# chsakell/aca-dotnet-workshop

Measured on AMD Instinct MI355X. Metric: tasks_e2e_per_sec, higher is better.
Workload: dtype n/a (JSON over HTTP)

## Files before the change

aca_dotnet_workshop_amd/native/src/applog.hpp:

```cpp
#pragma once

#include <fcntl.h>
#include <pthread.h>
#include <sys/stat.h>
#include <unistd.h>

#include <cerrno>
#include <algorithm>
#include <atomic>
#include <chrono>
#include <condition_variable>
#include <cstdint>
#include <cstdio>
#include <cstdlib>
#include <cstring>
#include <exception>
#include <functional>
#include <future>
#include <map>
#include <mutex>
#include <stdexcept>
#include <string>
#include <string_view>
#include <thread>
#include <vector>

namespace tt {

class AppLog {
 public:
  AppLog() = default;
  AppLog(const AppLog&) = delete;
  AppLog& operator=(const AppLog&) = delete;
  ~AppLog() {
    stop_committer();
    close();
  }

  bool open(const std::string& path, int fsync_mode) {
    path_ = path;
    fsync_ = fsync_mode;
    open_fd();
    if (fsync_ == 2 && !gc_thread_.joinable()) gc_thread_ = std::thread([this] { commit_loop(); });
    return true;
  }
  bool is_open() const { return fd_ >= 0; }
  uint64_t bytes() const { return bytes_; }
  const std::string& path() const { return path_; }

  void close() {
    std::lock_guard<std::mutex> f(fd_mu_);
    if (fd_ >= 0) { ::close(fd_); fd_ = -1; }
  }

  bool group() const { return fsync_ == 2 && fd_ >= 0; }
  uint64_t mark() const { return written_.load(std::memory_order_acquire); }
  void after_durable(uint64_t mark, std::function<void()> cb) {
    if (!group() || synced_.load(std::memory_order_acquire) >= mark) {
      cb();
      return;
    }
    {
      std::lock_guard<std::mutex> l(gc_mu_);
      waiters_.emplace(mark, std::move(cb));
      gc_want_ = true;
    }
    gc_cv_.notify_one();
  }
  void wait_durable(uint64_t mark) {
    if (!group() || synced_.load(std::memory_order_acquire) >= mark) return;
    std::promise<void> done;
    auto f = done.get_future();
    after_durable(mark, [&done] { done.set_value(); });
    f.wait();
  }
  void wait_durable() { wait_durable(mark()); }
  struct CommitStats {
    uint64_t syncs, acks, written, synced;
    double sync_ms_total, sync_ms_max;
  };
  CommitStats commit_stats() {
    std::lock_guard<std::mutex> l(gc_mu_);
    return {gc_syncs_, gc_acks_, mark(), synced_.load(), gc_sync_s_ * 1e3, gc_sync_max_s_ * 1e3};
  }

  static void put_field(std::string& rec, std::string_view f) {
    uint32_t n = (uint32_t)f.size();
    rec.append(reinterpret_cast<const char*>(&n), 4);
    rec.append(f.data(), f.size());
  }
  template <class T>
  static std::string_view pod(const T& v) { return std::string_view(reinterpret_cast<const char*>(&v), sizeof(T)); }

  void append(char kind, const std::vector<std::string_view>& fields) {
    if (fd_ < 0) return;
    std::string rec;
    rec.resize(5);
    rec[4] = kind;
    for (auto f : fields) put_field(rec, f);
    uint32_t total = (uint32_t)rec.size();
    std::memcpy(&rec[0], &total, 4);
    if (batching_) {
      batch_ += rec;
      return;
    }
    write_all(rec);
  }

  class BatchScope {
   public:
    explicit BatchScope(AppLog& log) : log_(log) { log_.batching_ = true; }
    ~BatchScope() noexcept(false) {
      log_.batching_ = false;
      if (log_.batch_.empty()) return;
      std::string b;
      b.swap(log_.batch_);
      if (std::uncaught_exceptions() == 0) {
        log_.write_all(b);
        return;
      }
      try {
        log_.write_all(b);
      } catch (...) {
      }
    }
    BatchScope(const BatchScope&) = delete;
    BatchScope& operator=(const BatchScope&) = delete;

   private:
    AppLog& log_;
  };

  void replay(const std::function<void(char, std::vector<std::string_view>&)>& fn) {
    if (fd_ < 0) return;
    std::string data;
    data.resize(bytes_);
    size_t off = 0;
    while (off < data.size()) {
      ssize_t r = ::pread(fd_, &data[off], data.size() - off, (off_t)off);
      if (r <= 0) break;
      off += (size_t)r;
    }
    size_t pos = 0;
    std::vector<std::string_view> fields;
    while (pos + 5 <= off) {
      uint32_t total;
      std::memcpy(&total, &data[pos], 4);
      if (total < 5 || pos + total > off) break;
      char kind = data[pos + 4];
      fields.clear();
      size_t p = pos + 5, end = pos + total;
      bool ok = true;
      while (p < end) {
        if (p + 4 > end) { ok = false; break; }
        uint32_t n;
        std::memcpy(&n, &data[p], 4);
        p += 4;
        if (p + n > end) { ok = false; break; }
        fields.emplace_back(&data[p], n);
        p += n;
      }
      if (!ok) break;
      fn(kind, fields);
      pos = end;
    }
    if (pos < bytes_) {
      if (::ftruncate(fd_, (off_t)pos) == 0) bytes_ = pos;
    }
  }

  void rewrite(const std::function<void(AppLog&)>& writer) {
    if (fd_ < 0) return;
    std::string tmp = path_ + ".compact";
    AppLog out;
    ::unlink(tmp.c_str());
    out.open(tmp, 0);
    writer(out);
    ::fdatasync(out.fd_);
    out.close();
    {
      std::lock_guard<std::mutex> f(fd_mu_);
      if (::rename(tmp.c_str(), path_.c_str()) != 0) throw std::runtime_error("log compaction rename failed");
      if (fd_ >= 0) ::close(fd_);
      fd_ = -1;
      open_fd_locked();
    }
    if (fsync_ == 2) {
      {
        std::lock_guard<std::mutex> l(gc_mu_);
        gc_want_ = true;
      }
      gc_cv_.notify_one();
    }
  }

  void sync() {
    std::lock_guard<std::mutex> f(fd_mu_);
    if (fd_ >= 0) ::fdatasync(fd_);
  }

 private:
  static FILE* stall_file(double& min_s) {
    static double th = [] {
      const char* p = std::getenv("TT_STALL_MS");
      double ms = p && *p ? std::atof(p) : 100.0;
      return (ms > 0 ? ms : 100.0) / 1e3;
    }();
    static FILE* f = [] {
      const char* p = std::getenv("TT_STALL_LOG");
      return p && *p ? std::fopen(p, "a") : nullptr;
    }();
    min_s = th;
    return f;
  }

  void write_all(const std::string& rec) {
    double min_s;
    FILE* stall = stall_file(min_s);
    auto t0 = stall ? std::chrono::steady_clock::now() : std::chrono::steady_clock::time_point{};
    size_t off = 0;
    while (off < rec.size()) {
      ssize_t w = ::write(fd_, rec.data() + off, rec.size() - off);
      if (w < 0) {
        if (errno == EINTR) continue;
        throw std::runtime_error(std::string("log write failed: ") + std::strerror(errno));
      }
      off += (size_t)w;
    }
    bytes_ += rec.size();
    written_.fetch_add(rec.size(), std::memory_order_release);
    if (fsync_ == 1) ::fdatasync(fd_);
    if (stall) {
      double s = std::chrono::duration<double>(std::chrono::steady_clock::now() - t0).count();
      if (s > min_s) {
        double wall = std::chrono::duration<double>(std::chrono::system_clock::now().time_since_epoch()).count();
        std::fprintf(stall, "{\"what\": \"log-write\", \"ms\": %.2f, \"bytes\": %zu, \"log\": \"%s\", \"pid\": %d, \"wall\": %.4f}\n",
                     s * 1e3, rec.size(), path_.c_str(), (int)::getpid(), wall);
        std::fflush(stall);
      }
    }
  }

  void open_fd() {
    std::lock_guard<std::mutex> f(fd_mu_);
    open_fd_locked();
  }
  void open_fd_locked() {
    fd_ = ::open(path_.c_str(), O_RDWR | O_CREAT | O_APPEND | O_CLOEXEC, 0644);
    if (fd_ < 0) throw std::runtime_error("cannot open log " + path_ + ": " + std::strerror(errno));
    struct stat st;
    if (::fstat(fd_, &st) == 0) bytes_ = (uint64_t)st.st_size;
  }

  void commit_loop() {
    pthread_setname_np(pthread_self(), "tt-log-commit");
    std::unique_lock<std::mutex> l(gc_mu_);
    static const auto delay = [] {
      const char* v = std::getenv("TT_LOG_COMMIT_DELAY_US");
      return std::chrono::microseconds(v && *v ? std::max(0L, std::atol(v)) : 100L);
    }();
    while (true) {
      gc_cv_.wait(l, [this] { return gc_stop_ || gc_want_; });
      if (gc_stop_ && waiters_.empty()) return;
      if (delay.count() > 0 && !gc_stop_) gc_cv_.wait_for(l, delay, [this] { return gc_stop_; });
      gc_want_ = false;
      l.unlock();
      const uint64_t target = written_.load(std::memory_order_acquire);
      const auto t0 = std::chrono::steady_clock::now();
      {
        std::lock_guard<std::mutex> f(fd_mu_);
        if (fd_ >= 0) ::fdatasync(fd_);
      }
      const double s = std::chrono::duration<double>(std::chrono::steady_clock::now() - t0).count();
      uint64_t prev = synced_.load();
      while (prev < target && !synced_.compare_exchange_weak(prev, target)) {
      }
      std::vector<std::function<void()>> ready;
      l.lock();
      ++gc_syncs_;
      gc_sync_s_ += s;
      gc_sync_max_s_ = std::max(gc_sync_max_s_, s);
      auto end = waiters_.upper_bound(target);
      for (auto it = waiters_.begin(); it != end; ++it) ready.push_back(std::move(it->second));
      waiters_.erase(waiters_.begin(), end);
      gc_acks_ += ready.size();
      if (!waiters_.empty()) gc_want_ = true;
      l.unlock();
      for (auto& f : ready) f();
      l.lock();
    }
  }
  void stop_committer() {
    if (!gc_thread_.joinable()) return;
    {
      std::lock_guard<std::mutex> l(gc_mu_);
      gc_stop_ = true;
      gc_want_ = true;
    }
    gc_cv_.notify_one();
    gc_thread_.join();
  }

  int fd_ = -1;
  int fsync_ = 0;
  uint64_t bytes_ = 0;
  std::string path_;
  bool batching_ = false;
  std::string batch_;
  std::mutex fd_mu_;
  std::atomic<uint64_t> written_{0}, synced_{0};
  std::mutex gc_mu_;
  std::condition_variable gc_cv_;
  std::multimap<uint64_t, std::function<void()>> waiters_;
  std::thread gc_thread_;
  bool gc_stop_ = false, gc_want_ = false;
  uint64_t gc_syncs_ = 0, gc_acks_ = 0;
  double gc_sync_s_ = 0, gc_sync_max_s_ = 0;
};

}
```

aca_dotnet_workshop_amd/native/src/backingfront.hpp:

```cpp
#pragma once

#include <condition_variable>
#include <deque>
#include <filesystem>
#include <unordered_set>

#include <fcntl.h>
#include <unistd.h>

#include <sys/eventfd.h>

#include <array>
#include <atomic>
#include <cassert>
#include <cstring>
#include <map>
#include <mutex>
#include <shared_mutex>
#include <thread>
#include <unordered_map>

#include "broker.hpp"
#include "docstore.hpp"
#include "evhttp.hpp"
#include "json.hpp"
#include "textutil.hpp"

namespace tt {

namespace bf {

using text::unquote;
inline std::string jstr(std::string_view s) { return text::json_str(s); }
inline bool utf8_ok(std::string_view s) { return text::valid_utf8(s); }
inline std::string b64(std::string_view in) { return text::base64(in); }

inline std::string problem_json(int status, std::string_view detail) {
  return "{\"type\": \"https://tools.ietf.org/html/rfc9110#section-15." + std::to_string(status / 100) +
         "\", \"title\": " + jstr(ev::reason_phrase(status)) + ", \"status\": " + std::to_string(status) +
         ", \"detail\": " + jstr(detail) + "}";
}

struct Grant {
  std::string principal, scope;
  std::vector<std::string> actions;
};

}

inline bool scan_bulk_items(const std::string& body, std::vector<DocStore::BulkItem>& out) {
  std::string_view text = body.empty() ? std::string_view("[]") : std::string_view(body);
  if (!valid(text)) return false;
  const char* p = ws_end(text.data(), text.data() + text.size());
  const char* e = text.data() + text.size();
  if (*p != '[') return false;
  ++p;
  while (true) {
    p = ws_end(p, e);
    if (*p == ']') return true;
    if (*p != '{') return false;
    ++p;
    DocStore::BulkItem b;
    bool have_key = false, have_value = false;
    while (true) {
      p = ws_end(p, e);
      if (*p == '}') { ++p; break; }
      const char* ks = p;
      p = skip_value(p, e);
      std::string_view ktok(ks, (size_t)(p - ks));
      std::string k = ktok.find('\\') == std::string_view::npos ? std::string(ktok.substr(1, ktok.size() - 2))
                                                               : parse(ktok).s;
      p = ws_end(ws_end(p, e) + 1, e);
      const char* vs = p;
      p = skip_value(p, e);
      std::string_view raw(vs, (size_t)(p - vs));
      if (k == "key") {
        if (raw.front() != '"') return false;
        b.key = raw.find('\\') == std::string_view::npos ? std::string(raw.substr(1, raw.size() - 2)) : parse(raw).s;
        have_key = true;
      } else if (k == "value") {
        have_value = true;
        b.value = raw.front() == '"' ? parse(raw).s : compact(raw);
      } else if (k == "etag") {
        b.etag.reset();
        if (raw.front() == '"') {
          std::string s = parse(raw).s;
          if (!s.empty()) b.etag = std::move(s);
        }
      } else if (k == "firstWrite") {
        b.first_write = raw == "true";
      } else if (k == "ttlMs") {
        if (raw.front() != 'n' && raw.front() != '"' && std::strtod(std::string(raw).c_str(), nullptr) != 0) return false;
      }
      p = ws_end(p, e);
      if (*p == ',') ++p;
    }
    if (!have_key) return false;
    if (!have_value) b.value = "null";
    out.push_back(std::move(b));
    p = ws_end(p, e);
    if (*p == ',') ++p;
  }
}

inline bool scan_value_array(const char* p, const char* e, std::vector<std::string>& out);

inline bool scan_bulk_values(const std::string& body, std::vector<std::string>& out) {
  std::string_view text = body.empty() ? std::string_view("[]") : std::string_view(body);
  if (!valid(text)) return false;
  return scan_value_array(ws_end(text.data(), text.data() + text.size()), text.data() + text.size(), out);
}

inline bool scan_tx_values(const std::string& body, std::vector<std::string>& out) {
  std::string_view text(body);
  if (text.empty() || !valid(text)) return false;
  const char* e = text.data() + text.size();
  const char* p = ws_end(text.data(), e);
  if (*p != '{') return false;
  ++p;
  bool found = false;
  while (true) {
    p = ws_end(p, e);
    if (*p == '}') return found;
    const char* ks = p;
    p = skip_value(p, e);
    std::string_view ktok(ks, (size_t)(p - ks));
    std::string k = ktok.find('\\') == std::string_view::npos ? std::string(ktok.substr(1, ktok.size() - 2))
                                                             : parse(ktok).s;
    p = ws_end(ws_end(p, e) + 1, e);
    if (k == "ops") {
      out.clear();
      if (!scan_value_array(p, e, out)) return false;
      found = true;
    }
    p = ws_end(skip_value(p, e), e);
    if (*p == ',') ++p;
  }
}

inline bool scan_value_array(const char* p, const char* e, std::vector<std::string>& out) {
  if (*p != '[') return false;
  ++p;
  while (true) {
    p = ws_end(p, e);
    if (*p == ']') return true;
    if (*p != '{') return false;
    ++p;
    std::string value = "null";
    while (true) {
      p = ws_end(p, e);
      if (*p == '}') { ++p; break; }
      const char* ks = p;
      p = skip_value(p, e);
      std::string_view ktok(ks, (size_t)(p - ks));
      std::string k = ktok.find('\\') == std::string_view::npos ? std::string(ktok.substr(1, ktok.size() - 2))
                                                               : parse(ktok).s;
      p = ws_end(ws_end(p, e) + 1, e);
      const char* vs = p;
      p = skip_value(p, e);
      std::string_view raw(vs, (size_t)(p - vs));
      if (k == "value") value = raw.front() == '"' ? parse(raw).s : compact(raw);
      p = ws_end(p, e);
      if (*p == ',') ++p;
    }
    out.push_back(std::move(value));
    p = ws_end(p, e);
    if (*p == ',') ++p;
  }
}

class BackingFront {
 public:
  BackingFront(const std::string& host, int port, const std::string& fallback_uds, int threads = 1,
               const std::string& uds = "")
      : fallback_(ev::Endpoint::parse("unix:" + fallback_uds)) {
    ev::reserve_fd_table();
    threads = std::max(1, std::min(threads, 64));
    for (int i = 0; i < threads; ++i) {
      shards_.push_back(std::make_shared<Shard>(*this));
      shards_.back()->self = shards_.back();
    }
    ev::Endpoint ep;
    ep.unix_socket = false;
    ep.host = host;
    ep.port = port;
    for (auto& sh : shards_) {
      int p = ev::listen_on(sh->loop, ep, sh->handler, threads > 1);
      if (ep.port == 0) ep.port = p;
    }
    port_ = ep.port;
    if (!uds.empty()) {
      ev::Endpoint u;
      u.path = uds;
      int unused = 0;
      int fd = ev::bind_listen(u, false, unused);
      for (size_t i = 0; i < shards_.size(); ++i) {
        int f = i == 0 ? fd : ::fcntl(fd, F_DUPFD_CLOEXEC, 0);
        if (f < 0) break;
        auto l = std::make_shared<ev::Listener>(shards_[i]->loop, f, shards_[i]->handler);
        l->hand_off = [this, i](int c) {
          size_t to = next_uds_shard_.fetch_add(1, std::memory_order_relaxed) % shards_.size();
          if (to == i) return false;
          Shard* sh = shards_[to].get();
          sh->post_task([sh, c] { ev::adopt(sh->loop, c, sh->handler); });
          return true;
        };
        shards_[i]->loop.add(l, EPOLLIN | EPOLLEXCLUSIVE);
      }
    }
    for (auto& sh : shards_) sh->start();
  }
  ~BackingFront() { stop(); }

  struct QueryJob {
    std::string account, db, coll, body, prefix, traceparent, sent_mono, front_mono;
    bool sort_keys = false;
  };
  struct QueryResult {
    int status = 0;
    std::string body;
    ev::HeaderList headers;
  };
  using QueryFn = std::function<QueryResult(const QueryJob&)>;
  void set_query_fn(QueryFn fn) {
    std::lock_guard l(q_mu_);
    query_fn_ = std::move(fn);
    if (q_threads_.empty() && query_fn_) {
      int n = 4;
      if (const char* v = std::getenv("TT_BACKING_QUERY_THREADS"); v && std::atoi(v) > 0) n = std::min(32, std::atoi(v));
      for (int i = 0; i < n; ++i)
        q_threads_.emplace_back([this] {
          pthread_setname_np(pthread_self(), "tt-front-query");
          query_loop();
        });
    }
  }

  int port() const { return port_; }
  int threads() const { return (int)shards_.size(); }

  void stop() {
    if (stopped_) return;
    stopped_ = true;
    {
      std::lock_guard l(q_mu_);
      q_stop_ = true;
    }
    q_cv_.notify_all();
    for (auto& t : q_threads_)
      if (t.joinable()) t.join();
    q_threads_.clear();
    {
      std::lock_guard l(q_mu_);
      query_fn_ = nullptr;
    }
    for (auto& sh : shards_) sh->request_stop();
    for (auto& sh : shards_) sh->join();
  }

  void attach_store(const std::string& account, const std::string& db, const std::string& coll, DocStore* s) {
    std::unique_lock l(cfg_mu_);
    auto& c = colls_[account + "\x1f" + db + "\x1f" + coll];
    if (!c) c = std::make_unique<Coll>();
    c->store = s;
  }
  void attach_broker(const std::string& ns, Broker* b) {
    std::unique_lock l(cfg_mu_);
    brokers_[ns] = b;
  }
  void set_policy(const std::string& mode, const std::vector<std::pair<std::string, std::string>>& keys,
                  const std::vector<std::tuple<std::string, std::string, std::vector<std::string>>>& grants) {
    std::unique_lock l(cfg_mu_);
    enforce_ = mode == "enforce";
    keys_ = keys;
    grants_.clear();
    for (auto& [p, s, a] : grants) grants_.push_back(bf::Grant{p, s, a});
  }
  void set_blob_root(const std::string& root) {
    std::lock_guard l(blob_mu_);
    blob_root_ = root;
  }
  void blob_note(const std::string& account, const std::string& container, const std::string& name, bool added) {
    std::lock_guard l(blob_mu_);
    auto& names = blob_names_locked(account, container);
    if (added) names.insert(name);
    else names.erase(name);
  }
  size_t blob_count(const std::string& account, const std::string& container, const std::string& prefix) {
    std::lock_guard l(blob_mu_);
    auto& names = blob_names_locked(account, container);
    if (prefix.empty()) return names.size();
    size_t n = 0;
    for (auto& x : names) n += x.compare(0, prefix.size(), prefix) == 0;
    return n;
  }

  void notify(const std::string& ns, const std::string& entity) {
    for (auto& sh : shards_) sh->post(ns + "|" + entity);
  }
  std::map<std::string, uint64_t> stats() {
    std::map<std::string, uint64_t> out;
    for (size_t i = 0; i < kCounters.size(); ++i)
      if (uint64_t v = counters_[i].load(std::memory_order_relaxed)) out[kCounters[i]] = v;
    return out;
  }

 private:
  struct Coll {
    DocStore* store = nullptr;
  };
  struct Shard;
  struct QueuedQuery {
    std::shared_ptr<QueryJob> job;
    Shard* sh = nullptr;
    ev::Reply reply;
  };
  std::mutex q_mu_;
  std::condition_variable q_cv_;
  std::deque<QueuedQuery> q_jobs_;
  QueryFn query_fn_;
  std::vector<std::thread> q_threads_;
  bool q_stop_ = false;
  struct Parked {
    std::string ns, entity;
    size_t max;
    int64_t lock_ms;
    double deadline;
    ev::Reply reply;
    bool storage = false;
  };
  struct Shard;
  struct Wake : ev::IoObj {
    Shard* sh;
    explicit Wake(Shard* x) : sh(x) {}
    void on_event(uint32_t) override;
  };
  struct Shard {
    BackingFront& f;
    ev::Loop loop;
    ev::Client client;
    ev::Handler handler;
    std::thread thread;
    int wake_fd = -1;
    std::atomic<bool> stop_flag{false};
    std::mutex mu;
    std::vector<std::string> posted;
    std::vector<std::function<void()>> tasks;
    std::multimap<std::string, Parked> parked;
    std::weak_ptr<Shard> self;

    explicit Shard(BackingFront& front) : f(front), client(loop) {
      handler = [this](ev::Message&& m, ev::Reply r) { f.on_request(*this, std::move(m), std::move(r)); };
      wake_fd = eventfd(0, EFD_NONBLOCK | EFD_CLOEXEC);
      auto w = std::make_shared<Wake>(this);
      w->fd = dup(wake_fd);
      loop.add(w, EPOLLIN);
    }
    ~Shard() {
      if (wake_fd >= 0) ::close(wake_fd);
    }
    void start() {
      thread = std::thread([this] {
        pthread_setname_np(pthread_self(), "tt-front");
        ev::GapTracer gaps("backing-front");
        gaps.attach(loop);
        loop.run([this, &gaps](double t) {
          gaps.tick(t);
          on_tick(t);
        });
      });
    }
    std::atomic<bool> wake_pending{false};
    void wake() {
      if (wake_pending.exchange(true, std::memory_order_acq_rel)) return;
      uint64_t one = 1;
      ssize_t r = ::write(wake_fd, &one, sizeof one);
      (void)r;
    }
    void post(std::string key) {
      {
        std::lock_guard l(mu);
        posted.push_back(std::move(key));
      }
      wake();
    }
    void post_task(std::function<void()> fn) {
      {
        std::lock_guard l(mu);
        tasks.push_back(std::move(fn));
      }
      wake();
    }
    void request_stop() {
      stop_flag = true;
      wake();
    }
    void join() {
      if (thread.joinable()) thread.join();
    }
    void on_wake() {
      if (stop_flag) {
        for (auto& kv : parked) kv.second.reply.json(503, bf::problem_json(503, "shutting down"));
        parked.clear();
        loop.stop();
        return;
      }
      std::vector<std::string> keys;
      std::vector<std::function<void()>> todo;
      wake_pending.store(false, std::memory_order_release);
      {
        std::lock_guard l(mu);
        keys.swap(posted);
        todo.swap(tasks);
      }
      for (auto& k : keys) f.retry_parked(*this, k);
      for (auto& fn : todo) fn();
    }
    void on_tick(double now) {
      if (stop_flag) {
        on_wake();
        return;
      }
      std::vector<std::string> keys;
      for (auto& kv : parked)
        if (keys.empty() || keys.back() != kv.first) keys.push_back(kv.first);
      for (auto& k : keys) f.retry_parked(*this, k, now);
    }
  };

  ev::Endpoint fallback_;
  std::vector<std::shared_ptr<Shard>> shards_;
  std::atomic<size_t> next_uds_shard_{0};
  int port_ = 0;
  bool stopped_ = false;

  std::shared_mutex cfg_mu_;
  std::unordered_map<std::string, std::unique_ptr<Coll>> colls_;
  std::unordered_map<std::string, Broker*> brokers_;
  bool enforce_ = false;
  std::vector<std::pair<std::string, std::string>> keys_;
  std::vector<bf::Grant> grants_;
  std::mutex blob_mu_;
  std::string blob_root_;
  std::unordered_map<std::string, std::unordered_set<std::string>> blob_names_;

  std::unordered_set<std::string>& blob_names_locked(const std::string& account, const std::string& container) {
    std::string key = account + "/" + container;
    auto it = blob_names_.find(key);
    if (it != blob_names_.end()) return it->second;
    auto& names = blob_names_[key];
    namespace fs = std::filesystem;
    std::error_code ec;
    fs::path root = fs::path(blob_root_) / account / container;
    if (!blob_root_.empty() && fs::is_directory(root, ec))
      for (auto i = fs::recursive_directory_iterator(root, ec); !ec && i != fs::recursive_directory_iterator();
           i.increment(ec)) {
        if (!i->is_regular_file(ec)) continue;
        std::string n = i->path().lexically_relative(root).string();
        if (!ends_with(n, ".meta.json") && !ends_with(n, ".tmp")) names.insert(std::move(n));
      }
    return names;
  }
  static bool ends_with(const std::string& s, const char* suf) {
    size_t n = std::strlen(suf);
    return s.size() >= n && s.compare(s.size() - n, n, suf) == 0;
  }
  static bool safe_name(const std::string& in, std::string& out) {
    out.clear();
    for (unsigned char c : in) {
      if (c >= 0x80) return false;
      bool keep = (c >= 'a' && c <= 'z') || (c >= 'A' && c <= 'Z') || (c >= '0' && c <= '9') || c == '.' || c == '_' ||
                  c == '-';
      out += keep ? (char)c : '_';
    }
    return true;
  }
  static bool write_file(const std::string& path, std::string_view data) {
    int fd = ::open(path.c_str(), O_WRONLY | O_CREAT | O_TRUNC | O_CLOEXEC, 0644);
    if (fd < 0) return false;
    size_t off = 0;
    while (off < data.size()) {
      ssize_t w = ::write(fd, data.data() + off, data.size() - off);
      if (w < 0 && errno == EINTR) continue;
      if (w <= 0) {
        ::close(fd);
        return false;
      }
      off += (size_t)w;
    }
    return ::close(fd) == 0;
  }

  bool handle_blob(ev::Message& m, ev::Reply& r, const std::vector<std::string>& seg, const std::string& qs) {
    std::string acct, cont, root;
    if (!safe_name(seg[1], acct) || !safe_name(seg[3], cont)) return false;
    {
      std::lock_guard l(blob_mu_);
      root = blob_root_;
    }
    if (root.empty()) return false;
    if (seg.size() == 4 && m.method == "GET") {
      std::string c = query_get(qs, "count");
      for (auto& ch : c) ch = ::tt::ascii_lower(ch);
      if (c != "1" && c != "true") return false;
      if (!authorize(m, r, "blob.read", "storage/" + seg[1])) return true;
      count("blob.count");
      r.send(200, {{"content-type", "application/json"}},
             "{\"count\": " + std::to_string(blob_count(acct, cont, query_get(qs, "prefix"))) + "}");
      return true;
    }
    if (seg.size() < 5 || m.method != "PUT") return false;
    std::string name;
    for (size_t i = 4; i < seg.size(); ++i) {
      const std::string& p = seg[i];
      if (p.empty() || p == "." || p == ".." || p.find('/') != std::string::npos) return false;
      for (unsigned char c : p)
        if (c < 0x20 || c >= 0x80) return false;
      if (i > 4) name += '/';
      name += p;
    }
    if (ends_with(name, ".tmp") || ends_with(name, ".meta.json")) return false;
    if (!authorize(m, r, "blob.write", "storage/" + seg[1])) return true;
    count("blob.put");
    namespace fs = std::filesystem;
    fs::path f = fs::path(root) / acct / cont / name;
    std::error_code ec;
    fs::create_directories(f.parent_path(), ec);
    const std::string tmp = f.string() + ".tmp";
    auto* ct = m.header("content-type");
    char meta[160];
    std::snprintf(meta, sizeof meta, ", \"lastModified\": %.6f, \"size\": %zu}",
                  std::chrono::duration<double>(std::chrono::system_clock::now().time_since_epoch()).count(),
                  m.body.size());
    if (ec || !write_file(tmp, m.body) || ::rename(tmp.c_str(), f.c_str()) != 0 ||
        !write_file(f.string() + ".meta.json",
                    "{\"contentType\": " + bf::jstr(ct ? *ct : "application/octet-stream") + meta)) {
      r.send(500, {{"content-type", "application/problem+json; charset=utf-8"}},
             bf::problem_json(500, "blob write failed: " + f.string()));
      return true;
    }
    blob_note(acct, cont, name, true);
    r.send(201, {{"content-type", "application/json"}},
           "{\"blobURL\": " + bf::jstr("/storage/" + seg[1] + "/blobs/" + seg[3] + "/" + name) + "}");
    return true;
  }

  static constexpr std::array<const char*, 19> kCounters = {
      "doc.put", "sb.publish", "sb.receive", "sb.settle", "doc.get", "doc.bulkget", "doc.bulkset", "doc.query",
      "doc.throttled", "doc.delete", "doc.query_worker", "doc.query_worker_done", "forwarded",
      "queue.put", "queue.get", "queue.delete", "queue.update", "blob.put", "blob.count"};
  std::array<std::atomic<uint64_t>, kCounters.size()> counters_{};

  void count(const char* k) {
    for (size_t i = 0; i < kCounters.size(); ++i)
      if (std::strcmp(kCounters[i], k) == 0) {
        counters_[i].fetch_add(1, std::memory_order_relaxed);
        return;
      }
    assert(!"unknown backing front counter");
  }
  void broadcast(Shard& here, const std::string& key) {
    retry_parked(here, key);
    if (shards_.size() > 1)
      for (auto& sh : shards_)
        if (sh.get() != &here) sh->post(key);
  }

  bool allowed(const ev::Message& m, const std::string& action, const std::string& scope) {
    std::shared_lock l(cfg_mu_);
    if (!enforce_) return true;
    auto* key = m.header("x-tt-key");
    if (key && !key->empty())
      for (auto& [ks, k] : keys_)
        if (scope.rfind(ks, 0) == 0 && *key == k) return true;
    auto* ident = m.header("x-tt-identity");
    if (ident && !ident->empty())
      for (auto& g : grants_) {
        if (g.principal != *ident || scope.rfind(g.scope, 0) != 0) continue;
        for (auto& a : g.actions)
          if (a == "*" || a == action) return true;
      }
    return false;
  }
  bool authorize(const ev::Message& m, const ev::Reply& r, const std::string& action, const std::string& scope) {
    if (allowed(m, action, scope)) return true;
    auto* ident = m.header("x-tt-identity");
    std::string who = ident && !ident->empty() ? *ident : "anonymous";
    r.send(403, {{"content-type", "application/problem+json; charset=utf-8"}},
           bf::problem_json(403, who + " is not authorized to perform " + action + " on " + scope));
    return false;
  }

  static void split(const std::string& target, std::string& path, std::string& qs) {
    auto q = target.find('?');
    path = target.substr(0, q);
    qs = q == std::string::npos ? "" : target.substr(q + 1);
  }
  static std::string query_get(const std::string& qs, const std::string& name) {
    size_t i = 0;
    while (i <= qs.size() && !qs.empty()) {
      size_t j = qs.find('&', i);
      if (j == std::string::npos) j = qs.size();
      std::string_view kv(qs.data() + i, j - i);
      size_t eq = kv.find('=');
      if (bf::unquote(kv.substr(0, eq), true) == name)
        return eq == std::string_view::npos ? "" : bf::unquote(kv.substr(eq + 1), true);
      i = j + 1;
    }
    return "";
  }

  void on_request(Shard& sh, ev::Message&& m, ev::Reply r) {
    std::string path, qs;
    split(m.target, path, qs);
    std::vector<std::string> seg;
    seg.reserve(8);
    for (size_t i = 1; i <= path.size();) {
      size_t j = path.find('/', i);
      if (j == std::string::npos) j = path.size();
      seg.push_back(bf::unquote(std::string_view(path).substr(i, j - i)));
      i = j + 1;
    }
    if (seg.size() == 6 && seg[0] == "cosmos" && seg[4] == "docs" && handle_doc(sh, m, r, seg)) return;
    if (seg.size() == 5 && seg[0] == "cosmos" && seg[4] == "bulkset" && m.method == "POST" &&
        handle_bulkset(sh, m, r, seg))
      return;
    if (seg.size() == 5 && seg[0] == "cosmos" && seg[4] == "bulkget" && m.method == "POST" && handle_bulkget(m, r, seg))
      return;
    if (seg.size() == 5 && seg[0] == "cosmos" && seg[4] == "query" && m.method == "POST" && handle_query(sh, m, r, seg, qs))
      return;
    if (seg.size() >= 3 && seg[0] == "servicebus" && handle_bus(sh, m, r, seg, qs)) return;
    if (seg.size() >= 5 && seg[0] == "storage" && seg[2] == "queues" && handle_storage_queue(sh, m, r, seg, qs)) return;
    if (seg.size() >= 4 && seg[0] == "storage" && seg[2] == "blobs" && handle_blob(m, r, seg, qs)) return;
    forward(sh, std::move(m), std::move(r));
  }

  void forward(Shard& sh, ev::Message&& m, ev::Reply r) {
    count("forwarded");
    ev::HeaderList h;
    for (auto& kv : m.headers)
      if (!ev::is_hop_header(kv.first)) h.push_back(kv);
    if (m.header("traceparent")) {
      char t[32];
      std::snprintf(t, sizeof t, "%.6f", ev::now_s());
      h.emplace_back("x-tt-front-mono", t);
    }
    sh.client.request(fallback_, m.method, m.target, h, m.body, 0, [r](ev::ClientResult&& res) {
      if (res.err) {
        r.send(503, {{"content-type", "application/problem+json; charset=utf-8"}},
               bf::problem_json(503, "backing control plane unreachable"));
        return;
      }
      if (res.resp.header("x-tt-handler-end-mono")) {
        ev::HeaderList h2 = res.resp.headers;
        char t[32];
        std::snprintf(t, sizeof t, "%.6f", ev::now_s());
        h2.emplace_back("x-tt-front-rx-mono", t);
        r.send(res.resp.status, h2, res.resp.body);
        return;
      }
      r.send(res.resp.status, res.resp.headers, res.resp.body);
    });
  }

  bool throttled(ev::Message& m, ev::Reply& r, DocStore* s, double ru, int kind) {
    if (!s->provisioned()) {
      s->charge(ru);
      return false;
    }
    uint64_t ticket = 0, out = 0;
    if (const std::string* t = m.header("x-tt-ru-ticket")) ticket = std::strtoull(t->c_str(), nullptr, 10);
    const uint64_t bind = DocStore::bind_of(m.method + " " + m.target,
                                            kind == DocStore::kQuery || m.method == "POST" ? std::string_view(m.body)
                                                                                           : std::string_view());
    int64_t wait_ms = s->charge(ru, ticket, out, bind, kind);
    if (!wait_ms) return false;
    count("doc.throttled");
    ev::HeaderList h{{"x-ms-retry-after-ms", std::to_string(wait_ms)},
                     {"retry-after", std::to_string((wait_ms + 999) / 1000)},
                     {"content-type", "application/problem+json; charset=utf-8"}};
    if (out) h.emplace_back("x-tt-ru-ticket", std::to_string(out));
    r.send(429, h, bf::problem_json(429, "Request rate is large: the container's provisioned throughput is exhausted"));
    return true;
  }

  Coll* coll_of(const std::vector<std::string>& seg) {
    thread_local std::string k;
    k.assign(seg[1]);
    k += '\x1f';
    k += seg[2];
    k += '\x1f';
    k += seg[3];
    std::shared_lock l(cfg_mu_);
    auto it = colls_.find(k);
    return it != colls_.end() && it->second->store ? it->second.get() : nullptr;
  }

  template <class Engine>
  void send_durable(Shard& sh, Engine* eng, ev::Reply& r, int status, ev::HeaderList h, std::string body) {
    if (!eng->group_commit()) {
      r.send(status, h, body);
      return;
    }
    std::weak_ptr<Shard> w = sh.self;
    eng->after_durable(eng->log_mark(), [w, r, status, h = std::move(h), body = std::move(body)] {
      if (auto s = w.lock()) s->post_task([r, status, h, body] { r.send(status, h, body); });
    });
  }

  bool handle_doc(Shard& sh, ev::Message& m, ev::Reply& r, const std::vector<std::string>& seg) {
    Coll* c = coll_of(seg);
    if (!c) return false;
    const std::string& key = seg[5];
    const std::string scope = "cosmos/" + seg[1];
    if (m.method == "GET") {
      if (!authorize(m, r, "cosmos.read", scope)) return true;
      count("doc.get");
      if (throttled(m, r, c->store, DocStore::read_ru(0), DocStore::kRead)) return true;
      auto v = c->store->get(key);
      if (!v) r.empty(404);
      else r.send(200, {{"etag", v->second}, {"content-type", "application/json"}}, v->first);
      return true;
    }
    if (m.method != "PUT" && m.method != "DELETE") return false;
    auto* ttl = m.header("x-tt-ttl-ms");
    if (ttl && !ttl->empty() && *ttl != "0") return false;
    if (!authorize(m, r, "cosmos.write", scope)) return true;
    auto* im = m.header("if-match");
    std::optional<std::string> etag;
    if (im && !im->empty()) etag = *im;
    const char* pj = "application/problem+json; charset=utf-8";
    if (throttled(m, r, c->store, DocStore::write_ru(m.method == "PUT" ? m.body.size() : 0),
                  m.method == "PUT" ? DocStore::kWrite : DocStore::kDelete))
      return true;
    if (m.method == "PUT") {
      count("doc.put");
      auto* fw = m.header("x-tt-first-write");
      try {
        std::string e = c->store->set(key, m.body, etag, fw && *fw == "1", 0);
        send_durable(sh, c->store, r, 200, {{"etag", e}, {"content-type", "application/json"}},
                     "{\"etag\": " + bf::jstr(e) + "}");
      } catch (const EtagMismatch& ex) {
        r.send(412, {{"content-type", pj}}, bf::problem_json(412, ex.what()));
      } catch (const ParseError& ex) {
        r.send(400, {{"content-type", pj}}, bf::problem_json(400, std::string("invalid JSON: ") + ex.what()));
      }
      return true;
    }
    count("doc.delete");
    try {
      bool ok = c->store->del(key, etag);
      if (ok) send_durable(sh, c->store, r, 204, {}, {});
      else r.empty(404);
    } catch (const EtagMismatch& ex) {
      r.send(412, {{"content-type", pj}}, bf::problem_json(412, ex.what()));
    }
    return true;
  }

  bool handle_bulkset(Shard& sh, ev::Message& m, ev::Reply& r, const std::vector<std::string>& seg) {
    Coll* c = coll_of(seg);
    if (!c) return false;
    std::vector<DocStore::BulkItem> batch;
    if (!scan_bulk_items(m.body, batch)) return false;
    if (!authorize(m, r, "cosmos.write", "cosmos/" + seg[1])) return true;
    count("doc.bulkset");
    double ru = 0;
    for (auto& b : batch) ru += DocStore::write_ru(b.value.size());
    if (throttled(m, r, c->store, ru, DocStore::kWrite)) return true;
    const std::vector<DocStore::BulkResult> res = c->store->set_many(batch);
    std::string out = "[";
    bool etag_err = false, other_err = false;
    for (size_t i = 0; i < res.size(); ++i) {
      if (i) out += ", ";
      out += "{\"key\": " + bf::jstr(batch[i].key);
      if (res[i].err == 0) {
        out += ", \"etag\": " + bf::jstr(res[i].etag) + "}";
      } else {
        (res[i].err == 1 ? etag_err : other_err) = true;
        out += std::string(", \"error\": ") + (res[i].err == 1 ? "\"etag\"" : "\"invalid\"") +
               ", \"detail\": " + bf::jstr(res[i].detail) + "}";
      }
    }
    out += "]";
    send_durable(sh, c->store, r, etag_err ? 412 : other_err ? 400 : 200, {{"content-type", "application/json"}}, out);
    return true;
  }

  bool handle_bulkget(ev::Message& m, ev::Reply& r, const std::vector<std::string>& seg) {
    Coll* c = coll_of(seg);
    if (!c) return false;
    Value body;
    try {
      body = parse(m.body);
    } catch (const ParseError&) {
      return false;
    }
    const Value* keys = body.get("keys");
    if (!keys || keys->t != Value::Array) return false;
    for (auto& k : keys->items)
      if (k.t != Value::String) return false;
    if (!authorize(m, r, "cosmos.read", "cosmos/" + seg[1])) return true;
    count("doc.bulkget");
    if (throttled(m, r, c->store, DocStore::read_ru(0) * (double)std::max<size_t>(1, keys->items.size()), DocStore::kRead))
      return true;
    std::string out = "[";
    for (size_t i = 0; i < keys->items.size(); ++i) {
      const std::string& k = keys->items[i].s;
      if (i) out += ", ";
      out += "{\"key\": " + bf::jstr(k);
      if (auto v = c->store->get(k)) out += ", \"data\": " + v->first + ", \"etag\": " + bf::jstr(v->second);
      out += "}";
    }
    out += "]";
    r.send(200, {{"content-type", "application/json"}}, out);
    return true;
  }

  static bool indexable(const Value* f) {
    if (!f || f->t != Value::Object || f->keys.size() != 1) return false;
    std::string op = f->keys[0];
    for (auto& ch : op) ch = (char)std::toupper((unsigned char)ch);
    const Value& arg = f->items[0];
    if (op == "EQ" || op == "IN") {
      if (arg.t != Value::Object || arg.items.empty()) return false;
      const Value& v = arg.items[0];
      auto plain = [](const Value& x) { return x.t == Value::Null || x.t == Value::Bool; };
      if (v.t != Value::Array) return !plain(v);
      for (auto& x : v.items)
        if (!plain(x)) return true;
      return false;
    }
    if (op == "AND") {
      if (arg.t != Value::Array) return false;
      for (auto& x : arg.items)
        if (indexable(&x)) return true;
      return false;
    }
    if (op == "OR") {
      if (arg.t != Value::Array || arg.items.empty()) return false;
      for (auto& x : arg.items)
        if (!indexable(&x)) return false;
      return true;
    }
    return false;
  }
  static bool sampled(const ev::Message& m) {
    const std::string* tp = m.header("traceparent");
    if (!tp || tp->size() < 55) return false;
    return (std::strtol(tp->c_str() + tp->size() - 2, nullptr, 16) & 1) != 0;
  }

  bool to_query_worker(Shard& sh, ev::Message& m, ev::Reply& r, Coll* c, const std::vector<std::string>& seg,
                       const std::string& qs) {
    {
      std::lock_guard l(q_mu_);
      if (!query_fn_ || q_stop_) return false;
    }
    if (!authorize(m, r, "cosmos.read", "cosmos/" + seg[1])) return true;
    if (throttled(m, r, c->store, DocStore::query_ru(0), DocStore::kQuery)) return true;
    count("doc.query_worker");
    auto job = std::make_shared<QueryJob>();
    job->account = seg[1];
    job->db = seg[2];
    job->coll = seg[3];
    job->body = std::move(m.body);
    job->prefix = query_get(qs, "prefix");
    std::string project = query_get(qs, "project");
    for (auto& ch : project) ch = (char)std::tolower((unsigned char)ch);
    job->sort_keys = project == "sortkeys";
    if (const std::string* tp = m.header("traceparent")) job->traceparent = *tp;
    if (const std::string* t = m.header("x-tt-sent-mono")) job->sent_mono = *t;
    char t[32];
    std::snprintf(t, sizeof t, "%.6f", ev::now_s());
    job->front_mono = t;
    {
      std::lock_guard l(q_mu_);
      q_jobs_.push_back({job, &sh, r});
    }
    q_cv_.notify_one();
    return true;
  }

  void query_loop() {
    while (true) {
      QueuedQuery qq;
      QueryFn fn;
      {
        std::unique_lock l(q_mu_);
        q_cv_.wait(l, [this] { return q_stop_ || !q_jobs_.empty(); });
        if (q_stop_) {
          for (auto& j : q_jobs_)
            j.sh->post_task([r = j.reply] { r.json(503, bf::problem_json(503, "shutting down")); });
          q_jobs_.clear();
          return;
        }
        qq = std::move(q_jobs_.front());
        q_jobs_.pop_front();
        fn = query_fn_;
      }
      QueryResult res;
      try {
        res = fn(*qq.job);
      } catch (const std::exception& ex) {
        res.status = 500;
        res.body = ex.what();
      }
      qq.sh->post_task([this, qq, res = std::move(res)]() mutable {
        count("doc.query_worker_done");
        if (res.status == 200) {
          if (!res.headers.empty()) {
            char t[32];
            std::snprintf(t, sizeof t, "%.6f", ev::now_s());
            res.headers.emplace_back("x-tt-front-rx-mono", t);
          }
          res.headers.emplace_back("content-type", "application/json");
          qq.reply.send(200, res.headers, res.body);
        } else {
          qq.reply.send(res.status ? res.status : 500, {{"content-type", "application/problem+json; charset=utf-8"}},
                        bf::problem_json(res.status ? res.status : 500, res.body));
        }
      });
    }
  }

  bool handle_query(Shard& sh, ev::Message& m, ev::Reply& r, const std::vector<std::string>& seg, const std::string& qs) {
    Coll* c = coll_of(seg);
    if (!c) return false;
    bool indexed = false;
    try {
      Value q = parse(m.body.empty() ? std::string("{}") : m.body);
      if (q.t != Value::Object) return false;
      indexed = indexable(q.get("filter"));
    } catch (const ParseError&) {
      return false;
    }
    if (!indexed || sampled(m)) return to_query_worker(sh, m, r, c, seg, qs);
    if (!authorize(m, r, "cosmos.read", "cosmos/" + seg[1])) return true;
    if (throttled(m, r, c->store, DocStore::query_ru(0), DocStore::kQuery)) return true;
    std::string body;
    try {
      std::string project = query_get(qs, "project");
      for (auto& ch : project) ch = (char)std::tolower((unsigned char)ch);
      body = c->store->query(m.body, query_get(qs, "prefix"), project == "sortkeys");
    } catch (const std::exception& ex) {
      r.send(400, {{"content-type", "application/problem+json; charset=utf-8"}}, bf::problem_json(400, ex.what()));
      return true;
    }
    count("doc.query");
    c->store->debit(DocStore::query_ru(body.size()) - DocStore::query_ru(0));
    r.send(200, {{"content-type", "application/json"}}, body);
    return true;
  }

  static std::string entity_scope(const std::string& entity) {
    auto p = entity.find("/subscriptions/");
    if (p != std::string::npos) return "topics/" + entity.substr(0, p);
    return "queues/" + entity;
  }

  bool handle_bus(Shard& sh, ev::Message& m, ev::Reply& r, const std::vector<std::string>& seg,
                  const std::string& qs) {
    Broker* b = nullptr;
    {
      std::shared_lock l(cfg_mu_);
      auto it = brokers_.find(seg[1]);
      if (it != brokers_.end()) b = it->second;
    }
    if (!b) return false;
    const std::string& ns = seg[1];
    if (seg.size() == 5 && seg[2] == "topics" && seg[4] == "messages" && m.method == "POST") {
      if (!authorize(m, r, "sb.send", "servicebus/" + ns + "/topics/" + seg[3])) return true;
      count("sb.publish");
      auto* ct = m.header("content-type");
      auto* props = m.header("x-tt-props");
      auto* mid = m.header("x-tt-message-id");
      auto* ttl = m.header("x-tt-ttl-ms");
      auto* delay = m.header("x-tt-delay-ms");
      uint64_t seq = b->publish(seg[3], m.body, ct ? *ct : "application/json", props ? *props : "{}", mid ? *mid : "",
                                ttl && !ttl->empty() ? std::atoll(ttl->c_str()) : 0,
                                delay && !delay->empty() ? std::atoll(delay->c_str()) : 0);
      send_durable(sh, b, r, 201, {{"content-type", "application/json"}}, "{\"seq\": " + std::to_string(seq) + "}");
      for (auto& sub : b->subscriptions(seg[3])) broadcast(sh, ns + "|" + seg[3] + "/subscriptions/" + sub);
      return true;
    }
    if (seg.size() == 3 && seg[2] == "receive" && m.method == "POST") {
      std::string entity = query_get(qs, "entity");
      if (!authorize(m, r, "sb.receive", "servicebus/" + ns + "/" + entity_scope(entity))) return true;
      count("sb.receive");
      std::string mx = query_get(qs, "max"), lk = query_get(qs, "lockMs"), wt = query_get(qs, "waitMs");
      Parked p{ns, entity, (size_t)std::max(1, mx.empty() ? 1 : std::atoi(mx.c_str())),
               lk.empty() ? 0 : std::atoll(lk.c_str()), ev::now_s() + (wt.empty() ? 0 : std::atoi(wt.c_str())) / 1000.0,
               r};
      if (!try_receive(b, p, false)) sh.parked.emplace(ns + "|" + entity, std::move(p));
      return true;
    }
    if (seg.size() == 3 && seg[2] == "settle" && m.method == "POST") {
      Value body;
      try {
        body = parse(m.body.empty() ? std::string_view("{}") : std::string_view(m.body));
      } catch (const std::exception&) {
        return false;
      }
      std::string entity;
      if (auto* e = body.get("entity"); e && e->t == Value::String) entity = e->s;
      if (!authorize(m, r, "sb.receive", "servicebus/" + ns + "/" + entity_scope(entity))) return true;
      count("sb.settle");
      auto list = [&](const char* k) -> const std::vector<Value>* {
        auto* v = body.get(k);
        return v && v->t == Value::Array ? &v->items : nullptr;
      };
      auto str = [](const Value& o, const char* k) {
        auto* v = o.get(k);
        return v && v->t == Value::String ? v->s : std::string();
      };
      auto num = [](const Value& o, const char* k) {
        auto* v = o.get(k);
        return v && v->t == Value::Number ? (int64_t)v->n : (int64_t)0;
      };
      std::string out = "{\"complete\": [";
      if (auto* l = list("complete"))
        for (size_t i = 0; i < l->size(); ++i) out += std::string(i ? ", " : "") + (b->complete(entity, (*l)[i].s) ? "true" : "false");
      out += "], \"abandon\": [";
      bool abandoned = false;
      if (auto* l = list("abandon"))
        for (size_t i = 0; i < l->size(); ++i) {
          abandoned = true;
          out += std::string(i ? ", " : "") +
                 (b->abandon(entity, str((*l)[i], "token"), num((*l)[i], "delayMs")) ? "true" : "false");
        }
      out += "], \"deadletter\": [";
      if (auto* l = list("deadletter"))
        for (size_t i = 0; i < l->size(); ++i)
          out += std::string(i ? ", " : "") +
                 (b->dead_letter(entity, str((*l)[i], "token"), str((*l)[i], "reason")) ? "true" : "false");
      out += "], \"renew\": [";
      if (auto* l = list("renew"))
        for (size_t i = 0; i < l->size(); ++i)
          out += std::string(i ? ", " : "") +
                 (b->renew(entity, str((*l)[i], "token"), num((*l)[i], "lockMs")) ? "true" : "false");
      out += "]}";
      send_durable(sh, b, r, 200, {{"content-type", "application/json"}}, out);
      if (abandoned) broadcast(sh, ns + "|" + entity);
      return true;
    }
    if (seg.size() == 3 && seg[2] == "counts" && m.method == "GET") {
      auto [a, s, l, d, e, c, rc] = b->counts(query_get(qs, "entity"));
      r.send(200, {{"content-type", "application/json"}},
             "{\"active\": " + std::to_string(a) + ", \"scheduled\": " + std::to_string(s) + ", \"locked\": " +
                 std::to_string(l) + ", \"dead_letter\": " + std::to_string(d) + ", \"enqueued\": " + std::to_string(e) +
                 ", \"completed\": " + std::to_string(c) + ", \"received\": " + std::to_string(rc) + "}");
      return true;
    }
    return false;
  }

  static bool plain_uint(const std::string& v, int64_t& out) {
    if (v.empty() || v.size() > 15) return false;
    int64_t x = 0;
    for (char c : v) {
      if (c < '0' || c > '9') return false;
      x = x * 10 + (c - '0');
    }
    out = x;
    return true;
  }
  static bool uint_param(const std::string& qs, const char* name, int64_t dflt, int64_t& out) {
    std::string v = query_get(qs, name);
    if (v.empty()) {
      out = dflt;
      return true;
    }
    return plain_uint(v, out);
  }

  bool handle_storage_queue(Shard& sh, ev::Message& m, ev::Reply& r, const std::vector<std::string>& seg,
                            const std::string& qs) {
    const std::string ns = "storage-" + seg[1];
    Broker* b = nullptr;
    {
      std::shared_lock l(cfg_mu_);
      auto it = brokers_.find(ns);
      if (it != brokers_.end()) b = it->second;
    }
    if (!b) return false;
    const std::string& account = seg[1];
    const std::string& queue = seg[3];
    if (seg.size() == 5 && seg[4] == "messages" && m.method == "POST") {
      int64_t ttl_s, delay_s;
      if (!uint_param(qs, "messagettl", 0, ttl_s) || !uint_param(qs, "visibilitytimeout", 0, delay_s)) return false;
      if (!authorize(m, r, "queue.send", "storage/" + account)) return true;
      count("queue.put");
      uint64_t seq = b->send(queue, m.body, "text/plain", "{}", "", ttl_s * 1000, delay_s * 1000);
      send_durable(sh, b, r, 201, {{"content-type", "application/json"}},
                   "{\"messageId\": \"" + std::to_string(seq) + "\"}");
      broadcast(sh, ns + "|" + queue);
      return true;
    }
    if (seg.size() == 5 && seg[4] == "messages" && m.method == "GET") {
      int64_t mx, vis, wait_ms;
      if (!uint_param(qs, "numofmessages", 1, mx) || mx < 1 || !uint_param(qs, "visibilityMs", 30000, vis) ||
          !uint_param(qs, "waitMs", 0, wait_ms))
        return false;
      if (!authorize(m, r, "queue.receive", "storage/" + account)) return true;
      count("queue.get");
      Parked p{ns, queue, (size_t)mx, vis, ev::now_s() + (double)wait_ms / 1000.0, r, true};
      if (!try_receive(b, p, false)) sh.parked.emplace(ns + "|" + queue, std::move(p));
      return true;
    }
    if (seg.size() == 6 && seg[4] == "messages" && (m.method == "DELETE" || m.method == "PUT")) {
      int64_t vis = 0;
      if (m.method == "PUT" && !uint_param(qs, "visibilityMs", 0, vis)) return false;
      if (!authorize(m, r, "queue.receive", "storage/" + account)) return true;
      count(m.method == "DELETE" ? "queue.delete" : "queue.update");
      bool ok = m.method == "DELETE" ? b->complete(queue, seg[5]) : b->abandon(queue, seg[5], vis);
      send_durable(sh, b, r, ok ? 204 : 404, {}, "");
      if (m.method == "PUT") broadcast(sh, ns + "|" + queue);
      return true;
    }
    return false;
  }

  bool try_receive(Broker* b, Parked& p, bool expired) {
    if (p.reply.abandoned()) {
      p.reply.send(204, {}, {});
      return true;
    }
    std::vector<Received> msgs;
    try {
      msgs = b->receive(p.entity, p.max, p.lock_ms);
    } catch (const std::exception& e) {
      p.reply.send(404, {{"content-type", "application/problem+json; charset=utf-8"}}, bf::problem_json(404, e.what()));
      return true;
    }
    if (msgs.empty() && !expired && ev::now_s() < p.deadline) return false;
    std::string out = "[";
    if (p.storage) {
      for (size_t i = 0; i < msgs.size(); ++i) {
        auto& x = msgs[i];
        if (i) out += ", ";
        out += "{\"messageId\": \"" + std::to_string(x.seq) + "\", \"popReceipt\": " + bf::jstr(x.lock_token) +
               ", \"dequeueCount\": " + std::to_string(x.delivery_count) +
               ", \"insertionMs\": " + std::to_string(x.enqueued_wall);
        if (bf::utf8_ok(x.body)) out += ", \"body\": " + bf::jstr(x.body) + "}";
        else out += ", \"bodyB64\": \"" + bf::b64(x.body) + "\"}";
      }
      out += "]";
      p.reply.send(200, {{"content-type", "application/json"}}, out);
      return true;
    }
    for (size_t i = 0; i < msgs.size(); ++i) {
      auto& x = msgs[i];
      if (i) out += ", ";
      std::string props = x.props.empty() ? "{}" : x.props;
      out += "{\"lockToken\": " + bf::jstr(x.lock_token) + ", \"seq\": " + std::to_string(x.seq) + ", \"id\": " +
             bf::jstr(x.id) + ", \"contentType\": " + bf::jstr(x.content_type) + ", \"props\": " + props +
             ", \"deliveryCount\": " + std::to_string(x.delivery_count) + ", \"enqueuedMs\": " +
             std::to_string(x.enqueued_wall);
      if (bf::utf8_ok(x.body)) out += ", \"body\": " + bf::jstr(x.body) + "}";
      else out += ", \"bodyB64\": \"" + bf::b64(x.body) + "\"}";
    }
    out += "]";
    p.reply.send(200, {{"content-type", "application/json"}}, out);
    return true;
  }

  void retry_parked(Shard& sh, const std::string& key, double now = 0) {
    auto range = sh.parked.equal_range(key);
    if (range.first == range.second) return;
    Broker* b = nullptr;
    {
      std::shared_lock l(cfg_mu_);
      auto it = brokers_.find(key.substr(0, key.find('|')));
      if (it != brokers_.end()) b = it->second;
    }
    for (auto it = range.first; it != range.second;) {
      bool expired = now > 0 && now >= it->second.deadline;
      if (b && try_receive(b, it->second, expired)) it = sh.parked.erase(it);
      else ++it;
    }
  }
};

inline void BackingFront::Wake::on_event(uint32_t) {
  uint64_t v;
  while (::read(fd, &v, sizeof v) == (ssize_t)sizeof v) {
  }
  sh->on_wake();
}

}
```

aca_dotnet_workshop_amd/native/src/broker.hpp:

```cpp
#pragma once

#include <chrono>
#include <cstdint>
#include <deque>
#include <map>
#include <memory>
#include <mutex>
#include <random>
#include <string>
#include <tuple>
#include <unordered_map>
#include <vector>

#include "applog.hpp"

namespace tt {

inline int64_t mono_ms() {
  return std::chrono::duration_cast<std::chrono::milliseconds>(std::chrono::steady_clock::now().time_since_epoch()).count();
}
inline int64_t wall_ms() {
  return std::chrono::duration_cast<std::chrono::milliseconds>(std::chrono::system_clock::now().time_since_epoch()).count();
}

struct Message {
  uint64_t seq = 0;
  std::string id;
  std::string body;
  std::string content_type;
  std::string props;
  int64_t enqueued_wall = 0;
  int64_t visible_at = 0;
  int64_t expires_at = 0;
  uint32_t delivery_count = 0;
  std::string lock_token;
  int64_t locked_until = 0;
  std::string dl_reason;
};
using MsgPtr = std::shared_ptr<Message>;

struct Received {
  std::string lock_token;
  uint64_t seq;
  std::string id;
  std::string body;
  std::string content_type;
  std::string props;
  uint32_t delivery_count;
  int64_t enqueued_wall;
};

struct QueueOptions {
  int64_t lock_ms = 60000;
  uint32_t max_delivery = 10;
  int64_t default_ttl_ms = 0;
  bool dead_letter_on_expiry = false;
};

class Queue {
 public:
  std::string path;
  QueueOptions opt;
  std::map<uint64_t, MsgPtr> ready;
  std::multimap<int64_t, MsgPtr> delayed;
  std::unordered_map<std::string, MsgPtr> locked;
  std::multimap<int64_t, std::string> lock_expiry;
  std::deque<MsgPtr> dlq;
  uint64_t n_enqueued = 0, n_completed = 0, n_dead = 0, n_received = 0, n_expired = 0;

  void enqueue(MsgPtr m, int64_t now) {
    ++n_enqueued;
    if (m->visible_at > now) delayed.emplace(m->visible_at, m);
    else ready.emplace(m->seq, m);
  }

  void tick(int64_t now) {
    while (!delayed.empty() && delayed.begin()->first <= now) {
      MsgPtr m = delayed.begin()->second;
      delayed.erase(delayed.begin());
      ready.emplace(m->seq, m);
    }
    while (!lock_expiry.empty() && lock_expiry.begin()->first <= now) {
      std::string tok = lock_expiry.begin()->second;
      lock_expiry.erase(lock_expiry.begin());
      auto it = locked.find(tok);
      if (it == locked.end() || it->second->locked_until > now) continue;
      MsgPtr m = it->second;
      locked.erase(it);
      release(m, now, "MaxDeliveryCountExceeded");
    }
  }

  void release(MsgPtr m, int64_t now, const char* reason) {
    m->lock_token.clear();
    m->locked_until = 0;
    if (opt.max_delivery && m->delivery_count >= opt.max_delivery) {
      dead_letter(m, reason);
      return;
    }
    if (m->visible_at > now) delayed.emplace(m->visible_at, m);
    else ready.emplace(m->seq, m);
  }

  void dead_letter(MsgPtr m, const std::string& reason) {
    m->dl_reason = reason;
    m->lock_token.clear();
    dlq.push_back(m);
    ++n_dead;
  }
};

class Broker {
 public:
  explicit Broker(const std::string& path = "", int fsync_mode = 0) : rng_(std::random_device{}()) {
    if (!path.empty()) {
      log_.open(path, fsync_mode);
      replaying_ = true;
      log_.replay([this](char kind, std::vector<std::string_view>& f) { apply_log(kind, f); });
      replaying_ = false;
    }
  }

  void create_queue(const std::string& name, const QueueOptions& o) {
    std::lock_guard<std::mutex> g(mu_);
    auto& q = queues_[name];
    q.path = name;
    q.opt = o;
  }

  void create_topic(const std::string& topic) {
    std::lock_guard<std::mutex> g(mu_);
    topics_[topic];
  }

  void create_subscription(const std::string& topic, const std::string& sub, const QueueOptions& o) {
    std::lock_guard<std::mutex> g(mu_);
    auto& t = topics_[topic];
    auto it = t.find(sub);
    if (it == t.end()) {
      std::string p = topic + "/subscriptions/" + sub;
      auto& q = t[sub];
      q.path = p;
      q.opt = o;
      if (!replaying_) log_.append('S', {topic, sub, AppLog::pod(o.lock_ms), AppLog::pod(o.max_delivery),
                                         AppLog::pod(o.default_ttl_ms)});
    } else {
      it->second.opt = o;
    }
  }

  bool delete_entity(const std::string& path) {
    std::lock_guard<std::mutex> g(mu_);
    if (queues_.erase(path)) return true;
    auto [topic, sub] = split(path);
    auto t = topics_.find(topic);
    if (t == topics_.end()) return false;
    if (sub.empty()) { topics_.erase(t); return true; }
    return t->second.erase(sub) > 0;
  }

  std::vector<std::string> subscriptions(const std::string& topic) {
    std::lock_guard<std::mutex> g(mu_);
    std::vector<std::string> out;
    auto t = topics_.find(topic);
    if (t != topics_.end())
      for (auto& [n, _] : t->second) out.push_back(n);
    return out;
  }

  std::vector<std::string> entities() {
    std::lock_guard<std::mutex> g(mu_);
    std::vector<std::string> out;
    for (auto& [n, _] : queues_) out.push_back(n);
    for (auto& [t, subs] : topics_) {
      out.push_back(t);
      for (auto& [s, _] : subs) out.push_back(t + "/subscriptions/" + s);
    }
    return out;
  }

  uint64_t publish(const std::string& topic, const std::string& body, const std::string& ctype,
                   const std::string& props, const std::string& id, int64_t ttl_ms, int64_t delay_ms) {
    std::lock_guard<std::mutex> g(mu_);
    auto& t = topics_[topic];
    uint64_t seq = ++seq_;
    int64_t now = mono_ms();
    std::string mid = id.empty() ? new_id() : id;
    for (auto& [name, q] : t) {
      auto m = make(seq, mid, body, ctype, props, ttl_ms ? ttl_ms : q.opt.default_ttl_ms, delay_ms, now);
      q.enqueue(m, now);
    }
    if (!t.empty()) log_msg('P', topic, seq, mid, body, ctype, props);
    total_published_++;
    return t.empty() ? 0 : seq;
  }

  uint64_t send(const std::string& queue, const std::string& body, const std::string& ctype,
                const std::string& props, const std::string& id, int64_t ttl_ms, int64_t delay_ms) {
    std::lock_guard<std::mutex> g(mu_);
    auto& q = queue_locked(queue);
    uint64_t seq = ++seq_;
    int64_t now = mono_ms();
    std::string mid = id.empty() ? new_id() : id;
    q.enqueue(make(seq, mid, body, ctype, props, ttl_ms ? ttl_ms : q.opt.default_ttl_ms, delay_ms, now), now);
    log_msg('Q', queue, seq, mid, body, ctype, props);
    total_published_++;
    return seq;
  }

  std::vector<Received> receive(const std::string& path, size_t max_messages, int64_t lock_ms) {
    std::lock_guard<std::mutex> g(mu_);
    Queue* q = find(path, true);
    std::vector<Received> out;
    if (!q) return out;
    int64_t now = mono_ms();
    q->tick(now);
    int64_t lms = lock_ms > 0 ? lock_ms : q->opt.lock_ms;
    while (out.size() < max_messages && !q->ready.empty()) {
      MsgPtr m = q->ready.begin()->second;
      q->ready.erase(q->ready.begin());
      if (m->expires_at && m->expires_at <= now) {
        ++q->n_expired;
        if (q->opt.dead_letter_on_expiry) q->dead_letter(m, "TTLExpiredException");
        continue;
      }
      m->delivery_count++;
      m->lock_token = new_token();
      m->locked_until = now + lms;
      q->locked.emplace(m->lock_token, m);
      q->lock_expiry.emplace(m->locked_until, m->lock_token);
      q->n_received++;
      out.push_back({m->lock_token, m->seq, m->id, m->body, m->content_type, m->props, m->delivery_count,
                     m->enqueued_wall});
    }
    return out;
  }

  bool complete(const std::string& path, const std::string& token) {
    std::lock_guard<std::mutex> g(mu_);
    Queue* q = find(path, false);
    if (!q) return false;
    auto it = q->locked.find(token);
    if (it == q->locked.end()) return false;
    uint64_t seq = it->second->seq;
    q->locked.erase(it);
    q->n_completed++;
    if (log_.is_open()) log_.append('C', {path, AppLog::pod(seq)});
    return true;
  }

  bool abandon(const std::string& path, const std::string& token, int64_t delay_ms) {
    std::lock_guard<std::mutex> g(mu_);
    Queue* q = find(path, false);
    if (!q) return false;
    auto it = q->locked.find(token);
    if (it == q->locked.end()) return false;
    MsgPtr m = it->second;
    q->locked.erase(it);
    int64_t now = mono_ms();
    m->visible_at = now + std::max<int64_t>(0, delay_ms);
    q->release(m, now, "MaxDeliveryCountExceeded");
    if (!m->dl_reason.empty() && log_.is_open()) log_.append('C', {path, AppLog::pod(m->seq)});
    return true;
  }

  bool dead_letter(const std::string& path, const std::string& token, const std::string& reason) {
    std::lock_guard<std::mutex> g(mu_);
    Queue* q = find(path, false);
    if (!q) return false;
    auto it = q->locked.find(token);
    if (it == q->locked.end()) return false;
    MsgPtr m = it->second;
    q->locked.erase(it);
    q->dead_letter(m, reason);
    if (log_.is_open()) log_.append('C', {path, AppLog::pod(m->seq)});
    return true;
  }

  bool renew(const std::string& path, const std::string& token, int64_t lock_ms) {
    std::lock_guard<std::mutex> g(mu_);
    Queue* q = find(path, false);
    if (!q) return false;
    auto it = q->locked.find(token);
    if (it == q->locked.end()) return false;
    int64_t now = mono_ms();
    it->second->locked_until = now + (lock_ms > 0 ? lock_ms : q->opt.lock_ms);
    q->lock_expiry.emplace(it->second->locked_until, token);
    return true;
  }

  std::vector<std::tuple<uint64_t, std::string, std::string, std::string, uint32_t>> drain_dead_letters(
      const std::string& path, size_t max) {
    std::lock_guard<std::mutex> g(mu_);
    std::vector<std::tuple<uint64_t, std::string, std::string, std::string, uint32_t>> out;
    Queue* q = find(path, false);
    if (!q) return out;
    while (out.size() < max && !q->dlq.empty()) {
      MsgPtr m = q->dlq.front();
      q->dlq.pop_front();
      out.emplace_back(m->seq, m->id, m->body, m->dl_reason, m->delivery_count);
    }
    return out;
  }

  std::tuple<size_t, size_t, size_t, size_t, uint64_t, uint64_t, uint64_t> counts(const std::string& path) {
    std::lock_guard<std::mutex> g(mu_);
    Queue* q = find(path, false);
    if (!q) return {0, 0, 0, 0, 0, 0, 0};
    q->tick(mono_ms());
    return {q->ready.size(), q->delayed.size(), q->locked.size(), q->dlq.size(), q->n_enqueued, q->n_completed,
            q->n_received};
  }

  size_t purge(const std::string& path) {
    std::lock_guard<std::mutex> g(mu_);
    Queue* q = find(path, false);
    if (!q) return 0;
    size_t n = q->ready.size() + q->delayed.size();
    q->ready.clear();
    q->delayed.clear();
    return n;
  }

  uint64_t total_published() {
    std::lock_guard<std::mutex> g(mu_);
    return total_published_;
  }

  bool group_commit() const { return log_.group(); }
  uint64_t log_mark() const { return log_.mark(); }
  void after_durable(uint64_t mark, std::function<void()> cb) { log_.after_durable(mark, std::move(cb)); }
  void wait_durable() { log_.wait_durable(); }
  AppLog::CommitStats commit_stats() { return log_.commit_stats(); }

 private:
  static std::pair<std::string, std::string> split(const std::string& path) {
    auto pos = path.find("/subscriptions/");
    if (pos == std::string::npos) return {path, ""};
    return {path.substr(0, pos), path.substr(pos + 15)};
  }

  Queue& queue_locked(const std::string& name) {
    auto it = queues_.find(name);
    if (it != queues_.end()) return it->second;
    auto& q = queues_[name];
    q.path = name;
    return q;
  }

  Queue* find(const std::string& path, bool create) {
    auto [topic, sub] = split(path);
    if (sub.empty()) {
      auto it = queues_.find(path);
      if (it != queues_.end()) return &it->second;
      if (!create) return nullptr;
      return &queue_locked(path);
    }
    auto& t = topics_[topic];
    auto it = t.find(sub);
    if (it != t.end()) return &it->second;
    if (!create) return nullptr;
    auto& q = t[sub];
    q.path = path;
    if (!replaying_ && log_.is_open()) log_.append('S', {topic, sub, AppLog::pod(q.opt.lock_ms),
                                                        AppLog::pod(q.opt.max_delivery), AppLog::pod(q.opt.default_ttl_ms)});
    return &q;
  }

  MsgPtr make(uint64_t seq, const std::string& id, const std::string& body, const std::string& ctype,
              const std::string& props, int64_t ttl_ms, int64_t delay_ms, int64_t now) {
    auto m = std::make_shared<Message>();
    m->seq = seq;
    m->id = id;
    m->body = body;
    m->content_type = ctype;
    m->props = props;
    m->enqueued_wall = wall_ms();
    m->visible_at = now + std::max<int64_t>(0, delay_ms);
    m->expires_at = ttl_ms > 0 ? now + ttl_ms : 0;
    return m;
  }

  std::string new_token() {
    uint64_t a = rng_(), b = rng_();
    char buf[40];
    std::snprintf(buf, sizeof buf, "%016llx%016llx", (unsigned long long)a, (unsigned long long)b);
    return buf;
  }
  std::string new_id() {
    uint64_t a = rng_(), b = rng_();
    char buf[40];
    std::snprintf(buf, sizeof buf, "%08llx-%04llx-4%03llx-%04llx-%012llx", (unsigned long long)(a >> 32),
                  (unsigned long long)((a >> 16) & 0xffff), (unsigned long long)(a & 0xfff),
                  (unsigned long long)(0x8000 | ((b >> 48) & 0x3fff)), (unsigned long long)(b & 0xffffffffffffULL));
    return buf;
  }

  void log_msg(char kind, const std::string& entity, uint64_t seq, const std::string& id, const std::string& body,
               const std::string& ctype, const std::string& props) {
    if (!log_.is_open() || replaying_) return;
    log_.append(kind, {entity, AppLog::pod(seq), id, body, ctype, props});
  }

  void apply_log(char kind, std::vector<std::string_view>& f) {
    int64_t now = mono_ms();
    if (kind == 'S' && f.size() == 5) {
      QueueOptions o;
      std::memcpy(&o.lock_ms, f[2].data(), 8);
      std::memcpy(&o.max_delivery, f[3].data(), 4);
      std::memcpy(&o.default_ttl_ms, f[4].data(), 8);
      auto& q = topics_[std::string(f[0])][std::string(f[1])];
      q.path = std::string(f[0]) + "/subscriptions/" + std::string(f[1]);
      q.opt = o;
    } else if ((kind == 'P' || kind == 'Q') && f.size() == 6) {
      uint64_t seq;
      std::memcpy(&seq, f[1].data(), 8);
      seq_ = std::max(seq_, seq);
      std::string entity(f[0]);
      if (kind == 'P') {
        for (auto& [name, q] : topics_[entity]) {
          q.enqueue(make(seq, std::string(f[2]), std::string(f[3]), std::string(f[4]), std::string(f[5]), 0, 0, now), now);
          pending_[q.path][seq] = true;
        }
      } else {
        auto& q = queue_locked(entity);
        q.enqueue(make(seq, std::string(f[2]), std::string(f[3]), std::string(f[4]), std::string(f[5]), 0, 0, now), now);
      }
    } else if (kind == 'C' && f.size() == 2) {
      uint64_t seq;
      std::memcpy(&seq, f[1].data(), 8);
      Queue* q = find(std::string(f[0]), false);
      if (q) q->ready.erase(seq);
    }
  }

  std::mutex mu_;
  std::map<std::string, Queue> queues_;
  std::map<std::string, std::map<std::string, Queue>> topics_;
  std::unordered_map<std::string, std::map<uint64_t, bool>> pending_;
  AppLog log_;
  bool replaying_ = false;
  uint64_t seq_ = 0;
  uint64_t total_published_ = 0;
  std::mt19937_64 rng_;
};

}
```

aca_dotnet_workshop_amd/native/src/docstore.hpp:

```cpp
#pragma once

#include <sys/random.h>

#include <algorithm>
#include <atomic>
#include <chrono>
#include <cmath>
#include <cstdint>
#include <map>
#include <memory>
#include <mutex>
#include <optional>
#include <string>
#include <thread>
#include <unordered_map>
#include <unordered_set>
#include <vector>

#include "applog.hpp"
#include "json.hpp"
#include "shardedmap.hpp"

namespace tt {

struct EtagMismatch : std::runtime_error {
  using std::runtime_error::runtime_error;
};
struct QueryError : std::runtime_error {
  using std::runtime_error::runtime_error;
};

inline int64_t now_ms() {
  return std::chrono::duration_cast<std::chrono::milliseconds>(std::chrono::system_clock::now().time_since_epoch()).count();
}

struct Filter {
  enum Op { ALL, EQ, NEQ, GT, GTE, LT, LTE, IN, AND, OR } op = ALL;
  std::string path;
  Value val;
  std::vector<Value> vals;
  std::vector<Filter> kids;
};

inline bool ieq(std::string_view a, const char* b) {
  size_t n = std::strlen(b);
  if (a.size() != n) return false;
  for (size_t i = 0; i < n; ++i)
    if (std::toupper((unsigned char)a[i]) != b[i]) return false;
  return true;
}

inline Filter compile_filter(const Value& f) {
  Filter out;
  if (f.t == Value::Null) return out;
  if (f.t != Value::Object) throw QueryError("filter must be an object");
  if (f.keys.empty()) return out;
  if (f.keys.size() != 1) throw QueryError("filter object must have exactly one operator");
  const std::string& op = f.keys[0];
  const Value& arg = f.items[0];
  if (ieq(op, "AND") || ieq(op, "OR")) {
    out.op = ieq(op, "AND") ? Filter::AND : Filter::OR;
    if (arg.t != Value::Array || arg.items.empty()) throw QueryError(op + " expects a non-empty array");
    for (auto& k : arg.items) out.kids.push_back(compile_filter(k));
    return out;
  }
  static const std::pair<const char*, Filter::Op> table[] = {
      {"EQ", Filter::EQ}, {"NEQ", Filter::NEQ}, {"GT", Filter::GT}, {"GTE", Filter::GTE},
      {"LT", Filter::LT}, {"LTE", Filter::LTE}, {"IN", Filter::IN}};
  bool found = false;
  for (auto& [name, code] : table)
    if (ieq(op, name)) { out.op = code; found = true; }
  if (!found) throw QueryError("unsupported filter operator " + op);
  if (arg.t != Value::Object || arg.keys.size() != 1) throw QueryError(op + " expects {\"path\": value}");
  out.path = arg.keys[0];
  if (out.op == Filter::IN) {
    if (arg.items[0].t != Value::Array) throw QueryError("IN expects an array of values");
    out.vals = arg.items[0].items;
  } else {
    out.val = arg.items[0];
  }
  return out;
}

inline bool eval_filter(const Filter& f, const Value& doc) {
  switch (f.op) {
    case Filter::ALL: return true;
    case Filter::AND:
      for (auto& k : f.kids) if (!eval_filter(k, doc)) return false;
      return true;
    case Filter::OR:
      for (auto& k : f.kids) if (eval_filter(k, doc)) return true;
      return false;
    case Filter::IN: {
      const Value* v = doc.path(f.path);
      if (!v) return false;
      for (auto& x : f.vals) if (equals(*v, x)) return true;
      return false;
    }
    default: {
      const Value* v = doc.path(f.path);
      if (!v) return f.op == Filter::NEQ;
      if (f.op == Filter::EQ) return equals(*v, f.val);
      if (f.op == Filter::NEQ) return !equals(*v, f.val);
      if (v->t != f.val.t) return false;
      int c = compare(*v, f.val);
      switch (f.op) {
        case Filter::GT: return c > 0;
        case Filter::GTE: return c >= 0;
        case Filter::LT: return c < 0;
        case Filter::LTE: return c <= 0;
        default: return false;
      }
    }
  }
}

struct SortKey {
  std::string path;
  bool desc = false;
};

struct Doc {
  std::string value;
  Value parsed;
  uint64_t etag = 0;
  uint64_t seq = 0;
  int64_t expire_ms = 0;
  uint32_t mrow = UINT32_MAX;
};

inline void mirror_key(const Value& v, std::string& k) {
  k.clear();
  switch (v.t) {
    case Value::Null: k = "n"; break;
    case Value::Bool: k = v.b ? "b1" : "b0"; break;
    case Value::Number: {
      double d = v.n + 0.0;
      uint64_t bits;
      std::memcpy(&bits, &d, sizeof bits);
      k.assign("d");
      k.append(reinterpret_cast<const char*>(&bits), sizeof bits);
      break;
    }
    case Value::String: k = "s"; k += v.s; break;
    default: k = "j"; dump_to(k, v);
  }
}

struct MirrorColumn {
  std::string path;
  ShardedMap<int32_t> dict;
  std::vector<std::string> values;
  std::vector<int32_t> ids;
};

struct ColumnMirror {
  bool on = false;
  bool disabled = false;
  uint64_t gen = 1;
  std::vector<MirrorColumn> cols;
  std::vector<std::pair<const std::string, Doc>*> nodes;
  std::vector<int64_t> seqs;
  std::vector<uint8_t> live;
  std::vector<uint32_t> kills;
  size_t live_rows = 0;
  uint64_t compactions = 0;
};

struct MirrorDelta {
  uint64_t gen = 0;
  bool on = false, disabled = false, full = false;
  size_t n = 0, from = 0, kill_cursor = 0;
  std::vector<std::string> paths;
  std::vector<size_t> dict_from;
  std::vector<std::vector<std::string>> new_values;
  std::vector<std::vector<int32_t>> ids;
  std::vector<int64_t> seqs;
  std::vector<uint8_t> live;
  std::vector<uint32_t> kills;
};

struct TxOp {
  bool is_delete = false;
  std::string key;
  std::string value;
  std::optional<std::string> etag;
  bool first_write = false;
  int64_t ttl_ms = 0;
};

class DocStore {
 public:
  explicit DocStore(const std::string& path = "", int fsync_mode = 0, size_t index_threshold = 256)
      : index_threshold_(index_threshold) {
    if (!path.empty()) {
      log_.open(path, fsync_mode);
      log_.replay([this](char kind, std::vector<std::string_view>& f) { apply_log(kind, f); });
    }
  }

  std::string set(const std::string& key, const std::string& value, const std::optional<std::string>& etag,
                  bool first_write, int64_t ttl_ms) {
    Value parsed = parse(value);
    std::string text(value);
    std::vector<Doc> graveyard;
    std::lock_guard<std::mutex> g(mu_);
    int64_t now = now_ms();
    auto it = docs_.find(key);
    check_etag_at(it, etag, first_write, now);
    it = put_at(it, key, std::move(text), std::move(parsed), ttl_ms > 0 ? now + ttl_ms : 0, &graveyard);
    log_put(key, it->second.value, it->second.etag, it->second.expire_ms);
    maybe_compact();
    return std::to_string(it->second.etag);
  }

  struct BulkItem {
    std::string key, value;
    std::optional<std::string> etag;
    bool first_write = false;
    bool have_parsed = false;
    Value parsed;
  };
  struct BulkResult {
    std::string etag;
    int err = 0;
    std::string detail;
  };
  std::vector<BulkResult> set_many(std::vector<BulkItem>& items) {
    std::vector<BulkResult> out(items.size());
    for (size_t i = 0; i < items.size(); ++i) {
      if (items[i].have_parsed) continue;
      try {
        items[i].parsed = parse(items[i].value);
      } catch (const ParseError& e) {
        out[i].err = 2;
        out[i].detail = std::string("invalid JSON: ") + e.what();
      }
    }
    std::vector<Doc> graveyard;
    graveyard.reserve(items.size());
    {
      std::lock_guard<std::mutex> g(mu_);
      {
        AppLog::BatchScope batch(log_);
        const int64_t now = now_ms();
        for (size_t i = 0; i < items.size(); ++i) {
          if (out[i].err) continue;
          BulkItem& it = items[i];
          auto dit = docs_.find(it.key);
          const bool exists = dit != docs_.end() && !expired(dit->second, now);
          if (it.etag && !it.etag->empty()) {
            if (!exists || *it.etag != std::to_string(dit->second.etag)) {
              out[i].err = 1;
              out[i].detail = "possible etag mismatch";
              continue;
            }
          } else if (it.first_write && exists) {
            out[i].err = 1;
            out[i].detail = "possible etag mismatch: first-write on existing key without etag";
            continue;
          }
          dit = put_at(dit, it.key, std::move(it.value), std::move(it.parsed), 0, &graveyard);
          log_put(it.key, dit->second.value, dit->second.etag, dit->second.expire_ms);
          out[i].etag = std::to_string(dit->second.etag);
        }
      }
      maybe_compact();
    }
    return out;
  }

  std::optional<std::pair<std::string, std::string>> get(const std::string& key) {
    std::lock_guard<std::mutex> g(mu_);
    auto it = docs_.find(key);
    if (it == docs_.end()) return std::nullopt;
    if (expired(it->second, now_ms())) { erase_locked(key, true); return std::nullopt; }
    return std::make_pair(it->second.value, std::to_string(it->second.etag));
  }

  bool del(const std::string& key, const std::optional<std::string>& etag) {
    std::lock_guard<std::mutex> g(mu_);
    auto it = docs_.find(key);
    int64_t now = now_ms();
    if (it == docs_.end() || expired(it->second, now)) {
      if (etag && !etag->empty()) throw EtagMismatch("possible etag mismatch: key not found");
      return false;
    }
    if (etag && !etag->empty() && *etag != std::to_string(it->second.etag)) throw EtagMismatch("possible etag mismatch");
    erase_locked(key, true);
    maybe_compact();
    return true;
  }

  void transact(const std::vector<TxOp>& ops) {
    std::vector<Value> parsed(ops.size());
    for (size_t i = 0; i < ops.size(); ++i)
      if (!ops[i].is_delete) parsed[i] = parse(ops[i].value);
    std::lock_guard<std::mutex> g(mu_);
    int64_t now = now_ms();
    for (auto& op : ops) {
      if (op.is_delete) {
        if (op.etag && !op.etag->empty()) {
          auto it = docs_.find(op.key);
          if (it == docs_.end() || *op.etag != std::to_string(it->second.etag)) throw EtagMismatch("possible etag mismatch in transaction");
        }
      } else {
        check_etag(op.key, op.etag, op.first_write, now);
      }
    }
    log_.append('T', {std::string_view("begin")});
    for (size_t i = 0; i < ops.size(); ++i) {
      auto& op = ops[i];
      if (op.is_delete) {
        if (docs_.count(op.key)) erase_locked(op.key, true);
      } else {
        uint64_t e = put(op.key, op.value, std::move(parsed[i]), op.ttl_ms > 0 ? now + op.ttl_ms : 0);
        log_put(op.key, op.value, e, docs_[op.key].expire_ms);
      }
    }
    log_.append('T', {std::string_view("commit")});
    maybe_compact();
  }

  static void sort_keys_to(std::string& out, std::string_view key, const Doc& d, const std::vector<std::string>& paths) {
    out += "{\"key\":";
    escape_to(out, key);
    out += ",\"etag\":\"";
    out += std::to_string(d.etag);
    out += "\",\"sort\":[";
    for (size_t j = 0; j < paths.size(); ++j) {
      if (j) out += ',';
      const Value* v = d.parsed.path(paths[j]);
      if (v) dump_to(out, *v);
      else out += "null";
    }
    out += "]}";
  }

  std::string query(const std::string& query_json, const std::string& prefix, bool sort_keys = false) {
    Value q = parse(query_json.empty() ? std::string("{}") : query_json);
    if (q.t != Value::Object) throw QueryError("query must be a JSON object");
    Filter f;
    if (auto* fv = q.get_ci("filter")) f = compile_filter(*fv);
    std::vector<SortKey> sort;
    if (auto* sv = q.get_ci("sort")) {
      if (sv->t != Value::Array) throw QueryError("sort must be an array");
      for (auto& s : sv->items) {
        const Value* k = s.get_ci("key");
        if (!k || k->t != Value::String) throw QueryError("sort entry needs a string key");
        SortKey sk{k->s, false};
        if (auto* o = s.get_ci("order")) sk.desc = o->t == Value::String && ieq(o->s, "DESC");
        sort.push_back(sk);
      }
    }
    size_t limit = 0, offset = 0;
    if (auto* pv = q.get_ci("page")) {
      if (auto* l = pv->get_ci("limit")) limit = l->t == Value::Number && l->n > 0 ? (size_t)l->n : 0;
      if (auto* t = pv->get_ci("token")) {
        if (t->t == Value::String && !t->s.empty()) offset = (size_t)std::strtoull(t->s.c_str(), nullptr, 10);
      }
    }

    std::lock_guard<std::mutex> g(mu_);
    int64_t now = now_ms();
    ensure_indexes(f);
    std::vector<std::pair<const std::string*, const Doc*>> hits;
    auto consider = [&](const std::string& key, const Doc& d) {
      if (!prefix.empty() && key.compare(0, prefix.size(), prefix) != 0) return;
      if (expired(d, now)) return;
      if (!eval_filter(f, d.parsed)) return;
      hits.emplace_back(&key, &d);
    };
    std::unordered_set<std::string> cand;
    if (candidates(f, cand)) {
      ++stats_indexed_queries_;
      for (auto& k : cand) {
        auto it = docs_.find(k);
        if (it != docs_.end()) consider(it->first, it->second);
      }
    } else {
      ++stats_scan_queries_;
      for (auto& [k, d] : docs_) consider(k, d);
    }
    if (sort.empty()) {
      std::sort(hits.begin(), hits.end(), [](auto& a, auto& b) { return a.second->seq < b.second->seq; });
    } else {
      static const Value kNull;
      std::stable_sort(hits.begin(), hits.end(), [&](auto& a, auto& b) {
        for (auto& sk : sort) {
          const Value* x = a.second->parsed.path(sk.path);
          const Value* y = b.second->parsed.path(sk.path);
          int c = compare(x ? *x : kNull, y ? *y : kNull);
          if (c) return sk.desc ? c > 0 : c < 0;
        }
        return a.second->seq < b.second->seq;
      });
    }
    size_t begin = std::min(offset, hits.size());
    size_t end = limit ? std::min(hits.size(), begin + limit) : hits.size();
    std::string out = "{\"results\":[";
    std::vector<std::string> sort_paths;
    if (sort_keys)
      for (auto& sk : sort) sort_paths.push_back(sk.path);
    for (size_t i = begin; i < end; ++i) {
      if (i > begin) out += ',';
      if (sort_keys) {
        sort_keys_to(out, std::string_view(*hits[i].first).substr(prefix.size()), *hits[i].second, sort_paths);
        continue;
      }
      out += "{\"key\":";
      escape_to(out, std::string_view(*hits[i].first).substr(prefix.size()));
      out += ",\"data\":";
      out += hits[i].second->value;
      out += ",\"etag\":\"";
      out += std::to_string(hits[i].second->etag);
      out += "\"}";
    }
    out += "]";
    if (limit && end < hits.size()) {
      out += ",\"token\":\"" + std::to_string(end) + "\"";
    }
    out += "}";
    return out;
  }

  std::vector<std::string> keys(const std::string& prefix, size_t limit) {
    std::lock_guard<std::mutex> g(mu_);
    std::vector<std::pair<uint64_t, std::string>> ks;
    int64_t now = now_ms();
    for (auto& [k, d] : docs_)
      if ((prefix.empty() || k.compare(0, prefix.size(), prefix) == 0) && !expired(d, now)) ks.emplace_back(d.seq, k);
    std::sort(ks.begin(), ks.end());
    std::vector<std::string> out;
    for (auto& p : ks) { if (limit && out.size() >= limit) break; out.push_back(p.second); }
    return out;
  }

  struct EncodedColumn {
    std::vector<std::string> values;
    std::vector<int32_t> ids;
  };
  struct Encoded {
    std::string key_blob;
    std::vector<int64_t> key_off;
    std::vector<int64_t> seqs;
    std::vector<EncodedColumn> cols;
  };
  Encoded encode_columns(const std::string& prefix, const std::vector<std::string>& paths) {
    std::lock_guard<std::mutex> g(mu_);
    int64_t now = now_ms();
    std::vector<std::pair<uint64_t, const std::pair<const std::string, Doc>*>> rows;
    rows.reserve(docs_.size());
    for (auto& kv : docs_)
      if ((prefix.empty() || kv.first.compare(0, prefix.size(), prefix) == 0) && !expired(kv.second, now))
        rows.emplace_back(kv.second.seq, &kv);
    std::sort(rows.begin(), rows.end(), [](auto& a, auto& b) { return a.first < b.first; });
    Encoded out;
    out.key_off.reserve(rows.size() + 1);
    out.seqs.reserve(rows.size());
    out.key_off.push_back(0);
    for (auto& r : rows) {
      out.key_blob += r.second->first;
      out.key_off.push_back((int64_t)out.key_blob.size());
      out.seqs.push_back((int64_t)r.first);
    }
    out.cols.resize(paths.size());
    auto encode_one = [&](size_t c) {
      const std::string& path = paths[c];
      EncodedColumn& col = out.cols[c];
      col.ids.resize(rows.size());
      std::unordered_map<std::string, int32_t> dict;
      std::string k;
      for (size_t i = 0; i < rows.size(); ++i) {
        const std::string& key = rows[i].second->first;
        const Value& doc = rows[i].second->second.parsed;
        Value tmp;
        const Value* v;
        if (path == std::string("\x00keyprefix", 10)) {
          size_t p = key.find("||");
          tmp = Value::string(p == std::string::npos ? std::string() : key.substr(0, p + 2));
          v = &tmp;
        } else if (path == std::string("\x00value", 6)) {
          v = doc.t == Value::Object ? nullptr : &doc;
        } else {
          v = doc.path(path);
        }
        if (!v) {
          col.ids[i] = -1;
          continue;
        }
        mirror_key(*v, k);
        auto it = dict.find(k);
        if (it == dict.end()) {
          it = dict.emplace(k, (int32_t)col.values.size()).first;
          col.values.push_back(dump(*v));
        }
        col.ids[i] = it->second;
      }
        };
    if (paths.size() <= 1 || rows.size() < 100000) {
      for (size_t c = 0; c < paths.size(); ++c) encode_one(c);
    } else {
      std::vector<std::thread> ts;
      for (size_t c = 0; c < paths.size(); ++c) ts.emplace_back(encode_one, c);
      for (auto& t : ts) t.join();
    }
    return out;
  }

  static double read_ru(size_t bytes) { return std::max<double>(1.0, std::ceil(bytes / 1024.0)); }
  static double write_ru(size_t bytes) { return 5.0 * std::max<double>(1.0, std::ceil(bytes / 1024.0)); }
  static double query_ru(size_t result_bytes) { return 2.5 + std::ceil(result_bytes / 1024.0); }

  void set_throughput(double ru_per_s, double ticket_ttl_s = kTicketTtlS) {
    std::lock_guard<std::mutex> g(ru_mu_);
    ru_ticket_ttl_s_ = ticket_ttl_s;
    ru_rate_ = std::max(0.0, ru_per_s);
    ru_on_.store(ru_rate_ > 0, std::memory_order_relaxed);
    ru_tokens_ = 0;
    ru_last_ = mono_s();
    ru_tickets_.clear();
    ru_by_slot_.clear();
    ru_by_bind_.clear();
  }

  static constexpr double kMaxReserveS = 25.0;
  static constexpr double kTicketTtlS = 10.0;
  enum Kind : int { kRead = 0, kWrite = 1, kQuery = 2, kDelete = 3 };

  int64_t charge(double ru) {
    uint64_t unused = 0;
    return charge(ru, 0, unused);
  }
  bool provisioned() const { return ru_on_.load(std::memory_order_relaxed); }

  static uint64_t bind_of(std::string_view a, std::string_view b = {}) {
    uint64_t h = 1469598103934665603ull;
    for (unsigned char c : a) h = (h ^ c) * 1099511628211ull;
    h = (h ^ 0xff) * 1099511628211ull;
    for (unsigned char c : b) h = (h ^ c) * 1099511628211ull;
    return h ? h : 1;
  }

  int64_t charge(double ru, uint64_t ticket, uint64_t& ticket_out, uint64_t bind = 0, int kind = kWrite) {
    std::lock_guard<std::mutex> g(ru_mu_);
    ticket_out = 0;
    if (ru_rate_ <= 0) {
      ru_consumed_ += ru;
      return 0;
    }
    double now = mono_s();
    ru_tokens_ = std::min(ru_rate_, ru_tokens_ + (now - ru_last_) * ru_rate_);
    ru_last_ = now;
    lapse(now);
    auto own = ru_tickets_.end();
    if (ticket) {
      own = ru_tickets_.find(ticket);
      if (own != ru_tickets_.end() && bind && own->second.bind != bind) own = ru_tickets_.end();
    }
    if (own == ru_tickets_.end() && bind) {
      auto range = ru_by_bind_.equal_range(bind);
      for (auto it = range.first; it != range.second; ++it) {
        auto t = ru_tickets_.find(it->second);
        if (t != ru_tickets_.end() && (own == ru_tickets_.end() || t->second.slot < own->second.slot)) own = t;
      }
    }
    if (own != ru_tickets_.end()) {
      if (now + 5e-4 >= own->second.slot) {
        ru_consumed_ += own->second.ru;
        ++ru_reserved_admits_;
        drop(own);
        return 0;
      }
      ticket_out = own->first;
      ++ru_throttled_;
      ++ru_early_retries_;
      return std::max<int64_t>(1, (int64_t)std::ceil((own->second.slot - now) * 1000.0));
    }
    ru = std::min(ru, ru_rate_);
    ++ru_calls_;
    if (ru_tokens_ >= ru) {
      ru_tokens_ -= ru;
      ru_consumed_ += ru;
      return 0;
    }
    ++ru_throttled_;
    ++ru_throttled_kind_[kind & 3];
    double wait = (ru - ru_tokens_) / ru_rate_;
    if (wait > kMaxReserveS) return std::max<int64_t>(1, (int64_t)std::ceil(wait * 1000.0));
    ru_tokens_ -= ru;
    do ticket_out = next_ticket();
    while (ru_tickets_.count(ticket_out));
    Reservation res{now + wait, ru, bind};
    ru_tickets_.emplace(ticket_out, res);
    ru_by_slot_.emplace(res.slot, ticket_out);
    if (bind) ru_by_bind_.emplace(bind, ticket_out);
    return std::max<int64_t>(1, (int64_t)std::ceil(wait * 1000.0));
  }

  void debit(double ru) {
    std::lock_guard<std::mutex> g(ru_mu_);
    ru_consumed_ += ru;
    if (ru_rate_ <= 0) return;
    double now = mono_s();
    ru_tokens_ = std::min(ru_rate_, ru_tokens_ + (now - ru_last_) * ru_rate_) - ru;
    ru_last_ = now;
  }

  std::unordered_map<std::string, double> throughput_stats() {
    std::lock_guard<std::mutex> g(ru_mu_);
    return {{"ru_per_s", ru_rate_}, {"ru_consumed", ru_consumed_}, {"throttled", (double)ru_throttled_},
            {"reserved_admits", (double)ru_reserved_admits_}, {"open_reservations", (double)ru_tickets_.size()},
            {"calls", (double)ru_calls_}, {"early_retries", (double)ru_early_retries_},
            {"lapsed_reservations", (double)ru_lapsed_}, {"refunded_ru", ru_refunded_},
            {"throttled_read", (double)ru_throttled_kind_[kRead]}, {"throttled_write", (double)ru_throttled_kind_[kWrite]},
            {"throttled_query", (double)ru_throttled_kind_[kQuery]},
            {"throttled_delete", (double)ru_throttled_kind_[kDelete]},
            {"mono", mono_s()}};
  }

  bool mirror_enable(const std::vector<std::string>& paths) {
    std::lock_guard<std::mutex> g(mu_);
    if (mirror_.disabled) return false;
    std::vector<std::string> add;
    for (auto& p : paths) {
      bool have = false;
      for (auto& c : mirror_.cols) have = have || c.path == p;
      for (auto& a : add) have = have || a == p;
      if (!have) add.push_back(p);
    }
    if (mirror_.on && add.empty()) return true;
    if (!mirror_.on) {
      for (auto& [k, d] : docs_)
        if (d.expire_ms) { mirror_.disabled = true; return false; }
      mirror_.on = true;
      mirror_.cols.clear();
      for (auto& p : add) { mirror_.cols.emplace_back(); mirror_.cols.back().path = p; }
      mirror_rebuild_rows();
    } else {
      size_t first = mirror_.cols.size();
      for (auto& p : add) { mirror_.cols.emplace_back(); mirror_.cols.back().path = p; }
      auto enc = [&](size_t c) {
        MirrorColumn& col = mirror_.cols[c];
        col.ids.assign(mirror_.nodes.size(), -1);
        std::string k;
        for (size_t r = 0; r < mirror_.nodes.size(); ++r) {
          if (!mirror_.live[r]) continue;
          auto& kv = *mirror_.nodes[r];
          col.ids[r] = mirror_encode(col, kv.first, kv.second.parsed, k);
        }
      };
      parallel_for_columns(first, mirror_.cols.size(), enc);
      ++mirror_.gen;
      mirror_.kills.clear();
    }
    return true;
  }

  MirrorDelta mirror_delta(uint64_t gen, size_t from, size_t kill_from, const std::vector<size_t>& dict_sizes) {
    std::lock_guard<std::mutex> g(mu_);
    MirrorDelta d;
    d.gen = mirror_.gen;
    d.on = mirror_.on;
    d.disabled = mirror_.disabled;
    if (!mirror_.on) return d;
    size_t n = mirror_.nodes.size();
    d.full = gen != mirror_.gen || dict_sizes.size() != mirror_.cols.size() || from > n ||
             kill_from > mirror_.kills.size();
    if (d.full) from = 0, kill_from = mirror_.kills.size();
    d.n = n;
    d.from = from;
    d.kill_cursor = mirror_.kills.size();
    for (size_t i = kill_from; i < mirror_.kills.size(); ++i)
      if (mirror_.kills[i] < from) d.kills.push_back(mirror_.kills[i]);
    d.seqs.assign(mirror_.seqs.begin() + from, mirror_.seqs.end());
    d.live.assign(mirror_.live.begin() + from, mirror_.live.end());
    for (size_t c = 0; c < mirror_.cols.size(); ++c) {
      auto& col = mirror_.cols[c];
      size_t df = d.full ? 0 : std::min(dict_sizes[c], col.values.size());
      d.paths.push_back(col.path);
      d.dict_from.push_back(df);
      d.new_values.emplace_back(col.values.begin() + df, col.values.end());
      d.ids.emplace_back(col.ids.begin() + from, col.ids.end());
    }
    return d;
  }

  bool mirror_results(const int32_t* rows, size_t nrows, const std::string& prefix, const std::string& token,
                      uint64_t gen, std::string& out, size_t* skipped = nullptr,
                      const std::vector<std::string>* sort_paths = nullptr) {
    std::lock_guard<std::mutex> g(mu_);
    if (gen != mirror_.gen) return false;
    int64_t now = now_ms();
    out.clear();
    if (!sort_paths && !docs_.empty()) out.reserve(32 + token.size() + nrows * (live_bytes_ / docs_.size() + 48));
    out += "{\"results\":[";
    size_t skip = 0;
    bool first = true;
    for (size_t i = 0; i < nrows; ++i) {
      uint32_t r = (uint32_t)rows[i];
      if (r >= mirror_.nodes.size() || !mirror_.live[r]) { ++skip; continue; }
      auto* it = mirror_.nodes[r];
      const std::string& key = it->first;
      if (it->second.mrow != r || expired(it->second, now)) { ++skip; continue; }
      if (!first) out += ',';
      first = false;
      if (sort_paths) {
        sort_keys_to(out, std::string_view(key).substr(std::min(prefix.size(), key.size())), it->second, *sort_paths);
        continue;
      }
      out += "{\"key\":";
      escape_to(out, std::string_view(key).substr(std::min(prefix.size(), key.size())));
      out += ",\"data\":";
      out += it->second.value;
      out += ",\"etag\":\"";
      out += std::to_string(it->second.etag);
      out += "\"}";
    }
    out += "]";
    if (!token.empty()) out += ",\"token\":\"" + token + "\"";
    out += "}";
    if (skipped) *skipped = skip;
    return true;
  }

  std::unordered_map<std::string, uint64_t> mirror_stats() {
    std::lock_guard<std::mutex> g(mu_);
    return {{"on", mirror_.on}, {"disabled", mirror_.disabled}, {"gen", mirror_.gen},
            {"rows", mirror_.nodes.size()}, {"live_rows", mirror_.live_rows}, {"columns", mirror_.cols.size()},
            {"compactions", mirror_.compactions}};
  }

  size_t size() {
    std::lock_guard<std::mutex> g(mu_);
    return docs_.size();
  }

  void compact() {
    std::lock_guard<std::mutex> g(mu_);
    compact_locked();
  }

  void sync() { std::lock_guard<std::mutex> g(mu_); log_.sync(); }
  bool group_commit() const { return log_.group(); }
  uint64_t log_mark() const { return log_.mark(); }
  void after_durable(uint64_t mark, std::function<void()> cb) { log_.after_durable(mark, std::move(cb)); }
  void wait_durable() { log_.wait_durable(); }
  AppLog::CommitStats commit_stats() { return log_.commit_stats(); }

  std::unordered_map<std::string, uint64_t> stats() {
    std::lock_guard<std::mutex> g(mu_);
    return {{"docs", docs_.size()}, {"live_bytes", live_bytes_}, {"log_bytes", log_.bytes()},
            {"indexes", indexes_.size()}, {"indexed_queries", stats_indexed_queries_},
            {"scan_queries", stats_scan_queries_}, {"etag", etag_}};
  }

  std::vector<std::string> indexed_paths() {
    std::lock_guard<std::mutex> g(mu_);
    std::vector<std::string> out;
    for (auto& [p, _] : indexes_) out.push_back(p);
    std::sort(out.begin(), out.end());
    return out;
  }

 private:
  using Index = std::unordered_map<std::string, std::unordered_set<std::string>>;
  using Docs = ShardedMap<Doc>;

  static bool expired(const Doc& d, int64_t now) { return d.expire_ms && d.expire_ms <= now; }

  void check_etag(const std::string& key, const std::optional<std::string>& etag, bool first_write, int64_t now) {
    check_etag_at(docs_.find(key), etag, first_write, now);
  }

  void check_etag_at(Docs::iterator it, const std::optional<std::string>& etag,
                     bool first_write, int64_t now) {
    bool exists = it != docs_.end() && !expired(it->second, now);
    if (etag && !etag->empty()) {
      if (!exists || *etag != std::to_string(it->second.etag)) throw EtagMismatch("possible etag mismatch");
    } else if (first_write && exists) {
      throw EtagMismatch("possible etag mismatch: first-write on existing key without etag");
    }
  }

  uint64_t put(const std::string& key, const std::string& value, Value parsed, int64_t expire_ms) {
    return put_at(docs_.find(key), key, std::string(value), std::move(parsed), expire_ms, nullptr)->second.etag;
  }

  static bool same_scalar(const Value* a, const Value* b) {
    if (!a || !b) return a == b;
    if (a->t != b->t) return false;
    switch (a->t) {
      case Value::Null: return true;
      case Value::Bool: return a->b == b->b;
      case Value::Number: return std::memcmp(&a->n, &b->n, sizeof(double)) == 0;
      case Value::String: return a->s == b->s;
      default: return false;
    }
  }

  Docs::iterator put_at(Docs::iterator it,
                                                       const std::string& key, std::string&& value, Value parsed,
                                                       int64_t expire_ms, std::vector<Doc>* graveyard) {
    uint64_t e = ++etag_;
    if (expire_ms && mirror_.on) mirror_disable();
    int32_t* reuse = nullptr;
    if (it == docs_.end()) {
      Doc d;
      live_bytes_ += key.size() + value.size();
      d.value = std::move(value);
      d.parsed = std::move(parsed);
      d.etag = e;
      d.seq = ++seq_;
      d.expire_ms = expire_ms;
      index_add(key, d.parsed);
      it = docs_.emplace(key, std::move(d)).first;
    } else {
      Doc& d = it->second;
      index_update(key, d.parsed, parsed);
      if (mirror_.on && d.mrow < mirror_.live.size() && mirror_.live[d.mrow]) {
        reuse_.resize(mirror_.cols.size());
        for (size_t c = 0; c < mirror_.cols.size(); ++c)
          reuse_[c] = same_column_value(mirror_.cols[c], d.parsed, parsed) ? mirror_.cols[c].ids[d.mrow] : kEncode;
        reuse = reuse_.data();
      }
      live_bytes_ += value.size();
      live_bytes_ -= d.value.size();
      if (graveyard) {
        graveyard->emplace_back();
        graveyard->back().value.swap(d.value);
        graveyard->back().parsed = std::move(d.parsed);
      }
      d.value = std::move(value);
      d.parsed = std::move(parsed);
      d.etag = e;
      d.expire_ms = expire_ms;
      mirror_kill(d);
    }
    if (mirror_.on) mirror_append(*it, reuse);
    return it;
  }

  void erase_locked(const std::string& key, bool log) {
    auto it = docs_.find(key);
    if (it == docs_.end()) return;
    index_remove(key, it->second.parsed);
    mirror_kill(it->second);
    live_bytes_ -= key.size() + it->second.value.size();
    docs_.erase(it);
    if (log) log_.append('D', {key});
  }

  void log_put(const std::string& key, const std::string& value, uint64_t etag, int64_t expire) {
    if (!log_.is_open()) return;
    log_.append('P', {key, value, AppLog::pod(etag), AppLog::pod(expire)});
  }

  void apply_log(char kind, std::vector<std::string_view>& f) {
    if (kind == 'P' && f.size() == 4) {
      std::string key(f[0]), value(f[1]);
      uint64_t e;
      int64_t exp;
      std::memcpy(&e, f[2].data(), 8);
      std::memcpy(&exp, f[3].data(), 8);
      Value parsed;
      try { parsed = parse(value); } catch (...) { return; }
      put(key, value, std::move(parsed), exp);
      docs_[key].etag = e;
      etag_ = std::max(etag_, e);
    } else if (kind == 'D' && f.size() == 1) {
      erase_locked(std::string(f[0]), false);
    }
  }

  void maybe_compact() {
    if (!log_.is_open()) return;
    uint64_t live = live_bytes_ + docs_.size() * 40;
    if (log_.bytes() > (1u << 20) && log_.bytes() > 4 * live) compact_locked();
  }

  void compact_locked() {
    if (!log_.is_open()) return;
    std::vector<std::pair<uint64_t, const std::pair<const std::string, Doc>*>> rows;
    for (auto& kv : docs_) rows.emplace_back(kv.second.seq, &kv);
    std::sort(rows.begin(), rows.end(), [](auto& a, auto& b) { return a.first < b.first; });
    log_.rewrite([&](AppLog& out) {
      for (auto& r : rows)
        out.append('P', {r.second->first, r.second->second.value, AppLog::pod(r.second->second.etag),
                         AppLog::pod(r.second->second.expire_ms)});
    });
  }

  template <class F>
  void parallel_for_columns(size_t lo, size_t hi, F&& f) {
    if (hi - lo <= 1 || mirror_.nodes.size() < 100000) {
      for (size_t c = lo; c < hi; ++c) f(c);
      return;
    }
    std::vector<std::thread> ts;
    for (size_t c = lo; c < hi; ++c) ts.emplace_back(f, c);
    for (auto& t : ts) t.join();
  }

  static int32_t mirror_encode(MirrorColumn& col, const std::string& key, const Value& doc, std::string& k) {
    static const std::string kPrefix("\x00keyprefix", 10), kValue("\x00value", 6);
    Value tmp;
    const Value* v;
    if (col.path == kPrefix) {
      size_t p = key.find("||");
      tmp = Value::string(p == std::string::npos ? std::string() : key.substr(0, p + 2));
      v = &tmp;
    } else if (col.path == kValue) {
      v = doc.t == Value::Object ? nullptr : &doc;
    } else {
      v = doc.path(col.path);
    }
    if (!v) return -1;
    mirror_key(*v, k);
    auto it = col.dict.find(k);
    if (it == col.dict.end()) {
      it = col.dict.emplace(k, (int32_t)col.values.size()).first;
      col.values.push_back(dump(*v));
    }
    return it->second;
  }

  static bool same_column_value(const MirrorColumn& col, const Value& before, const Value& after) {
    static const std::string kPrefix("\x00keyprefix", 10), kValue("\x00value", 6);
    if (col.path == kPrefix) return true;
    if (col.path == kValue)
      return before.t != Value::Object && after.t != Value::Object && same_scalar(&before, &after);
    return same_scalar(before.path(col.path), after.path(col.path));
  }

  void mirror_append(std::pair<const std::string, Doc>& kv, const int32_t* reuse = nullptr) {
    uint32_t r = (uint32_t)mirror_.nodes.size();
    mirror_.nodes.push_back(&kv);
    mirror_.seqs.push_back((int64_t)kv.second.seq);
    mirror_.live.push_back(1);
    std::string k;
    for (size_t c = 0; c < mirror_.cols.size(); ++c) {
      MirrorColumn& col = mirror_.cols[c];
      col.ids.push_back(reuse && reuse[c] != kEncode ? reuse[c] : mirror_encode(col, kv.first, kv.second.parsed, k));
    }
    kv.second.mrow = r;
    ++mirror_.live_rows;
    if (mirror_.nodes.size() > 65536 && mirror_.nodes.size() > 2 * mirror_.live_rows) mirror_compact();
  }

  void mirror_kill(Doc& d) {
    if (d.mrow == UINT32_MAX) return;
    if (mirror_.on && d.mrow < mirror_.live.size() && mirror_.live[d.mrow]) {
      mirror_.live[d.mrow] = 0;
      mirror_.kills.push_back(d.mrow);
      --mirror_.live_rows;
    }
    d.mrow = UINT32_MAX;
  }

  void mirror_disable() {
    for (auto& kv : docs_) kv.second.mrow = UINT32_MAX;
    uint64_t gen = mirror_.gen;
    mirror_ = ColumnMirror{};
    mirror_.gen = gen + 1;
    mirror_.disabled = true;
  }

  void mirror_rebuild_rows() {
    std::vector<std::pair<uint64_t, std::pair<const std::string, Doc>*>> rows;
    rows.reserve(docs_.size());
    for (auto& kv : docs_) rows.emplace_back(kv.second.seq, &kv);
    std::sort(rows.begin(), rows.end(), [](auto& a, auto& b) { return a.first < b.first; });
    mirror_.nodes.clear();
    mirror_.seqs.clear();
    mirror_.kills.clear();
    mirror_.nodes.reserve(rows.size());
    for (auto& r : rows) {
      r.second->second.mrow = (uint32_t)mirror_.nodes.size();
      mirror_.nodes.push_back(r.second);
      mirror_.seqs.push_back((int64_t)r.first);
    }
    mirror_.live.assign(rows.size(), 1);
    mirror_.live_rows = rows.size();
    auto enc = [&](size_t c) {
      MirrorColumn& col = mirror_.cols[c];
      col.ids.resize(rows.size());
      std::string k;
      for (size_t i = 0; i < rows.size(); ++i)
        col.ids[i] = mirror_encode(col, rows[i].second->first, rows[i].second->second.parsed, k);
    };
    parallel_for_columns(0, mirror_.cols.size(), enc);
    ++mirror_.gen;
  }

  void mirror_compact() {
    size_t w = 0, n = mirror_.nodes.size();
    for (size_t r = 0; r < n; ++r) {
      if (!mirror_.live[r]) continue;
      if (w != r) {
        mirror_.nodes[w] = mirror_.nodes[r];
        mirror_.seqs[w] = mirror_.seqs[r];
        for (auto& col : mirror_.cols) col.ids[w] = col.ids[r];
        mirror_.nodes[w]->second.mrow = (uint32_t)w;
      }
      ++w;
    }
    mirror_.nodes.resize(w);
    mirror_.seqs.resize(w);
    for (auto& col : mirror_.cols) col.ids.resize(w);
    mirror_.live.assign(w, 1);
    mirror_.live_rows = w;
    mirror_.kills.clear();
    ++mirror_.gen;
    ++mirror_.compactions;
  }

  void collect_eq_paths(const Filter& f, std::vector<std::string>& out) {
    if (f.op == Filter::EQ || f.op == Filter::IN) out.push_back(f.path);
    for (auto& k : f.kids) collect_eq_paths(k, out);
  }

  void ensure_indexes(const Filter& f) {
    if (docs_.size() < index_threshold_) return;
    std::vector<std::string> paths;
    collect_eq_paths(f, paths);
    for (auto& p : paths) {
      if (indexes_.count(p)) continue;
      Index& idx = indexes_[p];
      for (auto& [k, d] : docs_) {
        const Value* v = d.parsed.path(p);
        if (v && v->t != Value::Array && v->t != Value::Object) idx[index_key(*v)].insert(k);
      }
    }
  }

  void index_add(const std::string& key, const Value& doc) {
    for (auto& [p, idx] : indexes_) {
      const Value* v = doc.path(p);
      if (v && v->t != Value::Array && v->t != Value::Object) idx[index_key(*v)].insert(key);
    }
  }

  void index_update(const std::string& key, const Value& before, const Value& after) {
    for (auto& [p, idx] : indexes_) {
      const Value* a = before.path(p);
      const Value* b = after.path(p);
      if (same_scalar(a, b)) continue;
      if (a && a->t != Value::Array && a->t != Value::Object) {
        auto it = idx.find(index_key(*a));
        if (it != idx.end()) {
          it->second.erase(key);
          if (it->second.empty()) idx.erase(it);
        }
      }
      if (b && b->t != Value::Array && b->t != Value::Object) idx[index_key(*b)].insert(key);
    }
  }

  void index_remove(const std::string& key, const Value& doc) {
    for (auto& [p, idx] : indexes_) {
      const Value* v = doc.path(p);
      if (!v || v->t == Value::Array || v->t == Value::Object) continue;
      auto it = idx.find(index_key(*v));
      if (it != idx.end()) {
        it->second.erase(key);
        if (it->second.empty()) idx.erase(it);
      }
    }
  }

  bool candidates(const Filter& f, std::unordered_set<std::string>& out) {
    switch (f.op) {
      case Filter::EQ: {
        auto ix = indexes_.find(f.path);
        if (ix == indexes_.end() || f.val.t == Value::Array || f.val.t == Value::Object) return false;
        auto it = ix->second.find(index_key(f.val));
        if (it != ix->second.end()) out.insert(it->second.begin(), it->second.end());
        return true;
      }
      case Filter::IN: {
        auto ix = indexes_.find(f.path);
        if (ix == indexes_.end()) return false;
        for (auto& v : f.vals) {
          if (v.t == Value::Array || v.t == Value::Object) return false;
          auto it = ix->second.find(index_key(v));
          if (it != ix->second.end()) out.insert(it->second.begin(), it->second.end());
        }
        return true;
      }
      case Filter::AND: {
        bool any = false;
        std::unordered_set<std::string> best;
        for (auto& k : f.kids) {
          std::unordered_set<std::string> c;
          if (candidates(k, c) && (!any || c.size() < best.size())) { best.swap(c); any = true; }
        }
        if (any) out.insert(best.begin(), best.end());
        return any;
      }
      case Filter::OR: {
        std::unordered_set<std::string> acc;
        for (auto& k : f.kids)
          if (!candidates(k, acc)) return false;
        out.insert(acc.begin(), acc.end());
        return true;
      }
      default: return false;
    }
  }

  std::mutex mu_;
  Docs docs_;
  std::unordered_map<std::string, Index> indexes_;
  AppLog log_;
  uint64_t etag_ = 0;
  uint64_t seq_ = 0;
  uint64_t live_bytes_ = 0;
  uint64_t stats_indexed_queries_ = 0;
  uint64_t stats_scan_queries_ = 0;
  size_t index_threshold_;
  ColumnMirror mirror_;
  static constexpr int32_t kEncode = INT32_MIN;
  std::vector<int32_t> reuse_;
  std::mutex ru_mu_;
  std::atomic<bool> ru_on_{false};
  double ru_rate_ = 0, ru_tokens_ = 0, ru_last_ = 0, ru_consumed_ = 0;
  uint64_t ru_throttled_ = 0, ru_reserved_admits_ = 0, ru_calls_ = 0, ru_early_retries_ = 0, ru_lapsed_ = 0;
  uint64_t ru_throttled_kind_[4] = {0, 0, 0, 0};
  double ru_refunded_ = 0;
  double ru_ticket_ttl_s_ = kTicketTtlS;
  struct Reservation {
    double slot, ru;
    uint64_t bind;
  };
  std::unordered_map<uint64_t, Reservation> ru_tickets_;
  std::multimap<double, uint64_t> ru_by_slot_;
  std::unordered_multimap<uint64_t, uint64_t> ru_by_bind_;
  uint64_t ru_rng_[2] = {0, 0};
  uint64_t next_ticket() {
    if ((ru_rng_[0] | ru_rng_[1]) == 0) {
      if (getrandom(ru_rng_, sizeof ru_rng_, 0) != (ssize_t)sizeof ru_rng_ || (ru_rng_[0] | ru_rng_[1]) == 0)
        ru_rng_[0] = 0x9e3779b97f4a7c15ull ^ (uint64_t)(mono_s() * 1e9);
    }
    uint64_t a = ru_rng_[0];
    const uint64_t b = ru_rng_[1];
    ru_rng_[0] = b;
    a ^= a << 23;
    ru_rng_[1] = a ^ b ^ (a >> 17) ^ (b >> 26);
    uint64_t v = (ru_rng_[1] + b) >> 1;
    return v ? v : 1;
  }
  void drop(std::unordered_map<uint64_t, Reservation>::iterator it) {
    auto range = ru_by_slot_.equal_range(it->second.slot);
    for (auto s = range.first; s != range.second; ++s)
      if (s->second == it->first) {
        ru_by_slot_.erase(s);
        break;
      }
    if (it->second.bind) {
      auto b = ru_by_bind_.equal_range(it->second.bind);
      for (auto x = b.first; x != b.second; ++x)
        if (x->second == it->first) {
          ru_by_bind_.erase(x);
          break;
        }
    }
    ru_tickets_.erase(it);
  }
  void lapse(double now) {
    while (!ru_by_slot_.empty() && ru_by_slot_.begin()->first + ru_ticket_ttl_s_ < now) {
      auto t = ru_tickets_.find(ru_by_slot_.begin()->second);
      if (t == ru_tickets_.end()) {
        ru_by_slot_.erase(ru_by_slot_.begin());
        continue;
      }
      ru_tokens_ = std::min(ru_rate_, ru_tokens_ + t->second.ru);
      ru_refunded_ += t->second.ru;
      ++ru_lapsed_;
      drop(t);
    }
  }
  static double mono_s() {
    return std::chrono::duration<double>(std::chrono::steady_clock::now().time_since_epoch()).count();
  }
};

}
```

aca_dotnet_workshop_amd/native/src/module.cpp:

```cpp
#include <unistd.h>

#include <pybind11/pybind11.h>
#include <pybind11/numpy.h>
#include <pybind11/stl.h>

#include "apphost.hpp"
#include "daprpb.hpp"
#include "backingfront.hpp"
#include "broker.hpp"
#include "cpuscan.hpp"
#include "docstore.hpp"
#include "dutycycle.hpp"
#include "httpparse.hpp"
#include "taskcodec.hpp"
#include "sweepcodec.hpp"
#include "pcsample.hpp"
#include "formcodec.hpp"
#include "strrank.hpp"

namespace py = pybind11;
using namespace tt;

template <class List>
static py::dict headers_dict(const List& headers) {
  py::dict hd;
  for (auto& [k, v] : headers) {
    py::str key(k);
    if (hd.contains(key)) {
      if (k == "set-cookie") {
        py::object prev = hd[key];
        py::list l;
        if (py::isinstance<py::list>(prev)) l = prev.cast<py::list>();
        else l.append(prev);
        l.append(py::str(v));
        hd[key] = l;
      } else {
        hd[key] = py::str(hd[key].cast<std::string>() + ", " + v);
      }
    } else {
      hd[key] = py::str(v);
    }
  }
  return hd;
}

static ev::HeaderList header_list(const py::handle& seq) {
  ev::HeaderList out;
  for (auto item : seq) {
    auto t = item.cast<py::tuple>();
    std::string k = t[0].cast<std::string>();
    for (auto& ch : k) ch = (char)std::tolower((unsigned char)ch);
    out.emplace_back(std::move(k), py::str(t[1]).cast<std::string>());
  }
  return out;
}

static std::string_view utf8_view(PyObject* o) {
  Py_ssize_t n;
  const char* p = PyUnicode_AsUTF8AndSize(o, &n);
  if (p == nullptr) throw py::error_already_set();
  return std::string_view(p, (size_t)n);
}

static std::string str_of(PyObject* o) {
  if (PyUnicode_Check(o)) return std::string(utf8_view(o));
  py::object s = py::reinterpret_steal<py::object>(PyObject_Str(o));
  if (!s) throw py::error_already_set();
  return std::string(utf8_view(s.ptr()));
}

static std::string_view need_str(PyObject* o, const char* what) {
  if (!PyUnicode_Check(o)) throw py::type_error(std::string(what) + " must be a str");
  return utf8_view(o);
}

static long long need_int(PyObject* o, const char* what) {
  long long v = PyLong_AsLongLong(o);
  if (v == -1 && PyErr_Occurred()) {
    PyErr_Clear();
    throw py::type_error(std::string(what) + " must be an int");
  }
  return v;
}

static py::object seq_fast(PyObject* o, const char* what) {
  py::object f = py::reinterpret_steal<py::object>(PySequence_Fast(o, what));
  if (!f) throw py::error_already_set();
  return f;
}

static ev::HeaderList header_list_fast(PyObject* seq) {
  py::object f = seq_fast(seq, "headers must be a sequence of (name, value)");
  Py_ssize_t n = PySequence_Fast_GET_SIZE(f.ptr());
  PyObject** items = PySequence_Fast_ITEMS(f.ptr());
  ev::HeaderList out;
  out.reserve((size_t)n);
  for (Py_ssize_t i = 0; i < n; ++i) {
    py::object kv = seq_fast(items[i], "a header must be a (name, value) pair");
    if (PySequence_Fast_GET_SIZE(kv.ptr()) != 2) throw py::value_error("a header must be a (name, value) pair");
    PyObject** p = PySequence_Fast_ITEMS(kv.ptr());
    std::string k(need_str(p[0], "header name"));
    for (auto& ch : k) ch = (char)std::tolower((unsigned char)ch);
    out.emplace_back(std::move(k), str_of(p[1]));
  }
  return out;
}

static std::string body_of(PyObject* o) {
  char* p;
  Py_ssize_t n;
  if (PyBytes_AsStringAndSize(o, &p, &n) != 0) throw py::error_already_set();
  return std::string(p, (size_t)n);
}

static void set_item(PyObject* tup, Py_ssize_t i, PyObject* v) {
  if (v == nullptr) throw py::error_already_set();
  PyTuple_SET_ITEM(tup, i, v);
}

static PyObject* new_str(const std::string& s) { return PyUnicode_DecodeUTF8(s.data(), (Py_ssize_t)s.size(), "replace"); }

static PyObject* headers_dict_fast(const ev::HeaderList& headers) {
  py::object d = py::reinterpret_steal<py::object>(PyDict_New());
  if (!d) throw py::error_already_set();
  for (auto& [k, v] : headers) {
    py::object key = py::reinterpret_steal<py::object>(new_str(k));
    py::object val = py::reinterpret_steal<py::object>(new_str(v));
    if (!key || !val) throw py::error_already_set();
    PyObject* prev = PyDict_GetItemWithError(d.ptr(), key.ptr());
    if (prev == nullptr && PyErr_Occurred()) throw py::error_already_set();
    if (prev == nullptr) {
      if (PyDict_SetItem(d.ptr(), key.ptr(), val.ptr()) != 0) throw py::error_already_set();
    } else if (k == "set-cookie") {
      if (PyList_Check(prev)) {
        if (PyList_Append(prev, val.ptr()) != 0) throw py::error_already_set();
      } else {
        py::object l = py::reinterpret_steal<py::object>(PyList_New(2));
        if (!l) throw py::error_already_set();
        Py_INCREF(prev);
        PyList_SET_ITEM(l.ptr(), 0, prev);
        PyList_SET_ITEM(l.ptr(), 1, val.release().ptr());
        if (PyDict_SetItem(d.ptr(), key.ptr(), l.ptr()) != 0) throw py::error_already_set();
      }
    } else {
      std::string joined = str_of(prev) + ", " + v;
      py::object j = py::reinterpret_steal<py::object>(new_str(joined));
      if (!j || PyDict_SetItem(d.ptr(), key.ptr(), j.ptr()) != 0) throw py::error_already_set();
    }
  }
  return d.release().ptr();
}

static py::list events_to_py(std::vector<apphost::Event>& evs, bool with_times) {
  struct Item {
    long batch = -1;
    size_t ev = 0;
  };
  std::vector<Item> items;
  items.reserve(evs.size());
  std::vector<std::pair<std::pair<int, std::string>, std::string>> batches;
  for (size_t i = 0; i < evs.size(); ++i) {
    auto& e = evs[i];
    if (e.kind != apphost::Event::LOG || e.line.empty() || with_times) {
      items.push_back({-1, i});
      continue;
    }
    auto key = std::make_pair(e.err, e.msg.method);
    if (!items.empty() && items.back().batch >= 0 && batches[(size_t)items.back().batch].first == key) {
      batches[(size_t)items.back().batch].second += e.line;
      continue;
    }
    batches.emplace_back(key, e.line);
    items.push_back({(long)batches.size() - 1, 0});
  }
  py::list out(items.size());
  for (size_t ki = 0; ki < items.size(); ++ki) {
    if (items[ki].batch < 0) continue;
    auto& b = batches[(size_t)items[ki].batch];
    py::object t = py::reinterpret_steal<py::object>(PyTuple_New(4));
    if (!t) throw py::error_already_set();
    set_item(t.ptr(), 0, PyLong_FromLong(4));
    set_item(t.ptr(), 1, PyLong_FromLong(b.first.first));
    set_item(t.ptr(), 2, new_str(b.first.second));
    set_item(t.ptr(), 3, new_str(b.second));
    PyList_SET_ITEM(out.ptr(), (Py_ssize_t)ki, t.release().ptr());
  }
  for (size_t ki = 0; ki < items.size(); ++ki) {
    if (items[ki].batch >= 0) continue;
    auto& e = evs[items[ki].ev];
    py::object t;
    if (e.kind == apphost::Event::REQUEST) {
      t = py::reinterpret_steal<py::object>(PyTuple_New(with_times ? 9 : 8));
      if (!t) throw py::error_already_set();
      set_item(t.ptr(), 0, PyLong_FromLong(0));
      set_item(t.ptr(), 1, PyLong_FromUnsignedLongLong(e.id));
      set_item(t.ptr(), 2, PyLong_FromLong(e.server));
      set_item(t.ptr(), 3, new_str(e.msg.method));
      set_item(t.ptr(), 4, new_str(e.msg.target));
      set_item(t.ptr(), 5, PyBool_FromLong(e.msg.http10));
      set_item(t.ptr(), 6, headers_dict_fast(e.msg.headers));
      set_item(t.ptr(), 7, PyBytes_FromStringAndSize(e.msg.body.data(), (Py_ssize_t)e.msg.body.size()));
      if (with_times) set_item(t.ptr(), 8, PyFloat_FromDouble(e.t));
    } else if (e.kind == apphost::Event::RESPONSE) {
      t = py::reinterpret_steal<py::object>(PyTuple_New(with_times ? 6 : 5));
      if (!t) throw py::error_already_set();
      set_item(t.ptr(), 0, PyLong_FromLong(1));
      set_item(t.ptr(), 1, PyLong_FromUnsignedLongLong(e.id));
      set_item(t.ptr(), 2, PyLong_FromLong(e.msg.status));
      set_item(t.ptr(), 3, headers_dict_fast(e.msg.headers));
      set_item(t.ptr(), 4, PyBytes_FromStringAndSize(e.msg.body.data(), (Py_ssize_t)e.msg.body.size()));
      if (with_times) set_item(t.ptr(), 5, PyFloat_FromDouble(e.t));
    } else if (e.kind == apphost::Event::LOG) {
      t = py::reinterpret_steal<py::object>(PyTuple_New(with_times ? 8 : 7));
      if (!t) throw py::error_already_set();
      set_item(t.ptr(), 0, PyLong_FromLong(3));
      set_item(t.ptr(), 1, PyLong_FromLong(e.err));
      set_item(t.ptr(), 2, new_str(e.msg.method));
      set_item(t.ptr(), 3, new_str(e.msg.body));
      set_item(t.ptr(), 4, new_str(e.msg.target));
      set_item(t.ptr(), 5, new_str(e.msg.reason));
      set_item(t.ptr(), 6, new_str(e.line));
      if (with_times) set_item(t.ptr(), 7, PyFloat_FromDouble(e.t));
    } else {
      if (with_times) t = py::make_tuple(2, e.id, e.err, py::str(std::strerror(e.err)), e.t);
      else t = py::make_tuple(2, e.id, e.err, py::str(std::strerror(e.err)));
    }
    PyList_SET_ITEM(out.ptr(), (Py_ssize_t)ki, t.release().ptr());
  }
  return out;
}

static std::string bytes_of(const py::handle& b) {
  char* p;
  Py_ssize_t n;
  if (PyBytes_AsStringAndSize(b.ptr(), &p, &n) != 0) throw py::error_already_set();
  return std::string(p, (size_t)n);
}

PYBIND11_MODULE(_ttnative, m) {
  m.def("sharded_map_growth", [](size_t n) {
    tt::ShardedMap<int32_t> map;
    constexpr size_t S = tt::ShardedMap<int32_t>::shards();
    std::vector<size_t> bkt(S);
    for (size_t s = 0; s < S; ++s) bkt[s] = map.bucket_count(s);
    std::vector<std::pair<size_t, size_t>> out;
    uint64_t x = 0x9e3779b97f4a7c15ull;
    char key[37];
    for (size_t i = 0; i < n; ++i) {
      x ^= x << 13, x ^= x >> 7, x ^= x << 17;
      uint64_t y = x * 0x2545f4914f6cdd1dull;
      std::snprintf(key, sizeof key, "%08x-%04x-4%03x-a%03x-%012llx", (unsigned)(x >> 32), (unsigned)(x >> 16) & 0xffff,
                    (unsigned)x & 0xfff, (unsigned)(y >> 52), (unsigned long long)(y & 0xffffffffffffull));
      map[key] = (int32_t)i;
      size_t grown = 0;
      for (size_t s = 0; s < S; ++s)
        if (map.bucket_count(s) != bkt[s]) bkt[s] = map.bucket_count(s), ++grown;
      if (grown) out.emplace_back(i, grown);
    }
    return out;
  }, py::call_guard<py::gil_scoped_release>());
  m.def("pc_sample_start", [] { tt::pcsample::start(); });
  m.def("pc_sample_dump", [](const std::string& who) { tt::pcsample::dump(who.c_str()); },
        py::call_guard<py::gil_scoped_release>());
  m.doc() = "Native document store + message broker engines (C++17)";

  static py::exception<EtagMismatch> etag_exc(m, "EtagMismatch");
  py::register_exception_translator([](std::exception_ptr p) {
    try {
      if (p) std::rethrow_exception(p);
    } catch (const EtagMismatch& e) {
      PyErr_SetString(etag_exc.ptr(), e.what());
    } catch (const QueryError& e) {
      PyErr_SetString(PyExc_ValueError, e.what());
    } catch (const ParseError& e) {
      PyErr_SetString(PyExc_ValueError, (std::string("invalid JSON: ") + e.what()).c_str());
    }
  });

  m.def("schedstat_ns", [](const std::vector<int>& fds) {
    std::vector<long long> out(fds.size(), -1);
    {
      py::gil_scoped_release r;
      char buf[128];
      for (size_t i = 0; i < fds.size(); ++i) {
        ssize_t n = ::pread(fds[i], buf, sizeof buf - 1, 0);
        if (n <= 0) continue;
        buf[n] = 0;
        char* end = nullptr;
        long long v = std::strtoll(buf, &end, 10);
        if (end != buf) out[i] = v;
      }
    }
    return out;
  });
  m.def("bulk_values", [](py::bytes body) -> py::object {
    std::string b = body;
    std::vector<std::string> vals;
    if (!scan_bulk_values(b, vals)) return py::none();
    py::list l(vals.size());
    for (size_t i = 0; i < vals.size(); ++i) l[i] = py::str(vals[i]);
    return l;
  });

  m.def("tx_values", [](py::bytes body) -> py::object {
    std::string b = body;
    std::vector<std::string> vals;
    if (!scan_tx_values(b, vals)) return py::none();
    py::list l(vals.size());
    for (size_t i = 0; i < vals.size(); ++i) l[i] = py::str(vals[i]);
    return l;
  });

  py::class_<DutyCycle>(m, "DutyCycle")
      .def(py::init<double>(), py::arg("period_s"))
      .def("add", &DutyCycle::add, py::arg("name"), py::arg("pid"), py::arg("cpu"),
           py::call_guard<py::gil_scoped_release>())
      .def("remove", &DutyCycle::remove, py::arg("name"), py::call_guard<py::gil_scoped_release>())
      .def("start", &DutyCycle::start)
      .def("stop", &DutyCycle::stop, py::call_guard<py::gil_scoped_release>())
      .def_property_readonly("period_s", &DutyCycle::period_s)
      .def("stats", [](DutyCycle& d) {
        std::map<std::string, DutyCycle::Stats> st;
        {
          py::gil_scoped_release r;
          st = d.stats();
        }
        py::dict out;
        for (auto& kv : st) {
          py::dict x;
          x["throttled_periods"] = kv.second.throttled_periods;
          x["cpu_seconds"] = kv.second.cpu_seconds;
          x["stopped_seconds"] = kv.second.stopped_seconds;
          x["stopped"] = kv.second.stopped;
          out[py::str(kv.first)] = x;
        }
        return out;
      });
  m.def("parse_http_head", [](py::bytes raw) {
    std::string_view sv = raw;
    HttpHead h;
    try {
      h = parse_head(sv);
    } catch (const std::invalid_argument& e) {
      throw py::value_error(e.what());
    }
    return py::make_tuple(py::str(h.a), py::str(h.b), py::str(h.c), headers_dict(h.headers));
  });

  m.def("task_create", [](py::bytes body) -> py::object {
    static taskcodec::Entropy rng;
    static taskcodec::Created c;
    char* p;
    Py_ssize_t n;
    if (PyBytes_AsStringAndSize(body.ptr(), &p, &n) != 0) throw py::error_already_set();
    if (!taskcodec::create(std::string_view(p, (size_t)n), rng, c)) return py::none();
    return py::make_tuple(py::str(c.id), py::str(c.name), py::str(c.assigned_to),
                          py::bytes(c.task_json), py::bytes(c.state_body));
  });

  m.def("cloudevent_unwrap", [](py::bytes body) -> py::object {
    static taskcodec::Unwrapped u;
    char* p;
    Py_ssize_t n;
    if (PyBytes_AsStringAndSize(body.ptr(), &p, &n) != 0) throw py::error_already_set();
    if (!taskcodec::unwrap_cloudevent(std::string_view(p, (size_t)n), u)) return py::none();
    py::dict attrs;
    for (const auto& kv : u.attrs) {
      const tt::Value& v = *kv.second;
      py::object o;
      if (v.t == tt::Value::String) o = py::str(v.s);
      else if (v.t == tt::Value::Bool) o = py::bool_(v.b);
      else if (v.t == tt::Value::Null) o = py::none();
      else o = py::module_::import("json").attr("loads")(py::str(tt::dump(v)));
      attrs[py::str(kv.first)] = o;
    }
    return py::make_tuple(py::bytes(u.data), py::str(u.content_type), attrs);
  });

  m.def("tasks_mark_overdue", [](py::bytes body) -> py::object {
    char* p;
    Py_ssize_t n;
    if (PyBytes_AsStringAndSize(body.ptr(), &p, &n) != 0) throw py::error_already_set();
    std::vector<std::string> ids;
    std::string bulk;
    if (!taskcodec::mark_overdue(std::string_view(p, (size_t)n), ids, bulk)) return py::none();
    py::list l(ids.size());
    for (size_t i = 0; i < ids.size(); ++i) l[i] = py::str(ids[i]);
    return py::make_tuple(l, py::bytes(bulk));
  });

  auto view = [](const py::bytes& b) {
    char* p;
    Py_ssize_t n;
    if (PyBytes_AsStringAndSize(b.ptr(), &p, &n) != 0) throw py::error_already_set();
    return std::string_view(p, (size_t)n);
  };
  m.def("dapr_pb_save_state_bulk", [view](const std::string& store, py::bytes body) -> py::object {
    std::string out;
    if (!tt::daprpb::save_state_bulk(store, view(body), out)) return py::none();
    return py::bytes(out);
  });
  m.def("dapr_pb_get_bulk_state", [](const std::string& store, const std::vector<std::string>& keys, int parallelism) {
    return py::bytes(tt::daprpb::get_bulk_state(store, keys, parallelism));
  });
  m.def("dapr_pb_bulk_state_json", [view](py::bytes msg) -> py::object {
    std::string out;
    if (!tt::daprpb::bulk_state_response_json(view(msg), out)) return py::none();
    return py::bytes(out);
  });
  m.def("dapr_pb_query_from_json", [view](py::bytes body) -> py::object {
    std::string out;
    if (!tt::daprpb::query_response_pb(view(body), out)) return py::none();
    return py::bytes(out);
  });
  m.def("tasks_from_query_pb", [view](py::bytes msg, bool by_created, bool descending) -> py::object {
    std::string out;
    size_t count = 0;
    bool more = false;
    if (!taskcodec::query_pb_tasks(view(msg), out, count, by_created, &more, descending)) return py::none();
    return py::make_tuple(count, py::bytes(out), more);
  });
  m.def("tasks_conditional_mark_pb", [view](py::bytes msg, const std::string& store) -> py::object {
    std::string save;
    std::vector<std::string> ids;
    size_t skipped = 0;
    if (!taskcodec::conditional_mark_pb(view(msg), store, save, ids, skipped)) return py::none();
    return py::make_tuple(py::bytes(save), ids, skipped);
  });
  m.def("tasks_mark_overdue_ids", [view](py::bytes body) -> py::object {
    std::vector<std::string> ids;
    if (!taskcodec::mark_overdue_ids(view(body), ids)) return py::none();
    return py::cast(ids);
  });
  m.def("dapr_pb_query_json", [view](py::bytes msg) -> py::object {
    std::string out;
    if (!tt::daprpb::query_response_json(view(msg), out)) return py::none();
    return py::bytes(out);
  });

  m.def("task_update_bind", [view](py::bytes body) -> py::object {
    taskcodec::Update u;
    if (!taskcodec::bind_update(view(body), u)) return py::none();
    return py::make_tuple(py::str(u.name), py::str(u.assigned_to), py::str(u.due));
  });
  m.def("task_edit", [view](py::bytes stored, bool complete, py::object update) -> py::object {
    taskcodec::Update u;
    const taskcodec::Update* up = nullptr;
    if (!update.is_none()) {
      auto t = update.cast<py::tuple>();
      u.name = t[0].cast<std::string>();
      u.assigned_to = t[1].cast<std::string>();
      u.due = t[2].cast<std::string>();
      up = &u;
    }
    std::string out, id, old;
    if (!taskcodec::edit_task(view(stored), up, complete, out, id, old)) return py::none();
    return py::make_tuple(py::bytes(out), py::str(id), py::str(old));
  });
  m.def("task_json", [view](py::bytes stored) -> py::object {
    std::string out;
    if (!taskcodec::task_json(view(stored), out)) return py::none();
    return py::bytes(out);
  });
  m.def("ascii_ieq", [](const std::string& a, const std::string& b) -> py::object {
    int r = taskcodec::ascii_ieq(a, b);
    if (r < 0) return py::none();
    return py::bool_(r == 1);
  });

  m.def("tasks_conditional_mark", [](py::bytes got) -> py::object {
    char* p;
    Py_ssize_t n;
    if (PyBytes_AsStringAndSize(got.ptr(), &p, &n) != 0) throw py::error_already_set();
    std::vector<std::string> ids;
    std::string bulk;
    size_t skipped = 0;
    if (!taskcodec::conditional_mark(std::string_view(p, (size_t)n), bulk, ids, skipped)) return py::none();
    py::list l(ids.size());
    for (size_t i = 0; i < ids.size(); ++i) l[i] = py::str(ids[i]);
    return py::make_tuple(l, py::bytes(bulk), skipped);
  });

  m.def("tasks_overdue_filter", [](py::bytes body, const std::string& run_day) -> py::object {
    char* p;
    Py_ssize_t n;
    if (PyBytes_AsStringAndSize(body.ptr(), &p, &n) != 0) throw py::error_already_set();
    size_t retrieved = 0, kept = 0;
    std::string out;
    if (!taskcodec::overdue_filter(std::string_view(p, (size_t)n), run_day, retrieved, kept, out)) return py::none();
    return py::make_tuple(retrieved, kept, py::bytes(out));
  });

  m.def("tasks_overdue_filter_chunks", [](py::bytes body, const std::string& run_day, size_t chunk) -> py::object {
    char* p;
    Py_ssize_t n;
    if (PyBytes_AsStringAndSize(body.ptr(), &p, &n) != 0) throw py::error_already_set();
    if (chunk == 0) return py::none();
    size_t retrieved = 0, kept = 0;
    std::string out;
    std::vector<size_t> starts;
    if (!taskcodec::overdue_filter(std::string_view(p, (size_t)n), run_day, retrieved, kept, out, &starts))
      return py::none();
    py::list parts;
    const size_t body_end = out.size() - 1;
    for (size_t a = 0; a < starts.size(); a += chunk) {
      const size_t b = std::min(starts.size(), a + chunk);
      const size_t from = starts[a], to = b < starts.size() ? starts[b] - 1 : body_end;
      std::string part;
      part.reserve(to - from + 2);
      part += '[';
      part.append(out, from, to - from);
      part += ']';
      parts.append(py::bytes(part));
    }
    return py::make_tuple(retrieved, kept, parts);
  });

  m.def("frontend_create_form", [](py::bytes body, py::bytes cookie, py::bytes key) -> py::object {
    char *pb, *pc, *pk;
    Py_ssize_t nb, nc, nk;
    if (PyBytes_AsStringAndSize(body.ptr(), &pb, &nb) != 0 || PyBytes_AsStringAndSize(cookie.ptr(), &pc, &nc) != 0 ||
        PyBytes_AsStringAndSize(key.ptr(), &pk, &nk) != 0)
      throw py::error_already_set();
    std::string json;
    auto v = formcodec::create_task(std::string_view(pb, (size_t)nb), std::string_view(pc, (size_t)nc),
                                    std::string_view(pk, (size_t)nk), ".AspNetCore.Antiforgery", "TasksCreatedByCookie",
                                    json);
    if (v == formcodec::Verdict::kDecline) return py::none();
    if (v == formcodec::Verdict::kBadToken) return py::make_tuple(false, py::bytes(""));
    return py::make_tuple(true, py::bytes(json));
  });

  m.def("frontend_edit_form", [view](py::bytes body, py::bytes cookie, py::bytes key, const std::string& path_id)
            -> py::object {
    std::string json, id;
    auto v = formcodec::edit_task(view(body), view(cookie), view(key), ".AspNetCore.Antiforgery", path_id, json, id);
    if (v == formcodec::Verdict::kDecline) return py::none();
    if (v == formcodec::Verdict::kBadToken) return py::make_tuple(false, py::bytes(""), py::str(""));
    return py::make_tuple(true, py::bytes(json), py::str(id));
  });
  m.def("frontend_index_form", [view](py::bytes body, py::bytes cookie, py::bytes key) -> py::object {
    auto v = formcodec::index_post(view(body), view(cookie), view(key), ".AspNetCore.Antiforgery");
    if (v == formcodec::Verdict::kDecline) return py::none();
    return py::bool_(v == formcodec::Verdict::kOk);
  });

  m.def("tasks_from_query", [](py::bytes body, bool by_created, bool descending) -> py::object {
    char* p;
    Py_ssize_t n;
    if (PyBytes_AsStringAndSize(body.ptr(), &p, &n) != 0) throw py::error_already_set();
    std::string out;
    size_t count = 0;
    bool more = false;
    if (!taskcodec::query_tasks(std::string_view(p, (size_t)n), out, count, by_created, &more, descending))
      return py::none();
    return py::make_tuple(count, py::bytes(out), more);
  }, py::arg("body"), py::arg("by_created") = false, py::arg("descending") = false);
  m.def("tasks_query_in_store_layout", [](py::bytes body) {
    std::string_view b = body.cast<std::string_view>();
    std::string buf;
    std::vector<taskcodec::TaskRow> rows;
    bool token = false;
    return taskcodec::valid_utf8(b) && taskcodec::fast_query_tasks(b, buf, rows, token);
  });

  m.def("json_array_chunks", [](py::bytes body, long n) -> py::object {
    char* pb;
    Py_ssize_t nb;
    if (PyBytes_AsStringAndSize(body.ptr(), &pb, &nb) != 0) throw py::error_already_set();
    std::string_view s(pb, (size_t)nb);
    if (n < 1 || !tt::valid(s)) return py::none();
    const char* p = tt::ws_end(s.data(), s.data() + s.size());
    const char* e = s.data() + s.size();
    if (p >= e || *p != '[') return py::none();
    ++p;
    py::list out;
    std::string cur = "[";
    long in_cur = 0;
    while (true) {
      p = tt::ws_end(p, e);
      if (p < e && *p == ']') break;
      const char* vs = p;
      p = tt::skip_value(p, e);
      if (in_cur) cur += ',';
      cur.append(vs, (size_t)(p - vs));
      if (++in_cur == n) {
        cur += ']';
        out.append(py::bytes(cur));
        cur = "[";
        in_cur = 0;
      }
      p = tt::ws_end(p, e);
      if (p < e && *p == ',') ++p;
    }
    if (in_cur) {
      cur += ']';
      out.append(py::bytes(cur));
    }
    return out;
  });

  m.def("task_model_name", [](py::bytes body) -> py::object {
    char* p;
    Py_ssize_t n;
    if (PyBytes_AsStringAndSize(body.ptr(), &p, &n) != 0) throw py::error_already_set();
    std::string name;
    if (!taskcodec::task_model_name(std::string_view(p, (size_t)n), name)) return py::none();
    return py::str(name);
  });

  m.def("scan_select",
        [](py::list columns, py::array_t<uint16_t, py::array::c_style> live, int64_t nrows,
           py::array_t<int32_t, py::array::c_style> code, py::array_t<uint32_t, py::array::c_style> bitmaps,
           int threads, bool simd) {
          std::vector<cpuscan::Col> cols;
          std::vector<py::array> keep;
          const int64_t padded = (nrows + 63) / 64 * 64;
          for (auto item : columns) {
            auto t = item.cast<py::tuple>();
            py::array a = t[0].cast<py::array>();
            int w = t[1].cast<int>();
            if (w != 0 && w != 1 && w != 2 && w != 4) throw py::value_error("column width must be 0 (2 bits), 1, 2 or 4");
            if (!(a.flags() & py::array::c_style)) throw py::value_error("columns must be contiguous");
            if ((int64_t)a.nbytes() < (w == 0 ? padded / 4 : padded * w))
              throw py::value_error("column shorter than the padded row count");
            cols.push_back({static_cast<const uint8_t*>(a.data()), w});
            keep.push_back(a);
          }
          if ((int64_t)live.size() * 16 < padded) throw py::value_error("liveness shorter than the padded row count");
          if (code.ndim() != 2 || code.shape(1) != 4) throw py::value_error("code must be [L, 4]");
          cpuscan::Program pg;
          pg.code.assign(code.data(), code.data() + code.size());
          pg.bitmaps.assign(bitmaps.data(), bitmaps.data() + bitmaps.size());
          cpuscan::Selection sel(cols, live.data(), nrows, pg, std::max(1, threads), simd);
          int64_t total;
          {
            py::gil_scoped_release rel;
            total = sel.count();
          }
          int32_t* dst = static_cast<int32_t*>(cpuscan::huge_alloc((size_t)std::max<int64_t>(total, 1) * sizeof(int32_t)));
          py::capsule owner(dst, [](void* p) { std::free(p); });
          {
            py::gil_scoped_release rel;
            sel.write(dst);
          }
          return py::array_t<int32_t>({(py::ssize_t)total}, {(py::ssize_t)sizeof(int32_t)}, dst, owner);
        },
        py::arg("columns"), py::arg("live"), py::arg("nrows"), py::arg("code"), py::arg("bitmaps"), py::arg("threads"),
        py::arg("simd") = true);

  py::class_<TxOp>(m, "TxOp")
      .def(py::init([](bool is_delete, std::string key, std::string value, std::optional<std::string> etag,
                       bool first_write, int64_t ttl_ms) {
             TxOp op;
             op.is_delete = is_delete;
             op.key = std::move(key);
             op.value = std::move(value);
             op.etag = std::move(etag);
             op.first_write = first_write;
             op.ttl_ms = ttl_ms;
             return op;
           }),
           py::arg("is_delete"), py::arg("key"), py::arg("value") = "", py::arg("etag") = std::nullopt,
           py::arg("first_write") = false, py::arg("ttl_ms") = 0)
      .def_readonly("is_delete", &TxOp::is_delete)
      .def_readonly("key", &TxOp::key)
      .def_readonly("value", &TxOp::value)
      .def_readonly("ttl_ms", &TxOp::ttl_ms);

  py::class_<StrRanker>(m, "StrRanker")
      .def(py::init<>())
      .def_property_readonly("size", &StrRanker::size)
      .def(
          "extend",
          [](StrRanker& r, py::list values, py::array_t<int64_t, py::array::c_style> ranks) -> int64_t {
            const size_t n0 = r.size(), n = (size_t)PyList_GET_SIZE(values.ptr());
            if (n < n0) return -1;
            if ((size_t)ranks.size() < n || !ranks.writeable()) throw std::invalid_argument("rank buffer too small");
            std::vector<std::string_view> vs;
            vs.reserve(n - n0);
            for (size_t i = n0; i < n; ++i) {
              PyObject* o = PyList_GET_ITEM(values.ptr(), (Py_ssize_t)i);
              if (!PyUnicode_Check(o)) return -1;
              Py_ssize_t len = 0;
              const char* p = PyUnicode_AsUTF8AndSize(o, &len);
              if (!p) {
                PyErr_Clear();
                return -1;
              }
              vs.emplace_back(p, (size_t)len);
            }
            int64_t* out = ranks.mutable_data();
            return (int64_t)r.extend(vs.size(), [&](size_t i) { return vs[i]; }, out);
          },
          py::arg("values"), py::arg("ranks"));

  py::class_<DocStore>(m, "DocStore")
      .def(py::init<const std::string&, int, size_t>(), py::arg("path") = "", py::arg("fsync_mode") = 0,
           py::arg("index_threshold") = 256)
      .def("set",
           [](DocStore& s, const std::string& key, const std::string& value, const std::optional<std::string>& etag,
              bool first_write, int64_t ttl_ms) {
             std::string e = s.set(key, value, etag, first_write, ttl_ms);
             s.wait_durable();
             return e;
           },
           py::arg("key"), py::arg("value"), py::arg("etag") = std::nullopt, py::arg("first_write") = false,
           py::arg("ttl_ms") = 0, py::call_guard<py::gil_scoped_release>())
      .def("get", &DocStore::get, py::arg("key"))
      .def("delete",
           [](DocStore& s, const std::string& key, const std::optional<std::string>& etag) {
             bool ok = s.del(key, etag);
             s.wait_durable();
             return ok;
           },
           py::arg("key"), py::arg("etag") = std::nullopt, py::call_guard<py::gil_scoped_release>())
      .def("transact",
           [](DocStore& s, const std::vector<TxOp>& ops) {
             s.transact(ops);
             s.wait_durable();
           },
           py::arg("ops"), py::call_guard<py::gil_scoped_release>())
      .def("group_commit", &DocStore::group_commit)
      .def("wait_durable", &DocStore::wait_durable, py::call_guard<py::gil_scoped_release>())
      .def("commit_stats",
           [](DocStore& s) {
             auto c = s.commit_stats();
             py::dict d;
             d["syncs"] = c.syncs;
             d["acks"] = c.acks;
             d["written_bytes"] = c.written;
             d["synced_bytes"] = c.synced;
             d["sync_ms_total"] = c.sync_ms_total;
             d["sync_ms_max"] = c.sync_ms_max;
             return d;
           })
      .def("query", &DocStore::query, py::arg("query"), py::arg("prefix") = "", py::arg("sort_keys") = false,
           py::call_guard<py::gil_scoped_release>())
      .def("keys", &DocStore::keys, py::arg("prefix") = "", py::arg("limit") = 0)
      .def("encode_columns",
           [](DocStore& s, const std::string& prefix, const std::vector<std::string>& paths) {
             DocStore::Encoded e;
             {
               py::gil_scoped_release r;
               e = s.encode_columns(prefix, paths);
             }
             py::list cols;
             for (auto& c : e.cols) {
               py::array_t<int32_t> ids((py::ssize_t)c.ids.size());
               std::memcpy(ids.mutable_data(), c.ids.data(), c.ids.size() * sizeof(int32_t));
               cols.append(py::make_tuple(py::cast(c.values), ids));
             }
             py::array_t<int64_t> seqs((py::ssize_t)e.seqs.size());
             std::memcpy(seqs.mutable_data(), e.seqs.data(), e.seqs.size() * sizeof(int64_t));
             py::array_t<int64_t> offs((py::ssize_t)e.key_off.size());
             std::memcpy(offs.mutable_data(), e.key_off.data(), e.key_off.size() * sizeof(int64_t));
             return py::make_tuple(py::make_tuple(py::bytes(e.key_blob), offs), seqs, cols);
           },
           py::arg("prefix"), py::arg("paths"))
      .def("mirror_enable", &DocStore::mirror_enable, py::arg("paths"), py::call_guard<py::gil_scoped_release>())
      .def("mirror_delta",
           [](DocStore& s, uint64_t gen, size_t from, size_t kill_from, const std::vector<size_t>& dict_sizes) {
             MirrorDelta d;
             {
               py::gil_scoped_release r;
               d = s.mirror_delta(gen, from, kill_from, dict_sizes);
             }
             auto arr = [](const auto& v) {
               using T = typename std::decay_t<decltype(v)>::value_type;
               py::array_t<T> a((py::ssize_t)v.size());
               if (!v.empty()) std::memcpy(a.mutable_data(), v.data(), v.size() * sizeof(T));
               return a;
             };
             py::list cols;
             for (size_t c = 0; c < d.paths.size(); ++c) {
               const auto& nv = d.new_values[c];
               const bool all_str =
                   std::all_of(nv.begin(), nv.end(), [](const std::string& v) { return !v.empty() && v[0] == '"'; });
               cols.append(py::make_tuple(d.paths[c], d.dict_from[c], py::cast(nv), arr(d.ids[c]), all_str));
             }
             py::dict out;
             out["gen"] = d.gen;
             out["on"] = d.on;
             out["disabled"] = d.disabled;
             out["full"] = d.full;
             out["n"] = d.n;
             out["from"] = d.from;
             out["kill_cursor"] = d.kill_cursor;
             out["kills"] = arr(d.kills);
             out["seqs"] = arr(d.seqs);
             out["live"] = arr(d.live);
             out["columns"] = cols;
             return out;
           },
           py::arg("gen"), py::arg("from_row"), py::arg("kill_from"), py::arg("dict_sizes"))
      .def("mirror_results",
           [](DocStore& s, py::array_t<int32_t, py::array::c_style | py::array::forcecast> rows,
              const std::string& prefix, const std::string& token, uint64_t gen,
              std::optional<std::vector<std::string>> sort_paths) -> py::object {
             size_t skipped = 0;
             std::string out;
             const int32_t* p = rows.data();
             size_t n = (size_t)rows.size();
             bool ok;
             {
               py::gil_scoped_release r;
               ok = s.mirror_results(p, n, prefix, token, gen, out, &skipped, sort_paths ? &*sort_paths : nullptr);
             }
             if (!ok) return py::none();
             return py::make_tuple(py::bytes(out), skipped);
           },
           py::arg("rows"), py::arg("prefix") = "", py::arg("token") = "", py::arg("gen") = 0,
           py::arg("sort_paths") = py::none())
      .def("mirror_stats", &DocStore::mirror_stats)
      .def("set_throughput", &DocStore::set_throughput, py::arg("ru_per_s"), py::arg("ticket_ttl_s") = DocStore::kTicketTtlS)
      .def("charge", [](DocStore& s, double ru, uint64_t ticket, std::string bind, int kind) {
             uint64_t out = 0;
             int64_t wait = s.charge(ru, ticket, out, bind.empty() ? 0 : DocStore::bind_of(bind), kind);
             return py::make_tuple(wait, out);
           }, py::arg("ru"), py::arg("ticket") = 0, py::arg("bind") = "", py::arg("kind") = (int)DocStore::kWrite,
           "(wait_ms, ticket): 0 = admitted; else a 429 whose ticket claims the reserved slot.  `bind`: the "
           "request's identity (method + target [+ query / bulk body]): a retry of the same request without "
           "the ticket claims its due reservation; `kind`: 0 read, 1 write, 2 query, 3 delete")
      .def("debit", &DocStore::debit, py::arg("ru"))
      .def("throughput_stats", &DocStore::throughput_stats)
      .def_static("read_ru", &DocStore::read_ru)
      .def_static("write_ru", &DocStore::write_ru)
      .def_static("query_ru", &DocStore::query_ru)
      .def("size", &DocStore::size)
      .def("__len__", &DocStore::size)
      .def("compact", &DocStore::compact)
      .def("sync", &DocStore::sync)
      .def("stats", &DocStore::stats)
      .def("indexed_paths", &DocStore::indexed_paths);

  py::class_<QueueOptions>(m, "QueueOptions")
      .def(py::init([](int64_t lock_ms, uint32_t max_delivery, int64_t default_ttl_ms, bool dead_letter_on_expiry) {
             QueueOptions o;
             o.lock_ms = lock_ms;
             o.max_delivery = max_delivery;
             o.default_ttl_ms = default_ttl_ms;
             o.dead_letter_on_expiry = dead_letter_on_expiry;
             return o;
           }),
           py::arg("lock_ms") = 60000, py::arg("max_delivery") = 10, py::arg("default_ttl_ms") = 0,
           py::arg("dead_letter_on_expiry") = false)
      .def_readwrite("lock_ms", &QueueOptions::lock_ms)
      .def_readwrite("max_delivery", &QueueOptions::max_delivery)
      .def_readwrite("default_ttl_ms", &QueueOptions::default_ttl_ms)
      .def_readwrite("dead_letter_on_expiry", &QueueOptions::dead_letter_on_expiry);

  py::class_<Received>(m, "Received")
      .def_readonly("lock_token", &Received::lock_token)
      .def_readonly("seq", &Received::seq)
      .def_readonly("id", &Received::id)
      .def_property_readonly("body", [](const Received& r) { return py::bytes(r.body); })
      .def_readonly("content_type", &Received::content_type)
      .def_readonly("props", &Received::props)
      .def_readonly("delivery_count", &Received::delivery_count)
      .def_readonly("enqueued_ms", &Received::enqueued_wall);

  py::class_<Broker>(m, "Broker")
      .def(py::init<const std::string&, int>(), py::arg("path") = "", py::arg("fsync_mode") = 0)
      .def("create_queue", &Broker::create_queue, py::arg("name"), py::arg("options") = QueueOptions())
      .def("create_topic", &Broker::create_topic)
      .def("create_subscription", &Broker::create_subscription, py::arg("topic"), py::arg("subscription"),
           py::arg("options") = QueueOptions())
      .def("delete_entity", &Broker::delete_entity)
      .def("subscriptions", &Broker::subscriptions)
      .def("entities", &Broker::entities)
      .def("publish",
           [](Broker& b, const std::string& topic, py::bytes body, const std::string& ctype, const std::string& props,
              const std::string& id, int64_t ttl_ms, int64_t delay_ms) {
             std::string s = body;
             py::gil_scoped_release r;
             uint64_t seq = b.publish(topic, s, ctype, props, id, ttl_ms, delay_ms);
             b.wait_durable();
             return seq;
           },
           py::arg("topic"), py::arg("body"), py::arg("content_type") = "application/json", py::arg("props") = "{}",
           py::arg("id") = "", py::arg("ttl_ms") = 0, py::arg("delay_ms") = 0)
      .def("send",
           [](Broker& b, const std::string& q, py::bytes body, const std::string& ctype, const std::string& props,
              const std::string& id, int64_t ttl_ms, int64_t delay_ms) {
             std::string s = body;
             py::gil_scoped_release r;
             uint64_t seq = b.send(q, s, ctype, props, id, ttl_ms, delay_ms);
             b.wait_durable();
             return seq;
           },
           py::arg("queue"), py::arg("body"), py::arg("content_type") = "application/json", py::arg("props") = "{}",
           py::arg("id") = "", py::arg("ttl_ms") = 0, py::arg("delay_ms") = 0)
      .def("receive", &Broker::receive, py::arg("path"), py::arg("max_messages") = 1, py::arg("lock_ms") = 0)
      .def("complete",
           [](Broker& b, const std::string& path, const std::string& token) {
             bool ok = b.complete(path, token);
             b.wait_durable();
             return ok;
           },
           py::call_guard<py::gil_scoped_release>())
      .def("abandon",
           [](Broker& b, const std::string& path, const std::string& token, int64_t delay_ms) {
             bool ok = b.abandon(path, token, delay_ms);
             b.wait_durable();
             return ok;
           },
           py::arg("path"), py::arg("token"), py::arg("delay_ms") = 0, py::call_guard<py::gil_scoped_release>())
      .def("dead_letter",
           [](Broker& b, const std::string& path, const std::string& token, const std::string& reason) {
             bool ok = b.dead_letter(path, token, reason);
             b.wait_durable();
             return ok;
           },
           py::arg("path"), py::arg("token"), py::arg("reason") = "", py::call_guard<py::gil_scoped_release>())
      .def("group_commit", &Broker::group_commit)
      .def("commit_stats",
           [](Broker& b) {
             auto c = b.commit_stats();
             py::dict d;
             d["syncs"] = c.syncs;
             d["acks"] = c.acks;
             d["written_bytes"] = c.written;
             d["synced_bytes"] = c.synced;
             d["sync_ms_total"] = c.sync_ms_total;
             d["sync_ms_max"] = c.sync_ms_max;
             return d;
           })
      .def("renew", &Broker::renew, py::arg("path"), py::arg("token"), py::arg("lock_ms") = 0)
      .def("drain_dead_letters",
           [](Broker& b, const std::string& path, size_t max) {
             py::list out;
             for (auto& [seq, id, body, reason, dc] : b.drain_dead_letters(path, max))
               out.append(py::make_tuple(seq, id, py::bytes(body), reason, dc));
             return out;
           },
           py::arg("path"), py::arg("max") = 100)
      .def("counts",
           [](Broker& b, const std::string& path) {
             auto [a, s, l, d, e, c, r] = b.counts(path);
             py::dict out;
             out["active"] = a;
             out["scheduled"] = s;
             out["locked"] = l;
             out["dead_letter"] = d;
             out["enqueued"] = e;
             out["completed"] = c;
             out["received"] = r;
             return out;
           })
      .def("purge", &Broker::purge)
      .def("total_published", &Broker::total_published);

  py::class_<BackingFront>(m, "BackingFront")
      .def(py::init<const std::string&, int, const std::string&, int, const std::string&>(), py::arg("host"),
           py::arg("port"), py::arg("fallback_uds"), py::arg("threads") = 1, py::arg("uds") = "")
      .def("port", &BackingFront::port)
      .def("threads", &BackingFront::threads)
      .def("attach_store",
           [](BackingFront& f, const std::string& a, const std::string& d, const std::string& c, DocStore& s) {
             f.attach_store(a, d, c, &s);
           },
           py::keep_alive<1, 5>())
      .def("attach_broker", [](BackingFront& f, const std::string& ns, Broker& b) { f.attach_broker(ns, &b); },
           py::keep_alive<1, 3>())
      .def("set_policy", &BackingFront::set_policy, py::arg("mode"), py::arg("keys"), py::arg("grants"))
      .def("set_query_fn",
           [](BackingFront& f, py::function fn) {
             std::shared_ptr<py::function> held(new py::function(std::move(fn)), [](py::function* p) {
               py::gil_scoped_acquire g;
               delete p;
             });
             f.set_query_fn([held](const BackingFront::QueryJob& j) {
               BackingFront::QueryResult out;
               py::gil_scoped_acquire g;
               py::object r = (*held)(j.account, j.db, j.coll, py::bytes(j.body), j.prefix, j.sort_keys, j.traceparent,
                                      j.sent_mono, j.front_mono);
               if (r.is_none()) return out;
               auto t = r.cast<py::tuple>();
               out.status = t[0].cast<int>();
               out.body = t[1].cast<std::string>();
               for (auto h : t[2]) {
                 auto kv = h.cast<py::tuple>();
                 out.headers.emplace_back(kv[0].cast<std::string>(), kv[1].cast<std::string>());
               }
               return out;
             });
           }, py::arg("fn"))
      .def("notify", &BackingFront::notify)
      .def("set_blob_root", &BackingFront::set_blob_root)
      .def("blob_note", &BackingFront::blob_note, py::arg("account"), py::arg("container"), py::arg("name"),
           py::arg("added"), py::call_guard<py::gil_scoped_release>())
      .def("blob_count", &BackingFront::blob_count, py::arg("account"), py::arg("container"), py::arg("prefix") = "",
           py::call_guard<py::gil_scoped_release>())
      .def("stats", &BackingFront::stats)
      .def("stop", &BackingFront::stop, py::call_guard<py::gil_scoped_release>());

  py::class_<apphost::AppHost>(m, "AppHost")
      .def(py::init<>())
      .def("start", &apphost::AppHost::start)
      .def("stop", &apphost::AppHost::stop, py::call_guard<py::gil_scoped_release>())
      .def("event_fd", &apphost::AppHost::event_fd)
      .def("listen", &apphost::AppHost::listen, py::arg("server"), py::arg("endpoint"), py::arg("cert") = "",
           py::arg("key") = "", py::call_guard<py::gil_scoped_release>())
      .def("close_server", &apphost::AppHost::close_server)
      .def("close_connections", &apphost::AppHost::close_connections)
      .def("pending_replies", &apphost::AppHost::pending_replies)
      .def("add_route", &apphost::AppHost::add_route, py::arg("server"), py::arg("kind"), py::arg("cfg"),
           py::arg("bounds"), py::call_guard<py::gil_scoped_release>())
      .def("route_stats", [](apphost::AppHost& h) {
        auto st = h.take_route_stats();
        py::list out;
        for (auto& x : st) out.append(py::make_tuple(x.route, x.status, x.n, x.sum, x.buckets));
        return out;
      })
      .def("submit",
           [](apphost::AppHost& h, py::list ops) {
             std::vector<apphost::AppHost::Op> v;
             Py_ssize_t n = PyList_GET_SIZE(ops.ptr());
             v.reserve((size_t)n);
             for (Py_ssize_t i = 0; i < n; ++i) {
               py::object t = seq_fast(PyList_GET_ITEM(ops.ptr(), i), "an operation must be a tuple");
               Py_ssize_t len = PySequence_Fast_GET_SIZE(t.ptr());
               PyObject** f = PySequence_Fast_ITEMS(t.ptr());
               if (len < 2) throw py::value_error("operation too short");
               apphost::AppHost::Op op;
               long long kind = need_int(f[0], "operation kind");
               op.is_request = kind == 1 || kind == 2;
               op.is_grpc = kind == 2;
               op.id = (uint64_t)need_int(f[1], "operation id");
               if (!op.is_request) {
                 if (len != 5) throw py::value_error("respond operation: (0, token, status, headers, body)");
                 op.status = (int)need_int(f[2], "status");
                 op.headers = header_list_fast(f[3]);
                 op.body = body_of(f[4]);
               } else {
                 if (len != 8) throw py::value_error("request operation: (1, id, endpoint, method, target, headers, body, timeout)");
                 op.endpoint = std::string(need_str(f[2], "endpoint"));
                 op.method = std::string(need_str(f[3], "method"));
                 op.target = std::string(need_str(f[4], "target"));
                 op.headers = header_list_fast(f[5]);
                 op.body = body_of(f[6]);
                 op.timeout_s = PyFloat_AsDouble(f[7]);
                 if (op.timeout_s == -1.0 && PyErr_Occurred()) throw py::error_already_set();
               }
               v.push_back(std::move(op));
             }
             h.submit(std::move(v));
           })
      .def("drain_times", [](apphost::AppHost& h) {
        auto evs = h.drain();
        return events_to_py(evs, true);
      })
      .def("drain", [](apphost::AppHost& h) {
        auto evs = h.drain();
        return events_to_py(evs, false);
      });
}
```

aca_dotnet_workshop_amd/native/src/textutil.hpp:

```cpp
#pragma once

#include <cctype>
#include <cstdint>
#include <string>
#include <string_view>

#include "json.hpp"

namespace tt::text {

inline int hexv(char c) {
  if (c >= '0' && c <= '9') return c - '0';
  if (c >= 'a' && c <= 'f') return c - 'a' + 10;
  if (c >= 'A' && c <= 'F') return c - 'A' + 10;
  return -1;
}

inline std::string unquote(std::string_view s, bool plus_space = false) {
  std::string o;
  o.reserve(s.size());
  for (size_t i = 0; i < s.size(); ++i) {
    if (s[i] == '%' && i + 2 < s.size() && hexv(s[i + 1]) >= 0 && hexv(s[i + 2]) >= 0) {
      o += (char)(hexv(s[i + 1]) * 16 + hexv(s[i + 2]));
      i += 2;
    } else if (plus_space && s[i] == '+') {
      o += ' ';
    } else {
      o += s[i];
    }
  }
  return o;
}

inline std::string quote_all(std::string_view s) {
  static const char* d = "0123456789ABCDEF";
  std::string o;
  for (unsigned char c : s) {
    if (std::isalnum(c) || c == '_' || c == '.' || c == '-' || c == '~') {
      o += (char)c;
    } else {
      o += '%';
      o += d[c >> 4];
      o += d[c & 15];
    }
  }
  return o;
}

inline std::string lower(std::string_view s) {
  std::string o(s);
  for (auto& c : o) c = (char)std::tolower((unsigned char)c);
  return o;
}

inline std::string json_str(std::string_view s) {
  std::string o;
  escape_to(o, s);
  return o;
}

inline bool valid_utf8(std::string_view s) {
  for (size_t i = 0; i < s.size();) {
    unsigned char c = (unsigned char)s[i];
    size_t n = c < 0x80 ? 0 : (c >> 5) == 6 ? 1 : (c >> 4) == 14 ? 2 : (c >> 3) == 30 ? 3 : 99;
    if (n == 99 || i + n >= s.size() + (n == 0)) return n == 0;
    for (size_t k = 1; k <= n; ++k)
      if (((unsigned char)s[i + k] >> 6) != 2) return false;
    i += n + 1;
  }
  return true;
}

inline std::string base64(std::string_view in) {
  static const char* t = "ABCDEFGHIJKLMNOPQRSTUVWXYZabcdefghijklmnopqrstuvwxyz0123456789+/";
  std::string o;
  size_t i = 0;
  for (; i + 2 < in.size(); i += 3) {
    uint32_t v = ((uint8_t)in[i] << 16) | ((uint8_t)in[i + 1] << 8) | (uint8_t)in[i + 2];
    o += t[v >> 18];
    o += t[(v >> 12) & 63];
    o += t[(v >> 6) & 63];
    o += t[v & 63];
  }
  if (i + 1 == in.size()) {
    uint32_t v = (uint8_t)in[i] << 16;
    o += t[v >> 18];
    o += t[(v >> 12) & 63];
    o += "==";
  } else if (i + 2 == in.size()) {
    uint32_t v = ((uint8_t)in[i] << 16) | ((uint8_t)in[i + 1] << 8);
    o += t[v >> 18];
    o += t[(v >> 12) & 63];
    o += t[(v >> 6) & 63];
    o += '=';
  }
  return o;
}

inline std::string unbase64(std::string_view in) {
  std::string o;
  uint32_t acc = 0;
  int bits = 0;
  for (char c : in) {
    int v = c >= 'A' && c <= 'Z' ? c - 'A' : c >= 'a' && c <= 'z' ? c - 'a' + 26 : c >= '0' && c <= '9' ? c - '0' + 52
            : c == '+' ? 62 : c == '/' ? 63 : -1;
    if (v < 0) continue;
    acc = (acc << 6) | (uint32_t)v;
    bits += 6;
    if (bits >= 8) {
      bits -= 8;
      o += (char)((acc >> bits) & 0xFF);
    }
  }
  return o;
}

}
```

Before: 90840.

## Cut per-request allocations in HTTP routing, auth scopes, log append and settle

Reuses thread-local scratch buffers for path segments and the query string, and builds auth scopes as concatenated string_view parts instead of allocating strings. Merges the collection lookup and the auth check under one shared lock, reuses static or thread-local header lists, and moves document bodies into the store. AppLog append now writes straight into reusable buffers, and a batched broker settle operation with its Python binding is added. Many unrelated micro-optimisations ship together, and the thread-local buffer reuse adds re-entrancy complexity.

```diff
diff --git a/aca_dotnet_workshop_amd/native/src/applog.hpp b/aca_dotnet_workshop_amd/native/src/applog.hpp
--- a/aca_dotnet_workshop_amd/native/src/applog.hpp
+++ b/aca_dotnet_workshop_amd/native/src/applog.hpp
@@ -17,6 +17,7 @@
 #include <exception>
 #include <functional>
 #include <future>
+#include <initializer_list>
 #include <map>
 #include <mutex>
 #include <stdexcept>
@@ -92,19 +93,22 @@
   template <class T>
   static std::string_view pod(const T& v) { return std::string_view(reinterpret_cast<const char*>(&v), sizeof(T)); }
 
-  void append(char kind, const std::vector<std::string_view>& fields) {
+  void append(char kind, std::initializer_list<std::string_view> fields) {
     if (fd_ < 0) return;
-    std::string rec;
-    rec.resize(5);
-    rec[4] = kind;
+    std::string& rec = batching_ ? batch_ : rec_;
+    if (!batching_) rec.clear();
+    const size_t at = rec.size();
+    size_t need = 5;
+    for (auto f : fields) need += 4 + f.size();
+    if (rec.capacity() - at < need) rec.reserve(std::max(at + need, 2 * rec.capacity()));
+    rec.resize(at + 5);
+    rec[at + 4] = kind;
     for (auto f : fields) put_field(rec, f);
-    uint32_t total = (uint32_t)rec.size();
-    std::memcpy(&rec[0], &total, 4);
-    if (batching_) {
-      batch_ += rec;
-      return;
-    }
+    uint32_t total = (uint32_t)(rec.size() - at);
+    std::memcpy(&rec[at], &total, 4);
+    if (batching_) return;
     write_all(rec);
+    if (rec.capacity() > kKeepBatch) std::string().swap(rec);
   }
 
   class BatchScope {
@@ -113,14 +117,19 @@
     ~BatchScope() noexcept(false) {
       log_.batching_ = false;
       if (log_.batch_.empty()) return;
-      std::string b;
-      b.swap(log_.batch_);
+      struct Clear {
+        std::string& b;
+        ~Clear() {
+          if (b.capacity() > kKeepBatch) std::string().swap(b);
+          else b.clear();
+        }
+      } clear{log_.batch_};
       if (std::uncaught_exceptions() == 0) {
-        log_.write_all(b);
+        log_.write_all(log_.batch_);
         return;
       }
       try {
-        log_.write_all(b);
+        log_.write_all(log_.batch_);
       } catch (...) {
       }
     }
@@ -306,7 +315,8 @@
   uint64_t bytes_ = 0;
   std::string path_;
   bool batching_ = false;
-  std::string batch_;
+  static constexpr size_t kKeepBatch = 1u << 20;
+  std::string batch_, rec_;
   std::mutex fd_mu_;
   std::atomic<uint64_t> written_{0}, synced_{0};
   std::mutex gc_mu_;
diff --git a/aca_dotnet_workshop_amd/native/src/backingfront.hpp b/aca_dotnet_workshop_amd/native/src/backingfront.hpp
--- a/aca_dotnet_workshop_amd/native/src/backingfront.hpp
+++ b/aca_dotnet_workshop_amd/native/src/backingfront.hpp
@@ -306,6 +306,41 @@
   }
 
  private:
+  struct Segs {
+    const std::string* p;
+    size_t n;
+    size_t size() const { return n; }
+    const std::string& operator[](size_t i) const { return p[i]; }
+  };
+
+  struct Scope {
+    std::array<std::string_view, 5> part{};
+    Scope(std::string_view a, std::string_view b = {}, std::string_view c = {}, std::string_view d = {},
+          std::string_view e = {})
+        : part{a, b, c, d, e} {}
+    Scope(const std::string& s) : part{std::string_view(s)} {}
+    Scope(const char* s) : part{std::string_view(s)} {}
+    bool starts_with(std::string_view prefix) const {
+      for (auto x : part) {
+        const size_t k = std::min(x.size(), prefix.size());
+        if (x.compare(0, k, prefix.substr(0, k)) != 0) return false;
+        prefix.remove_prefix(k);
+        if (prefix.empty()) return true;
+      }
+      return false;
+    }
+    std::string str() const {
+      std::string s;
+      for (auto x : part) s.append(x);
+      return s;
+    }
+  };
+  static Scope entity_scope(std::string_view ns, std::string_view entity) {
+    auto p = entity.find("/subscriptions/");
+    if (p != std::string_view::npos) return {"servicebus/", ns, "/topics/", entity.substr(0, p)};
+    return {"servicebus/", ns, "/queues/", entity};
+  }
+
   struct Coll {
     DocStore* store = nullptr;
   };
@@ -491,7 +526,7 @@
     return ::close(fd) == 0;
   }
 
-  bool handle_blob(ev::Message& m, ev::Reply& r, const std::vector<std::string>& seg, const std::string& qs) {
+  bool handle_blob(ev::Message& m, ev::Reply& r, const Segs& seg, const std::string& qs) {
     std::string acct, cont, root;
     if (!safe_name(seg[1], acct) || !safe_name(seg[3], cont)) return false;
     {
@@ -505,7 +540,7 @@
       if (c != "1" && c != "true") return false;
       if (!authorize(m, r, "blob.read", "storage/" + seg[1])) return true;
       count("blob.count");
-      r.send(200, {{"content-type", "application/json"}},
+      r.send(200, json_headers(),
              "{\"count\": " + std::to_string(blob_count(acct, cont, query_get(qs, "prefix"))) + "}");
       return true;
     }
@@ -540,7 +575,7 @@
       return true;
     }
     blob_note(acct, cont, name, true);
-    r.send(201, {{"content-type", "application/json"}},
+    r.send(201, json_headers(),
            "{\"blobURL\": " + bf::jstr("/storage/" + seg[1] + "/blobs/" + seg[3] + "/" + name) + "}");
     return true;
   }
@@ -566,36 +601,41 @@
         if (sh.get() != &here) sh->post(key);
   }
 
-  bool allowed(const ev::Message& m, const std::string& action, const std::string& scope) {
-    std::shared_lock l(cfg_mu_);
+  bool allowed_locked(const ev::Message& m, std::string_view action, const Scope& scope) const {
     if (!enforce_) return true;
     auto* key = m.header("x-tt-key");
     if (key && !key->empty())
       for (auto& [ks, k] : keys_)
-        if (scope.rfind(ks, 0) == 0 && *key == k) return true;
+        if (scope.starts_with(ks) && *key == k) return true;
     auto* ident = m.header("x-tt-identity");
     if (ident && !ident->empty())
       for (auto& g : grants_) {
-        if (g.principal != *ident || scope.rfind(g.scope, 0) != 0) continue;
+        if (g.principal != *ident || !scope.starts_with(g.scope)) continue;
         for (auto& a : g.actions)
           if (a == "*" || a == action) return true;
       }
     return false;
   }
-  bool authorize(const ev::Message& m, const ev::Reply& r, const std::string& action, const std::string& scope) {
-    if (allowed(m, action, scope)) return true;
+  void refuse(const ev::Message& m, const ev::Reply& r, std::string_view action, const Scope& scope) {
     auto* ident = m.header("x-tt-identity");
     std::string who = ident && !ident->empty() ? *ident : "anonymous";
     r.send(403, {{"content-type", "application/problem+json; charset=utf-8"}},
-           bf::problem_json(403, who + " is not authorized to perform " + action + " on " + scope));
-    return false;
-  }
-
-  static void split(const std::string& target, std::string& path, std::string& qs) {
-    auto q = target.find('?');
-    path = target.substr(0, q);
-    qs = q == std::string::npos ? "" : target.substr(q + 1);
-  }
+           bf::problem_json(403, who + " is not authorized to perform " + std::string(action) + " on " + scope.str()));
+  }
+  bool authorize(const ev::Message& m, const ev::Reply& r, std::string_view action, const Scope& scope) {
+    bool ok;
+    {
+      std::shared_lock l(cfg_mu_);
+      ok = allowed_locked(m, action, scope);
+    }
+    if (!ok) refuse(m, r, action, scope);
+    return ok;
+  }
+
+  struct Scratch {
+    std::vector<std::string> pool;
+    std::string qs;
+  };
   static std::string query_get(const std::string& qs, const std::string& name) {
     size_t i = 0;
     while (i <= qs.size() && !qs.empty()) {
@@ -611,16 +651,34 @@
   }
 
   void on_request(Shard& sh, ev::Message&& m, ev::Reply r) {
-    std::string path, qs;
-    split(m.target, path, qs);
-    std::vector<std::string> seg;
-    seg.reserve(8);
-    for (size_t i = 1; i <= path.size();) {
+    thread_local Scratch kept;
+    thread_local bool kept_busy = false;
+    Scratch own;
+    struct Hold {
+      bool mine;
+      ~Hold() {
+        if (mine) kept_busy = false;
+      }
+    } hold{!kept_busy};
+    Scratch& sc = hold.mine ? kept : own;
+    kept_busy = true;
+    std::vector<std::string>& pool = sc.pool;
+    std::string& qs = sc.qs;
+    const std::string_view target(m.target);
+    const size_t q = target.find('?');
+    const std::string_view path = target.substr(0, q);
+    qs.assign(q == std::string_view::npos ? std::string_view() : target.substr(q + 1));
+    size_t n = 0;
+    for (size_t i = 1; i <= path.size(); ++n) {
       size_t j = path.find('/', i);
-      if (j == std::string::npos) j = path.size();
-      seg.push_back(bf::unquote(std::string_view(path).substr(i, j - i)));
+      if (j == std::string_view::npos) j = path.size();
+      const std::string_view part = path.substr(i, j - i);
+      if (n == pool.size()) pool.emplace_back();
+      if (part.find('%') == std::string_view::npos) pool[n].assign(part);
+      else pool[n] = bf::unquote(part);
       i = j + 1;
     }
+    const Segs seg{pool.data(), n};
     if (seg.size() == 6 && seg[0] == "cosmos" && seg[4] == "docs" && handle_doc(sh, m, r, seg)) return;
     if (seg.size() == 5 && seg[0] == "cosmos" && seg[4] == "bulkset" && m.method == "POST" &&
         handle_bulkset(sh, m, r, seg))
@@ -684,48 +742,78 @@
     return true;
   }
 
-  Coll* coll_of(const std::vector<std::string>& seg) {
+  Coll* coll_of(const Segs& seg) {
+    const std::string& k = coll_key(seg);
+    std::shared_lock l(cfg_mu_);
+    return coll_locked(k);
+  }
+  Coll* coll_locked(const std::string& k) const {
+    auto it = colls_.find(k);
+    return it != colls_.end() && it->second->store ? it->second.get() : nullptr;
+  }
+  static const std::string& coll_key(const Segs& seg) {
     thread_local std::string k;
     k.assign(seg[1]);
     k += '\x1f';
     k += seg[2];
     k += '\x1f';
     k += seg[3];
-    std::shared_lock l(cfg_mu_);
-    auto it = colls_.find(k);
-    return it != colls_.end() && it->second->store ? it->second.get() : nullptr;
+    return k;
   }
 
   template <class Engine>
-  void send_durable(Shard& sh, Engine* eng, ev::Reply& r, int status, ev::HeaderList h, std::string body) {
+  void send_durable(Shard& sh, Engine* eng, ev::Reply& r, int status, const ev::HeaderList& h, std::string_view body) {
     if (!eng->group_commit()) {
       r.send(status, h, body);
       return;
     }
     std::weak_ptr<Shard> w = sh.self;
-    eng->after_durable(eng->log_mark(), [w, r, status, h = std::move(h), body = std::move(body)] {
+    eng->after_durable(eng->log_mark(), [w, r, status, h = ev::HeaderList(h), body = std::string(body)] {
       if (auto s = w.lock()) s->post_task([r, status, h, body] { r.send(status, h, body); });
     });
   }
 
-  bool handle_doc(Shard& sh, ev::Message& m, ev::Reply& r, const std::vector<std::string>& seg) {
-    Coll* c = coll_of(seg);
-    if (!c) return false;
+  static const ev::HeaderList& json_headers() {
+    static const ev::HeaderList h{{"content-type", "application/json"}};
+    return h;
+  }
+
+  bool handle_doc(Shard& sh, ev::Message& m, ev::Reply& r, const Segs& seg) {
+    const bool read = m.method == "GET";
+    if (!read) {
+      if (m.method != "PUT" && m.method != "DELETE") return false;
+      auto* ttl = m.header("x-tt-ttl-ms");
+      if (ttl && !ttl->empty() && *ttl != "0") return false;
+    }
     const std::string& key = seg[5];
-    const std::string scope = "cosmos/" + seg[1];
-    if (m.method == "GET") {
-      if (!authorize(m, r, "cosmos.read", scope)) return true;
+    const Scope scope("cosmos/", seg[1]);
+    const char* action = read ? "cosmos.read" : "cosmos.write";
+    Coll* c;
+    bool ok;
+    {
+      const std::string& k = coll_key(seg);
+      std::shared_lock l(cfg_mu_);
+      c = coll_locked(k);
+      if (!c) return false;
+      ok = allowed_locked(m, action, scope);
+    }
+    if (!ok) {
+      refuse(m, r, action, scope);
+      return true;
+    }
+    thread_local ev::HeaderList etag_headers{{"etag", ""}, {"content-type", "application/json"}};
+    if (read) {
       count("doc.get");
       if (throttled(m, r, c->store, DocStore::read_ru(0), DocStore::kRead)) return true;
       auto v = c->store->get(key);
-      if (!v) r.empty(404);
-      else r.send(200, {{"etag", v->second}, {"content-type", "application/json"}}, v->first);
-      return true;
-    }
-    if (m.method != "PUT" && m.method != "DELETE") return false;
-    auto* ttl = m.header("x-tt-ttl-ms");
-    if (ttl && !ttl->empty() && *ttl != "0") return false;
-    if (!authorize(m, r, "cosmos.write", scope)) return true;
+      if (!v) {
+        r.empty(404);
+      } else {
+        etag_headers[0].second.assign(v->second);
+        r.send(200, etag_headers, v->first);
+      }
+      return true;
+    }
     auto* im = m.header("if-match");
     std::optional<std::string> etag;
     if (im && !im->empty()) etag = *im;
@@ -737,9 +825,11 @@
       count("doc.put");
       auto* fw = m.header("x-tt-first-write");
       try {
-        std::string e = c->store->set(key, m.body, etag, fw && *fw == "1", 0);
-        send_durable(sh, c->store, r, 200, {{"etag", e}, {"content-type", "application/json"}},
-                     "{\"etag\": " + bf::jstr(e) + "}");
+        std::string& e = etag_headers[0].second;
+        e = c->store->set(key, std::move(m.body), etag, fw && *fw == "1", 0);
+        char out[48];
+        const int n = std::snprintf(out, sizeof out, "{\"etag\": \"%s\"}", e.c_str());
+        send_durable(sh, c->store, r, 200, etag_headers, std::string_view(out, (size_t)n));
       } catch (const EtagMismatch& ex) {
         r.send(412, {{"content-type", pj}}, bf::problem_json(412, ex.what()));
       } catch (const ParseError& ex) {
@@ -758,7 +848,7 @@
     return true;
   }
 
-  bool handle_bulkset(Shard& sh, ev::Message& m, ev::Reply& r, const std::vector<std::string>& seg) {
+  bool handle_bulkset(Shard& sh, ev::Message& m, ev::Reply& r, const Segs& seg) {
     Coll* c = coll_of(seg);
     if (!c) return false;
     std::vector<DocStore::BulkItem> batch;
@@ -783,11 +873,11 @@
       }
     }
     out += "]";
-    send_durable(sh, c->store, r, etag_err ? 412 : other_err ? 400 : 200, {{"content-type", "application/json"}}, out);
+    send_durable(sh, c->store, r, etag_err ? 412 : other_err ? 400 : 200, json_headers(), out);
     return true;
   }
 
-  bool handle_bulkget(ev::Message& m, ev::Reply& r, const std::vector<std::string>& seg) {
+  bool handle_bulkget(ev::Message& m, ev::Reply& r, const Segs& seg) {
     Coll* c = coll_of(seg);
     if (!c) return false;
     Value body;
@@ -813,7 +903,7 @@
       out += "}";
     }
     out += "]";
-    r.send(200, {{"content-type", "application/json"}}, out);
+    r.send(200, json_headers(), out);
     return true;
   }
 
@@ -851,7 +941,7 @@
     return (std::strtol(tp->c_str() + tp->size() - 2, nullptr, 16) & 1) != 0;
   }
 
-  bool to_query_worker(Shard& sh, ev::Message& m, ev::Reply& r, Coll* c, const std::vector<std::string>& seg,
+  bool to_query_worker(Shard& sh, ev::Message& m, ev::Reply& r, Coll* c, const Segs& seg,
                        const std::string& qs) {
     {
       std::lock_guard l(q_mu_);
@@ -924,7 +1014,7 @@
     }
   }
 
-  bool handle_query(Shard& sh, ev::Message& m, ev::Reply& r, const std::vector<std::string>& seg, const std::string& qs) {
+  bool handle_query(Shard& sh, ev::Message& m, ev::Reply& r, const Segs& seg, const std::string& qs) {
     Coll* c = coll_of(seg);
     if (!c) return false;
     bool indexed = false;
@@ -949,44 +1039,64 @@
     }
     count("doc.query");
     c->store->debit(DocStore::query_ru(body.size()) - DocStore::query_ru(0));
-    r.send(200, {{"content-type", "application/json"}}, body);
+    r.send(200, json_headers(), body);
     return true;
   }
 
-  static std::string entity_scope(const std::string& entity) {
-    auto p = entity.find("/subscriptions/");
-    if (p != std::string::npos) return "topics/" + entity.substr(0, p);
-    return "queues/" + entity;
-  }
-
-  bool handle_bus(Shard& sh, ev::Message& m, ev::Reply& r, const std::vector<std::string>& seg,
+  bool handle_bus(Shard& sh, ev::Message& m, ev::Reply& r, const Segs& seg,
                   const std::string& qs) {
+    const std::string& ns = seg[1];
+    enum { Publish, Receive, Settle, Counts } route;
+    if (seg.size() == 5 && seg[2] == "topics" && seg[4] == "messages" && m.method == "POST") route = Publish;
+    else if (seg.size() == 3 && seg[2] == "receive" && m.method == "POST") route = Receive;
+    else if (seg.size() == 3 && seg[2] == "settle" && m.method == "POST") route = Settle;
+    else if (seg.size() == 3 && seg[2] == "counts" && m.method == "GET") route = Counts;
+    else return false;
+    std::string entity;
+    Value body;
+    if (route == Receive) {
+      entity = query_get(qs, "entity");
+    } else if (route == Settle) {
+      try {
+        body = parse(m.body.empty() ? std::string_view("{}") : std::string_view(m.body));
+      } catch (const std::exception&) {
+        return false;
+      }
+      if (auto* e = body.get("entity"); e && e->t == Value::String) entity = e->s;
+    }
+    const Scope scope = route == Publish ? Scope("servicebus/", ns, "/topics/", seg[3]) : entity_scope(ns, entity);
+    const char* action = route == Publish ? "sb.send" : "sb.receive";
     Broker* b = nullptr;
+    bool ok = true;
     {
       std::shared_lock l(cfg_mu_);
-      auto it = brokers_.find(seg[1]);
+      auto it = brokers_.find(ns);
       if (it != brokers_.end()) b = it->second;
-    }
-    if (!b) return false;
-    const std::string& ns = seg[1];
-    if (seg.size() == 5 && seg[2] == "topics" && seg[4] == "messages" && m.method == "POST") {
-      if (!authorize(m, r, "sb.send", "servicebus/" + ns + "/topics/" + seg[3])) return true;
+      if (!b) return false;
+      if (route != Counts) ok = allowed_locked(m, action, scope);
+    }
+    if (!ok) {
+      refuse(m, r, action, scope);
+      return true;
+    }
+    if (route == Publish) {
       count("sb.publish");
+      static const std::string kJson("application/json"), kNoProps("{}"), kNoId;
       auto* ct = m.header("content-type");
       auto* props = m.header("x-tt-props");
       auto* mid = m.header("x-tt-message-id");
       auto* ttl = m.header("x-tt-ttl-ms");
       auto* delay = m.header("x-tt-delay-ms");
-      uint64_t seq = b->publish(seg[3], m.body, ct ? *ct : "application/json", props ? *props : "{}", mid ? *mid : "",
+      uint64_t seq = b->publish(seg[3], m.body, ct ? *ct : kJson, props ? *props : kNoProps, mid ? *mid : kNoId,
                                 ttl && !ttl->empty() ? std::atoll(ttl->c_str()) : 0,
                                 delay && !delay->empty() ? std::atoll(delay->c_str()) : 0);
-      send_durable(sh, b, r, 201, {{"content-type", "application/json"}}, "{\"seq\": " + std::to_string(seq) + "}");
+      char out[40];
+      const int n = std::snprintf(out, sizeof out, "{\"seq\": %llu}", (unsigned long long)seq);
+      send_durable(sh, b, r, 201, json_headers(), std::string_view(out, (size_t)n));
       for (auto& sub : b->subscriptions(seg[3])) broadcast(sh, ns + "|" + seg[3] + "/subscriptions/" + sub);
       return true;
     }
-    if (seg.size() == 3 && seg[2] == "receive" && m.method == "POST") {
-      std::string entity = query_get(qs, "entity");
-      if (!authorize(m, r, "sb.receive", "servicebus/" + ns + "/" + entity_scope(entity))) return true;
+    if (route == Receive) {
       count("sb.receive");
       std::string mx = query_get(qs, "max"), lk = query_get(qs, "lockMs"), wt = query_get(qs, "waitMs");
       Parked p{ns, entity, (size_t)std::max(1, mx.empty() ? 1 : std::atoi(mx.c_str())),
@@ -995,16 +1105,7 @@
       if (!try_receive(b, p, false)) sh.parked.emplace(ns + "|" + entity, std::move(p));
       return true;
     }
-    if (seg.size() == 3 && seg[2] == "settle" && m.method == "POST") {
-      Value body;
-      try {
-        body = parse(m.body.empty() ? std::string_view("{}") : std::string_view(m.body));
-      } catch (const std::exception&) {
-        return false;
-      }
-      std::string entity;
-      if (auto* e = body.get("entity"); e && e->t == Value::String) entity = e->s;
-      if (!authorize(m, r, "sb.receive", "servicebus/" + ns + "/" + entity_scope(entity))) return true;
+    if (route == Settle) {
       count("sb.settle");
       auto list = [&](const char* k) -> const std::vector<Value>* {
         auto* v = body.get(k);
@@ -1012,41 +1113,48 @@
       };
       auto str = [](const Value& o, const char* k) {
         auto* v = o.get(k);
-        return v && v->t == Value::String ? v->s : std::string();
+        return v && v->t == Value::String ? std::string_view(v->s) : std::string_view();
       };
       auto num = [](const Value& o, const char* k) {
         auto* v = o.get(k);
         return v && v->t == Value::Number ? (int64_t)v->n : (int64_t)0;
       };
-      std::string out = "{\"complete\": [";
+      using Op = Broker::SettleOp;
+      std::vector<Op> ops;
+      size_t ends[4] = {0, 0, 0, 0};
       if (auto* l = list("complete"))
-        for (size_t i = 0; i < l->size(); ++i) out += std::string(i ? ", " : "") + (b->complete(entity, (*l)[i].s) ? "true" : "false");
-      out += "], \"abandon\": [";
-      bool abandoned = false;
+        for (auto& t : *l) ops.push_back({Op::Complete, std::string_view(t.s), 0, {}});
+      ends[0] = ops.size();
       if (auto* l = list("abandon"))
-        for (size_t i = 0; i < l->size(); ++i) {
-          abandoned = true;
-          out += std::string(i ? ", " : "") +
-                 (b->abandon(entity, str((*l)[i], "token"), num((*l)[i], "delayMs")) ? "true" : "false");
+        for (auto& a : *l) ops.push_back({Op::Abandon, str(a, "token"), num(a, "delayMs"), {}});
+      ends[1] = ops.size();
+      if (auto* l = list("deadletter"))
+        for (auto& d : *l) ops.push_back({Op::DeadLetter, str(d, "token"), 0, str(d, "reason")});
+      ends[2] = ops.size();
+      if (auto* l = list("renew"))
+        for (auto& x : *l) ops.push_back({Op::Renew, str(x, "token"), num(x, "lockMs"), {}});
+      ends[3] = ops.size();
+      const bool abandoned = ends[1] > ends[0];
+      std::vector<char> res;
+      b->settle(entity, ops, res);
+      static const char* const kNames[4] = {"{\"complete\": [", "], \"abandon\": [", "], \"deadletter\": [", "], \"renew\": ["};
+      std::string out;
+      out.reserve(64 + 7 * ops.size());
+      for (size_t k = 0, i = 0; k < 4; ++k) {
+        out += kNames[k];
+        for (const size_t from = i; i < ends[k]; ++i) {
+          if (i > from) out += ", ";
+          out += res[i] ? "true" : "false";
         }
-      out += "], \"deadletter\": [";
-      if (auto* l = list("deadletter"))
-        for (size_t i = 0; i < l->size(); ++i)
-          out += std::string(i ? ", " : "") +
-                 (b->dead_letter(entity, str((*l)[i], "token"), str((*l)[i], "reason")) ? "true" : "false");
-      out += "], \"renew\": [";
-      if (auto* l = list("renew"))
-        for (size_t i = 0; i < l->size(); ++i)
-          out += std::string(i ? ", " : "") +
-                 (b->renew(entity, str((*l)[i], "token"), num((*l)[i], "lockMs")) ? "true" : "false");
+      }
       out += "]}";
-      send_durable(sh, b, r, 200, {{"content-type", "application/json"}}, out);
+      send_durable(sh, b, r, 200, json_headers(), out);
       if (abandoned) broadcast(sh, ns + "|" + entity);
       return true;
     }
-    if (seg.size() == 3 && seg[2] == "counts" && m.method == "GET") {
+    {
       auto [a, s, l, d, e, c, rc] = b->counts(query_get(qs, "entity"));
-      r.send(200, {{"content-type", "application/json"}},
+      r.send(200, json_headers(),
              "{\"active\": " + std::to_string(a) + ", \"scheduled\": " + std::to_string(s) + ", \"locked\": " +
                  std::to_string(l) + ", \"dead_letter\": " + std::to_string(d) + ", \"enqueued\": " + std::to_string(e) +
                  ", \"completed\": " + std::to_string(c) + ", \"received\": " + std::to_string(rc) + "}");
@@ -1074,7 +1182,7 @@
     return plain_uint(v, out);
   }
 
-  bool handle_storage_queue(Shard& sh, ev::Message& m, ev::Reply& r, const std::vector<std::string>& seg,
+  bool handle_storage_queue(Shard& sh, ev::Message& m, ev::Reply& r, const Segs& seg,
                             const std::string& qs) {
     const std::string ns = "storage-" + seg[1];
     Broker* b = nullptr;
@@ -1092,7 +1200,7 @@
       if (!authorize(m, r, "queue.send", "storage/" + account)) return true;
       count("queue.put");
       uint64_t seq = b->send(queue, m.body, "text/plain", "{}", "", ttl_s * 1000, delay_s * 1000);
-      send_durable(sh, b, r, 201, {{"content-type", "application/json"}},
+      send_durable(sh, b, r, 201, json_headers(),
                    "{\"messageId\": \"" + std::to_string(seq) + "\"}");
       broadcast(sh, ns + "|" + queue);
       return true;
@@ -1146,7 +1254,7 @@
         else out += ", \"bodyB64\": \"" + bf::b64(x.body) + "\"}";
       }
       out += "]";
-      p.reply.send(200, {{"content-type", "application/json"}}, out);
+      p.reply.send(200, json_headers(), out);
       return true;
     }
     for (size_t i = 0; i < msgs.size(); ++i) {
@@ -1161,7 +1269,7 @@
       else out += ", \"bodyB64\": \"" + bf::b64(x.body) + "\"}";
     }
     out += "]";
-    p.reply.send(200, {{"content-type", "application/json"}}, out);
+    p.reply.send(200, json_headers(), out);
     return true;
   }
 
diff --git a/aca_dotnet_workshop_amd/native/src/broker.hpp b/aca_dotnet_workshop_amd/native/src/broker.hpp
--- a/aca_dotnet_workshop_amd/native/src/broker.hpp
+++ b/aca_dotnet_workshop_amd/native/src/broker.hpp
@@ -8,6 +8,7 @@
 #include <mutex>
 #include <random>
 #include <string>
+#include <string_view>
 #include <tuple>
 #include <unordered_map>
 #include <vector>
@@ -239,54 +240,51 @@
   bool complete(const std::string& path, const std::string& token) {
     std::lock_guard<std::mutex> g(mu_);
     Queue* q = find(path, false);
-    if (!q) return false;
-    auto it = q->locked.find(token);
-    if (it == q->locked.end()) return false;
-    uint64_t seq = it->second->seq;
-    q->locked.erase(it);
-    q->n_completed++;
-    if (log_.is_open()) log_.append('C', {path, AppLog::pod(seq)});
-    return true;
+    return q && complete_locked(*q, path, token);
   }
 
   bool abandon(const std::string& path, const std::string& token, int64_t delay_ms) {
     std::lock_guard<std::mutex> g(mu_);
     Queue* q = find(path, false);
-    if (!q) return false;
-    auto it = q->locked.find(token);
-    if (it == q->locked.end()) return false;
-    MsgPtr m = it->second;
-    q->locked.erase(it);
-    int64_t now = mono_ms();
-    m->visible_at = now + std::max<int64_t>(0, delay_ms);
-    q->release(m, now, "MaxDeliveryCountExceeded");
-    if (!m->dl_reason.empty() && log_.is_open()) log_.append('C', {path, AppLog::pod(m->seq)});
-    return true;
+    return q && abandon_locked(*q, path, token, delay_ms);
   }
 
   bool dead_letter(const std::string& path, const std::string& token, const std::string& reason) {
     std::lock_guard<std::mutex> g(mu_);
     Queue* q = find(path, false);
-    if (!q) return false;
-    auto it = q->locked.find(token);
-    if (it == q->locked.end()) return false;
-    MsgPtr m = it->second;
-    q->locked.erase(it);
-    q->dead_letter(m, reason);
-    if (log_.is_open()) log_.append('C', {path, AppLog::pod(m->seq)});
-    return true;
+    return q && dead_letter_locked(*q, path, token, reason);
   }
 
   bool renew(const std::string& path, const std::string& token, int64_t lock_ms) {
     std::lock_guard<std::mutex> g(mu_);
     Queue* q = find(path, false);
-    if (!q) return false;
-    auto it = q->locked.find(token);
-    if (it == q->locked.end()) return false;
-    int64_t now = mono_ms();
-    it->second->locked_until = now + (lock_ms > 0 ? lock_ms : q->opt.lock_ms);
-    q->lock_expiry.emplace(it->second->locked_until, token);
-    return true;
+    return q && renew_locked(*q, token, lock_ms);
+  }
+
+  struct SettleOp {
+    enum Kind : uint8_t { Complete, Abandon, DeadLetter, Renew };
+    Kind kind;
+    std::string_view token;
+    int64_t ms = 0;
+    std::string_view reason;
+  };
+  void settle(const std::string& path, const std::vector<SettleOp>& ops, std::vector<char>& ok) {
+    ok.assign(ops.size(), 0);
+    if (ops.empty()) return;
+    std::lock_guard<std::mutex> g(mu_);
+    Queue* q = find(path, false);
+    if (!q) return;
+    AppLog::BatchScope batch(log_);
+    for (size_t i = 0; i < ops.size(); ++i) {
+      const SettleOp& op = ops[i];
+      settle_key_.assign(op.token);
+      switch (op.kind) {
+        case SettleOp::Complete: ok[i] = complete_locked(*q, path, settle_key_); break;
+        case SettleOp::Abandon: ok[i] = abandon_locked(*q, path, settle_key_, op.ms); break;
+        case SettleOp::DeadLetter: ok[i] = dead_letter_locked(*q, path, settle_key_, std::string(op.reason)); break;
+        case SettleOp::Renew: ok[i] = renew_locked(*q, settle_key_, op.ms); break;
+      }
+    }
   }
 
   std::vector<std::tuple<uint64_t, std::string, std::string, std::string, uint32_t>> drain_dead_letters(
@@ -365,6 +363,47 @@
     if (!replaying_ && log_.is_open()) log_.append('S', {topic, sub, AppLog::pod(q.opt.lock_ms),
                                                         AppLog::pod(q.opt.max_delivery), AppLog::pod(q.opt.default_ttl_ms)});
     return &q;
+  }
+
+  bool complete_locked(Queue& q, const std::string& path, const std::string& token) {
+    auto it = q.locked.find(token);
+    if (it == q.locked.end()) return false;
+    uint64_t seq = it->second->seq;
+    q.locked.erase(it);
+    q.n_completed++;
+    if (log_.is_open()) log_.append('C', {path, AppLog::pod(seq)});
+    return true;
+  }
+
+  bool abandon_locked(Queue& q, const std::string& path, const std::string& token, int64_t delay_ms) {
+    auto it = q.locked.find(token);
+    if (it == q.locked.end()) return false;
+    MsgPtr m = it->second;
+    q.locked.erase(it);
+    int64_t now = mono_ms();
+    m->visible_at = now + std::max<int64_t>(0, delay_ms);
+    q.release(m, now, "MaxDeliveryCountExceeded");
+    if (!m->dl_reason.empty() && log_.is_open()) log_.append('C', {path, AppLog::pod(m->seq)});
+    return true;
+  }
+
+  bool dead_letter_locked(Queue& q, const std::string& path, const std::string& token, const std::string& reason) {
+    auto it = q.locked.find(token);
+    if (it == q.locked.end()) return false;
+    MsgPtr m = it->second;
+    q.locked.erase(it);
+    q.dead_letter(m, reason);
+    if (log_.is_open()) log_.append('C', {path, AppLog::pod(m->seq)});
+    return true;
+  }
+
+  bool renew_locked(Queue& q, const std::string& token, int64_t lock_ms) {
+    auto it = q.locked.find(token);
+    if (it == q.locked.end()) return false;
+    int64_t now = mono_ms();
+    it->second->locked_until = now + (lock_ms > 0 ? lock_ms : q.opt.lock_ms);
+    q.lock_expiry.emplace(it->second->locked_until, token);
+    return true;
   }
 
   MsgPtr make(uint64_t seq, const std::string& id, const std::string& body, const std::string& ctype,
@@ -435,6 +474,7 @@
   }
 
   std::mutex mu_;
+  std::string settle_key_;
   std::map<std::string, Queue> queues_;
   std::map<std::string, std::map<std::string, Queue>> topics_;
   std::unordered_map<std::string, std::map<uint64_t, bool>> pending_;
diff --git a/aca_dotnet_workshop_amd/native/src/docstore.hpp b/aca_dotnet_workshop_amd/native/src/docstore.hpp
--- a/aca_dotnet_workshop_amd/native/src/docstore.hpp
+++ b/aca_dotnet_workshop_amd/native/src/docstore.hpp
@@ -201,14 +201,17 @@
 
   std::string set(const std::string& key, const std::string& value, const std::optional<std::string>& etag,
                   bool first_write, int64_t ttl_ms) {
+    return set(key, std::string(value), etag, first_write, ttl_ms);
+  }
+  std::string set(const std::string& key, std::string&& value, const std::optional<std::string>& etag,
+                  bool first_write, int64_t ttl_ms) {
     Value parsed = parse(value);
-    std::string text(value);
     std::vector<Doc> graveyard;
     std::lock_guard<std::mutex> g(mu_);
     int64_t now = now_ms();
     auto it = docs_.find(key);
     check_etag_at(it, etag, first_write, now);
-    it = put_at(it, key, std::move(text), std::move(parsed), ttl_ms > 0 ? now + ttl_ms : 0, &graveyard);
+    it = put_at(it, key, std::move(value), std::move(parsed), ttl_ms > 0 ? now + ttl_ms : 0, &graveyard);
     log_put(key, it->second.value, it->second.etag, it->second.expire_ms);
     maybe_compact();
     return std::to_string(it->second.etag);
diff --git a/aca_dotnet_workshop_amd/native/src/module.cpp b/aca_dotnet_workshop_amd/native/src/module.cpp
--- a/aca_dotnet_workshop_amd/native/src/module.cpp
+++ b/aca_dotnet_workshop_amd/native/src/module.cpp
@@ -913,6 +913,40 @@
              return ok;
            },
            py::arg("path"), py::arg("token"), py::arg("reason") = "", py::call_guard<py::gil_scoped_release>())
+      .def("settle",
+           [](Broker& b, const std::string& path, const std::vector<std::string>& complete,
+              const std::vector<std::pair<std::string, int64_t>>& abandon,
+              const std::vector<std::pair<std::string, std::string>>& deadletter,
+              const std::vector<std::pair<std::string, int64_t>>& renew) {
+             using Op = Broker::SettleOp;
+             std::vector<Op> ops;
+             for (auto& t : complete) ops.push_back({Op::Complete, t, 0, {}});
+             for (auto& a : abandon) ops.push_back({Op::Abandon, a.first, a.second, {}});
+             for (auto& d : deadletter) ops.push_back({Op::DeadLetter, d.first, 0, d.second});
+             for (auto& x : renew) ops.push_back({Op::Renew, x.first, x.second, {}});
+             std::vector<char> ok;
+             {
+               py::gil_scoped_release rel;
+               b.settle(path, ops, ok);
+               b.wait_durable();
+             }
+             py::dict out;
+             size_t i = 0;
+             auto take = [&](const char* name, size_t n) {
+               py::list l;
+               for (size_t k = 0; k < n; ++k) l.append(py::bool_(ok[i++] != 0));
+               out[name] = l;
+             };
+             take("complete", complete.size());
+             take("abandon", abandon.size());
+             take("deadletter", deadletter.size());
+             take("renew", renew.size());
+             return out;
+           },
+           py::arg("path"), py::arg("complete") = std::vector<std::string>(),
+           py::arg("abandon") = std::vector<std::pair<std::string, int64_t>>(),
+           py::arg("deadletter") = std::vector<std::pair<std::string, std::string>>(),
+           py::arg("renew") = std::vector<std::pair<std::string, int64_t>>())
       .def("group_commit", &Broker::group_commit)
       .def("commit_stats",
            [](Broker& b) {
diff --git a/aca_dotnet_workshop_amd/native/src/textutil.hpp b/aca_dotnet_workshop_amd/native/src/textutil.hpp
--- a/aca_dotnet_workshop_amd/native/src/textutil.hpp
+++ b/aca_dotnet_workshop_amd/native/src/textutil.hpp
@@ -32,18 +32,36 @@
   return o;
 }
 
+struct QuoteSafe {
+  bool safe[256] = {};
+  constexpr QuoteSafe() {
+    for (int c = '0'; c <= '9'; ++c) safe[c] = true;
+    for (int c = 'a'; c <= 'z'; ++c) safe[c] = true;
+    for (int c = 'A'; c <= 'Z'; ++c) safe[c] = true;
+    safe[(int)'_'] = safe[(int)'.'] = safe[(int)'-'] = safe[(int)'~'] = true;
+  }
+};
+inline constexpr QuoteSafe kQuoteSafe{};
+
+inline void quote_all_to(std::string& o, std::string_view s) {
+  static const char* d = "0123456789ABCDEF";
+  size_t run = 0;
+  for (size_t i = 0; i < s.size(); ++i) {
+    const unsigned char c = (unsigned char)s[i];
+    if (kQuoteSafe.safe[c]) continue;
+    o.append(s.data() + run, i - run);
+    run = i + 1;
+    o += '%';
+    o += d[c >> 4];
+    o += d[c & 15];
+  }
+  o.append(s.data() + run, s.size() - run);
+}
+
 inline std::string quote_all(std::string_view s) {
-  static const char* d = "0123456789ABCDEF";
   std::string o;
-  for (unsigned char c : s) {
-    if (std::isalnum(c) || c == '_' || c == '.' || c == '-' || c == '~') {
-      o += (char)c;
-    } else {
-      o += '%';
-      o += d[c >> 4];
-      o += d[c & 15];
-    }
-  }
+  o.reserve(s.size() + 8);
+  quote_all_to(o, s);
   return o;
 }
 
```

After: 91370 (median of 4 runs). No clear change (+0.6%).
